# zhizdev/mvdfusion

Measured on AMD Instinct MI355X. Metric: denoising-steps/sec, higher is better.
Workload: dtype f16x3 (f16 MFMA operands split hi+lo, 3 partial products, fp32 accumulate); 1 GPU; BASELINE.json configs[1]: V=4 views x 256^2 images (32x32 latents), D=1, 50-step DDIM (eta 1), cfg 2.5, SD1.x UNet 320ch + 10 view-aligned transformers + GridAttn, random-init (deterministic fill) weights; views=4, latent=32, depth_samples=1, parallelism=single GPU, CFG pair batched as 2V, hipgraph=True, gemm_tuning=mvdfusion_amd/tuned/gemm_f16.json: 426 problems; 0 problems tuned in this run

## Files before the change

include/mvd_hip.h:

```cpp
#ifndef MVD_HIP_H
#define MVD_HIP_H
#include <stddef.h>
#include <stdint.h>
#ifdef __cplusplus
extern "C" {
#endif

typedef void* mvd_stream_t;

#define MVD_VERSION 100
#define MVD_PREC_X1 1
#define MVD_PREC_X3 3
#define MVD_PREC_X4 4

int mvd_version(void);
const char* mvd_last_error(void);
int mvd_operand_format(void);

size_t mvd_packed_weight_bytes(int N, int K);
int mvd_pack_linear_weight(const float* w, int N, int K, int ldw, int geglu, float scale, void* packed,
                           mvd_stream_t stream);
int mvd_pack_linear_weight_t(const float* wt, int N, int K, int ldw, float scale, void* packed, mvd_stream_t stream);
int mvd_pack_conv3x3_weight(const float* w, int Cout, int Cin, int cin_pad, float scale, void* packed,
                            mvd_stream_t stream);

#define MVD_A_DENSE 0
#define MVD_A_CONV3X3 1

#define MVD_EPI_STORE 0
#define MVD_EPI_GEGLU 1
#define MVD_EPI_QKV 2

#define MVD_ACT_NONE 0
#define MVD_ACT_GELU 1
#define MVD_ACT_SILU 2
#define MVD_ACT_QUICKGELU 3

#define MVD_GEMM_TILES 5
#define MVD_GEMM_LOOPS 8
#define MVD_GEMM_CFG_STRIDE 32
#define MVD_B_PACKED 0
#define MVD_B_PLANES 1

typedef struct mvd_prefetch_item_s {
  const void* ptr;
  unsigned long long bytes;
  int start_after;
  int consumer;
} mvd_prefetch_item;

typedef struct mvd_gemm_desc {
  int M, N, K;
  const void* A;
  int lda;
  int a_mode;
  int B, Hin, Win, Cin, Hout, Wout, stride, upsample;
  int no_pad_tl;
  const void* Wp;
  int b_mode;
  int ldb;
  float acc_scale;
  int prec;
  int epi;
  int act;
  float* out;
  int ldo;
  void* out_sp;
  int ldp;
  int n_store;
  const float* bias;
  const float* bias_b;
  int rows_per_batch;
  int ldbb;
  const float* colscale;
  const float* res;
  int ldr;
  void *q_hi, *q_lo, *k_hi, *k_lo, *vt_hi, *vt_lo;
  int heads, dhead, L, Lpad;
  float qscale;
  int splitk;
  float* workspace;
  size_t workspace_elems;
  int cfg;
  long long* gn_stats;
  int gn_hw, gn_groups;
  float* rs_out;
  int* rs_count;
  int rs_ld;
  const float* ln_stats;
  const int* ln_count;
  const float* ln_colsum;
  int ln_ld, ln_dim;
  float ln_eps;
  void* gna_out_sp;
  const float* gna_gamma;
  const float* gna_beta;
  float gna_eps;
  int gna_flags;
  const float* cat_b;
  int cat_cb;
  void* cat_raw_sp;
  const float* acc_scale_dev;
  const struct mvd_prefetch_item_s* pf_items;
  int pf_n;
  int tap_mode;
  const void* A2;
  int lda2, Cin2;
} mvd_gemm_desc;
#define MVD_TAPS_FULL 0
#define MVD_TAPS_UP4 1
#define MVD_TAPS_CENTRE_TAIL 2
#define MVD_GNA_SILU 1
#define MVD_GNA_ROUND_F16 2
#define MVD_GNA_OUT_UNUSED 4

int mvd_gemm(const mvd_gemm_desc* d, mvd_stream_t stream);
int mvd_gemm_cfg_supported(const mvd_gemm_desc* d, int cfg);

int mvd_split_planes(const float* x, void* sp, size_t rows, int cols, int ldx, int ldp, mvd_stream_t stream);
int mvd_split_planes_scaled(const float* x, void* sp, size_t rows, int cols, int ldx, int ldp, const float* scale_dev, mvd_stream_t stream);

int mvd_gemv(const float* W, const float* bias, const float* x, float* y, int M, int N, int K, int ldx, int ldy,
             int act_in, int act_out, mvd_stream_t stream);

int mvd_groupnorm_chunks(int HW);
int mvd_groupnorm_nhwc(const float* x, void* y_sp, const float* gamma, const float* beta, int B, int HW, int C,
                       int groups, float eps, int silu, double* ws, size_t ws_elems, mvd_stream_t stream);
int mvd_groupnorm_from_stats(const float* x, void* y_sp, const float* gamma, const float* beta, const long long* stats, int B, int HW,
                             int C, int groups, float eps, int silu, mvd_stream_t stream);
int mvd_softmax_rows(const float* x, void* y_sp, int rows, int cols, int ldx, float scale, float out_scale,
                     mvd_stream_t stream);

int mvd_layernorm(const float* x, void* y_sp, float* y_f32, const float* w, const float* b, int rows, int C, float eps,
                  int w_plus_one, mvd_stream_t stream);
int mvd_layernorm_groups(const float* x, void* y_sp, float* y_f32, const float* w, const float* b, int ldw, int rows, int rows_per_group,
                         int C, float eps, int w_plus_one, mvd_stream_t stream);

size_t mvd_attn_qk_plane_elems(int B, int heads, int L, int dhead);
size_t mvd_attn_vt_plane_elems(int B, int heads, int L, int dhead);
int mvd_attn_lpad(int L);
int mvd_attention(const void* q_hi, const void* q_lo, const void* k_hi, const void* k_lo, const void* vt_hi,
                  const void* vt_lo, void* out_sp, int ldo, int B, int heads, int L, int Lkeys, int dhead, int prec,
                  mvd_stream_t stream);

int mvd_pixel_cross_attn(const float* q, const float* k, const float* v, void* out_sp, int P, int D, int heads,
                         int dhead, mvd_stream_t stream);

int mvd_unet_input(const float* x, const float* input_latents, void* out_sp, int V, int S, int cpad, int cfg,
                   mvd_stream_t stream);
int mvd_unet_input_scenes(const float* x, const float* input_latents, void* out_sp, int nscene, int V, int S, int cpad, int cfg,
                          mvd_stream_t stream);
int mvd_concat_channels(const float* a, int Ca, const float* b, int Cb, float* out, void* out_sp, int rows, long long* gn_stats,
                        int gn_hw, int gn_groups, mvd_stream_t stream);
int mvd_concat_groupnorm_fits(int Ca, int Cb, int hw, int groups);
int mvd_concat_groupnorm(const float* a, int Ca, const float* b, int Cb, float* out, void* raw_sp, void* y_sp, const float* gamma,
                         const float* beta, long long* gn_stats, int B, int hw, int groups, float eps, int silu, mvd_stream_t stream);
int mvd_area_pool(const float* vol, void* out_sp, int B, int S, int D, int C, int factor, int ldp, mvd_stream_t stream);
int mvd_fill_zero(float* p, size_t n, mvd_stream_t stream);

#define MVD_STEP_STRIDE 8
int mvd_timestep_embedding(const float* steps, const int* iter, const float* freqs, float* out, int dim,
                           mvd_stream_t stream);
int mvd_timestep_embedding_scenes(const float* steps, const int* iter, const float* freqs, float* out, int dim, int nscene,
                                  int steps_scene_stride, mvd_stream_t stream);
int mvd_advance_iter(int* iter, mvd_stream_t stream);

#define MVD_CAM_RECORD 20
#define MVD_TOKEN_DIM 723
#define MVD_TOKEN_LD 736
int mvd_zembed(const float* lat, const float* w, const float* b, float* feat, int N, int S, mvd_stream_t stream);
int mvd_gridattn_tokens(const float* x, const float* depth_noise, const float* steps, const int* iter,
                        const float* grid_lin ,
                        const float* feat, const float* in_feat, const float* cams, const float* in_cam,
                        void* tokens_sp, int V, int q0, int Vq, int S, int D, float depth_scale, float depth_shift,
                        mvd_stream_t stream);
int mvd_gridattn_tokens_scenes(const float* x, const float* depth_noise, const float* steps, const int* iter, const float* grid_lin,
                               const float* feat, const float* in_feat, const float* cams, const float* in_cam, void* tokens_sp,
                               int nscene, int V, int q0, int Vq, int S, int D, float depth_scale, float depth_shift,
                               mvd_stream_t stream);
int mvd_gridattn_tokens_scenes_t(const float* x, const float* depth_noise, const float* steps, const int* iter, const float* grid_lin,
                                 const float* feat, const float* in_feat, const float* cams, const float* in_cam, void* tokens_sp,
                                 int nscene, int V, int q0, int Vq, int S, int D, float depth_scale, float depth_shift,
                                 int steps_scene_stride, mvd_stream_t stream);
int mvd_gridattn_fused_slots(void);
size_t mvd_gridattn_fused_stream_bytes(void);
size_t mvd_gridattn_fused_vec_floats(void);
int mvd_gridattn_fused(const float* x, const float* depth_noise, const float* steps, const int* iter, const float* grid_lin,
                       const float* feat, const float* in_feat, const float* cams, const float* in_cam, const void* wstream,
                       const float* vecs, void* pooled_sp, int V, int q0, int Vq, int S, int D, float depth_scale,
                       float depth_shift, int prec ,
                       mvd_stream_t stream);
int mvd_gridattn_fused_scenes(const float* x, const float* depth_noise, const float* steps, const int* iter, const float* grid_lin,
                              const float* feat, const float* in_feat, const float* cams, const float* in_cam, const void* wstream,
                              const float* vecs, void* pooled_sp, int nscene, int V, int q0, int Vq, int S, int D, float depth_scale,
                              float depth_shift, int prec, mvd_stream_t stream);
int mvd_gridattn_fused_scenes_t(const float* x, const float* depth_noise, const float* steps, const int* iter, const float* grid_lin,
                                const float* feat, const float* in_feat, const float* cams, const float* in_cam, const void* wstream,
                                const float* vecs, void* pooled_sp, int nscene, int V, int q0, int Vq, int S, int D, float depth_scale,
                                float depth_shift, int prec, int steps_scene_stride, int vecs_scene_stride, mvd_stream_t stream);
int mvd_gridattn_tokens_window(const float* x, const float* depth_noise, const float* steps, const int* iter, const float* grid_lin,
                               const float* feat, const float* in_feat, const float* cams, const float* in_cam, void* tokens_sp,
                               int nscene, int V, int q0, int Vq, int S, int D, float depth_scale, float depth_shift,
                               int steps_scene_stride, int window, mvd_stream_t stream);
int mvd_gridattn_fused_window(const float* x, const float* depth_noise, const float* steps, const int* iter, const float* grid_lin,
                              const float* feat, const float* in_feat, const float* cams, const float* in_cam, const void* wstream,
                              const float* vecs, void* pooled_sp, int nscene, int V, int q0, int Vq, int S, int D, float depth_scale,
                              float depth_shift, int prec, int steps_scene_stride, int vecs_scene_stride, int window,
                              mvd_stream_t stream);
int mvd_view_mha(const float* qkv, void* out_sp, int Nseq, int V, int heads, int dhead,
                 mvd_stream_t stream);
int mvd_view_pool(const float* x, const float* w, const float* b, void* out_sp, int Nseq, int V, int C,
                  mvd_stream_t stream);

int mvd_cfg_ddim_update(const float* eps_nhwc, int ldc, float* x, float* x0, float* eps_out,
                        const float* ddim_noise, size_t noise_stride ,
                        const float* steps, const int* iter, int V, int S, int cfg, float cfg_scale, int do_update,
                        mvd_stream_t stream);

int mvd_pin_views(float* x, float* x0, const float* known, const float* noise, size_t noise_stride ,
                  const float* steps, const int* iter, int groups, int group_views, int K, int S, int mode, mvd_stream_t stream);

#define MVD_FUSE_FOREGROUND 1
#define MVD_FUSE_STAGE_AUTO 0
#define MVD_FUSE_STAGE_GLOBAL 1
#define MVD_FUSE_STAGE_LDS 2
int mvd_fuse_points(const float* lat, const float* rgb, const float* cams, const float* ndc_lin, float* xyz, float* color,
                    uint8_t* support, uint8_t* conflict, uint8_t* flags, int nscene, int V, int S, int up, float depth_scale,
                    float depth_shift, float lo, float hi, float tau, int stage, mvd_stream_t stream);
size_t mvd_compact_points_scratch(size_t npts);
int mvd_compact_points(const float* xyz, const float* color, const uint8_t* support, const uint8_t* conflict, const uint8_t* flags,
                       size_t npts, int min_support, int max_conflicts, float* out_xyz, float* out_color, uint8_t* out_support,
                       int* out_index, unsigned* count, void* scratch, size_t scratch_bytes, mvd_stream_t stream);

#define MVD_SPLAT_MAX_RADIUS 4
#define MVD_RENDER_FILL 1
#define MVD_RENDER_SPLAT 2
#define MVD_RENDER_RESOLVE 4
#define MVD_RENDER_ALL 7
size_t mvd_render_points_scratch(int ncam, int P);
int mvd_render_points(const float* xyz, const float* color, const int* scene_start, const float* cams, size_t n, int nscene, int M, int P,
                      int radius, float znear, float empty_depth, const float* background, int* index, float* depth, float* rgb,
                      void* scratch, size_t scratch_bytes, mvd_stream_t stream);
int mvd_render_points_stages(const float* xyz, const float* color, const int* scene_start, const float* cams, size_t n, int nscene, int M,
                             int P, int radius, float znear, float empty_depth, const float* background, int* index, float* depth,
                             float* rgb, void* scratch, size_t scratch_bytes, int stages, mvd_stream_t stream);

size_t mvd_render_mesh_scratch(int ncam, int P);
int mvd_render_mesh(const float* vertices, const float* colors, const int* faces, const int* vertex_start, const int* face_start,
                    const float* cams, size_t nvert, size_t nface, int nscene, int M, int P, int cull, float znear, float empty_depth,
                    const float* background, int* face_out, float* depth, float* bary, float* normal, float* rgb, void* scratch,
                    size_t scratch_bytes, mvd_stream_t stream);
int mvd_render_mesh_stages(const float* vertices, const float* colors, const int* faces, const int* vertex_start, const int* face_start,
                           const float* cams, size_t nvert, size_t nface, int nscene, int M, int P, int cull, float znear,
                           float empty_depth, const float* background, int* face_out, float* depth, float* bary, float* normal, float* rgb,
                           void* scratch, size_t scratch_bytes, int stages, mvd_stream_t stream);

#define MVD_NN_AUTO 0
#define MVD_NN_BRUTE 1
#define MVD_NN_GRID 2
#define MVD_NN_BUILD 1
#define MVD_NN_QUERY 2
#define MVD_NN_ALL 3
size_t mvd_nearest_points_scratch(size_t nt, int nscene, int method, int grid);
int mvd_nearest_points(const float* query, const int* query_start, const float* target, const int* target_start, size_t nq, size_t nt,
                       int nscene, int method, int grid, int* index, float* dist2, void* scratch, size_t scratch_bytes,
                       mvd_stream_t stream);
int mvd_nearest_points_stages(const float* query, const int* query_start, const float* target, const int* target_start, size_t nq,
                              size_t nt, int nscene, int method, int grid, int* index, float* dist2, void* scratch, size_t scratch_bytes,
                              int stages, mvd_stream_t stream);

#define MVD_KNN_MAX_K 32
#define MVD_NORMALS_MAX_K 256
#define MVD_NORMALS_SWEEPS 10
int mvd_knn_points(const float* query, const int* query_start, const float* target, const int* target_start, size_t nq, size_t nt,
                   int nscene, int k, int method, int grid, int* index, float* dist2, void* scratch, size_t scratch_bytes,
                   mvd_stream_t stream);
int mvd_knn_points_stages(const float* query, const int* query_start, const float* target, const int* target_start, size_t nq, size_t nt,
                          int nscene, int k, int method, int grid, int* index, float* dist2, void* scratch, size_t scratch_bytes,
                          int stages, mvd_stream_t stream);
int mvd_point_normals(const float* target, size_t nt, const int* index, size_t n, int k, const float* points, const float* toward,
                      float* normal, float* variation, mvd_stream_t stream);

#define MVD_ALIGN_SCALE 1
#define MVD_ALIGN_NO_STEP 2
#define MVD_ALIGN_CHUNK 1024
#define MVD_ALIGN_SUMS 19
#define MVD_ALIGN_HISTORY 3
#define MVD_ALIGN_MAX_ITERS 1024
size_t mvd_align_scratch(size_t nq, size_t nt, int nscene, int method, int grid);
int mvd_align_solve(const double* sums, int flags, double* step, double* scale);
int mvd_align_apply(const float* src, const int* src_start, size_t n, int nscene, const double* transform, float* out,
                    mvd_stream_t stream);
int mvd_align_fit(const float* moved, const int* start, const float* target, const int* index, const float* dist2, size_t n, size_t nt,
                  int nscene, int flags, float max_dist2, double* transform, double* history_row, void* scratch, size_t scratch_bytes,
                  mvd_stream_t stream);
int mvd_align_icp(const float* source, const int* source_start, const float* target, const int* target_start, size_t nq, size_t nt,
                  int nscene, int method, int grid, int iters, int flags, float max_dist2, double* transform, double* history,
                  float* moved, int* index, float* dist2, void* scratch, size_t scratch_bytes, mvd_stream_t stream);

#define MVD_PLANE_NO_STEP 2
#define MVD_PLANE_SUMS 30
#define MVD_PLANE_HISTORY 4
#define MVD_PLANE_EPS_RANK 1e-9
size_t mvd_plane_scratch(size_t nq, size_t nt, int nscene, int method, int grid);
int mvd_plane_solve(const double* sums, double* step, int* rank);
int mvd_plane_fit(const float* moved, const int* start, const float* target, const float* normals, const int* index, const float* dist2,
                  size_t n, size_t nt, int nscene, int flags, float max_dist2, double* transform, double* history_row, void* scratch,
                  size_t scratch_bytes, mvd_stream_t stream);
int mvd_plane_icp(const float* source, const int* source_start, const float* target, const int* target_start, const float* normals,
                  size_t nq, size_t nt, int nscene, int method, int grid, int iters, float max_dist2, double* transform, double* history,
                  float* moved, int* index, float* dist2, void* scratch, size_t scratch_bytes, mvd_stream_t stream);

#define MVD_MESH_SPAN 3
size_t mvd_nearest_on_mesh_scratch(size_t nf, int nscene, int method, int grid);
int mvd_nearest_on_mesh(const float* query, const int* query_start, const float* vertices, const int* faces, const int* face_start, size_t nq,
                        size_t nv, size_t nf, int nscene, int method, int grid, int* face, float* dist2, float* point, float* bary,
                        int* region, float* normal, void* scratch, size_t scratch_bytes, mvd_stream_t stream);
int mvd_nearest_on_mesh_stages(const float* query, const int* query_start, const float* vertices, const int* faces, const int* face_start,
                               size_t nq, size_t nv, size_t nf, int nscene, int method, int grid, int* face, float* dist2, float* point,
                               float* bary, int* region, float* normal, void* scratch, size_t scratch_bytes, int stages,
                               mvd_stream_t stream);
size_t mvd_mesh_icp_scratch(size_t nq, size_t nf, int nscene, int method, int grid);
int mvd_mesh_icp(const float* source, const int* source_start, const float* vertices, const int* faces, const int* face_start, size_t nq,
                 size_t nv, size_t nf, int nscene, int method, int grid, int iters, float max_dist2, double* transform, double* history,
                 float* moved, int* face, float* dist2, float* point, float* normal, void* scratch, size_t scratch_bytes,
                 mvd_stream_t stream);

#define MVD_REGISTER_MAX_H 16384
#define MVD_REGISTER_MAX_K 32
size_t mvd_register_scratch(size_t ns, size_t nt, int nscene, int H, int method, int grid);
int mvd_register_score(const float* sample, const int* sample_start, const float* target, const int* target_start, size_t ns, size_t nt,
                       int nscene, int H, const double* hyp, float trunc2, int method, int grid, double* score, int* inliers, void* scratch,
                       size_t scratch_bytes, mvd_stream_t stream);
int mvd_register_select(const double* score, const double* quat, int nscene, int H, int K, double cos_half, int* top, double* top_score,
                        mvd_stream_t stream);

int mvd_tsdf_integrate(const float* lat, const float* rgb, const float* cams, float* tsdf, uint8_t* weight, float* color, uint8_t* cweight,
                       int nscene, int V, int S, int up, int G, float cx, float cy, float cz, float half_extent, float trunc, int carve,
                       float depth_scale, float depth_shift, float lo, float hi, mvd_stream_t stream);
size_t mvd_mesh_scratch(int nscene, int G);
int mvd_mesh_count(const float* tsdf, const uint8_t* weight, int nscene, int G, int* vertex_start, int* face_start, void* scratch,
                   size_t scratch_bytes, mvd_stream_t stream);
int mvd_mesh_emit(const float* tsdf, const uint8_t* weight, const float* color, const uint8_t* cweight, int nscene, int G, float cx, float cy,
                  float cz, float half_extent, const float* fill, float* vertices, float* colors, int* faces, size_t nvert, size_t nface,
                  const void* scratch, size_t scratch_bytes, mvd_stream_t stream);

#define MVD_TOPO_TOTALS 11
#define MVD_TOPO_FLAG_BOUNDARY 1
#define MVD_TOPO_FLAG_NONMANIFOLD 2
#define MVD_SMOOTH_MAX_PASSES 2000
size_t mvd_mesh_incidence_scratch(size_t nv, size_t nf);
int mvd_mesh_incidence(const int* faces, const int* vertex_start, const int* face_start, size_t nv, size_t nf, int nscene, int* inc_start,
                       int* inc, void* scratch, size_t scratch_bytes, mvd_stream_t stream);
size_t mvd_mesh_label_scratch(size_t nv, size_t nf);
int mvd_mesh_label(const int* faces, const int* vertex_start, const int* face_start, size_t nv, size_t nf, int nscene, int* vertex_component,
                   int* face_component, int* component_start, void* scratch, size_t scratch_bytes, mvd_stream_t stream);
int mvd_mesh_component_table(const int* vertex_component, const int* face_component, size_t nv, size_t nf, size_t ncomp, int* root, int* faces,
                             int* vertices, mvd_stream_t stream);
size_t mvd_mesh_topology_scratch(size_t nv, size_t nf);
int mvd_mesh_topology(const int* faces, const int* vertex_start, const int* face_start, size_t nv, size_t nf, int nscene, const int* inc_start,
                      const int* inc, const int* vertex_component, const int* component_start, int* totals, uint8_t* vertex_flags,
                      void* scratch, size_t scratch_bytes, mvd_stream_t stream);
size_t mvd_mesh_filter_scratch(size_t nv, size_t nf);
int mvd_mesh_filter_count(const int* faces, const uint8_t* keep, const int* vertex_start, const int* face_start, size_t nv, size_t nf,
                          int nscene, int* new_vertex_start, int* new_face_start, void* scratch, size_t scratch_bytes, mvd_stream_t stream);
int mvd_mesh_filter_emit(const float* vertices, const float* rgb, const int* faces, size_t nv, size_t nf, float* out_vertices, float* out_rgb,
                         int* out_faces, int* vertex_index, int* face_index, size_t nvo, size_t nfo, const void* scratch,
                         size_t scratch_bytes, mvd_stream_t stream);
int mvd_mesh_vertex_normals(const float* vertices, const int* faces, const int* inc_start, const int* inc, size_t nv, size_t nf,
                            float* normals, mvd_stream_t stream);
// ... 92 lines not shown
```

mvdfusion_amd/csrc/elementwise.hip:

```cpp
#include "common.hpp"
#include "../../include/mvd_hip.h"

namespace {

__device__ __forceinline__ float act_apply(float v, int act) {
  if (act == MVD_ACT_GELU) return gelu_erf(v);
  if (act == MVD_ACT_SILU) return silu_f(v);
  return v;
}

template <int MR>
__global__ __launch_bounds__(256) void gemv_kernel(const float* __restrict__ W, const float* __restrict__ bias,
                                                   const float* __restrict__ x, float* __restrict__ y, int M, int N, int K, int ldx,
                                                   int ldy, int act_in, int act_out) {
  const int lane = threadIdx.x & 63;
  const int n = blockIdx.x * 4 + (threadIdx.x >> 6);
  if (n >= N) return;
  float acc[MR];
#pragma unroll
  for (int m = 0; m < MR; ++m) acc[m] = 0.f;
  const float* wr = W + (size_t)n * K;
  if ((K & 3) == 0) {
    for (int k = lane * 4; k < K; k += 256) {
      const float4 w4 = *(const float4*)(wr + k);
#pragma unroll
      for (int m = 0; m < MR; ++m) {
        if (m < M) {
          float4 x4 = *(const float4*)(x + (size_t)m * ldx + k);
          if (act_in) {
            x4.x = act_apply(x4.x, act_in);
            x4.y = act_apply(x4.y, act_in);
            x4.z = act_apply(x4.z, act_in);
            x4.w = act_apply(x4.w, act_in);
          }
          acc[m] += w4.x * x4.x + w4.y * x4.y + w4.z * x4.z + w4.w * x4.w;
        }
      }
    }
  } else {
    for (int k = lane; k < K; k += 64) {
      const float w1 = wr[k];
#pragma unroll
      for (int m = 0; m < MR; ++m)
        if (m < M) acc[m] += w1 * act_apply(x[(size_t)m * ldx + k], act_in);
    }
  }
#pragma unroll
  for (int m = 0; m < MR; ++m) {
    if (m < M) {
      float v = wave_sum(acc[m]);
      if (lane == 0) {
        if (bias) v += bias[n];
        y[(size_t)m * ldy + n] = act_apply(v, act_out);
      }
    }
  }
}

__global__ __launch_bounds__(256) void unet_input_kernel(const float* __restrict__ x, const float* __restrict__ il,
                                                         u16* __restrict__ out_sp, int V, int Vs, int S, int cpad, int nb) {
  const int SS = S * S;
  const size_t total = (size_t)nb * SS * cpad;
  for (size_t e = (size_t)blockIdx.x * 256 + threadIdx.x; e < total; e += (size_t)gridDim.x * 256) {
    const int c = (int)(e % cpad);
    const int pix = (int)((e / cpad) % SS);
    const int b = (int)(e / ((size_t)cpad * SS));
    const int v = b < V ? b : b - V;
    float o = 0.f;
    if (c < 5) {
      o = x[((size_t)v * 5 + c) * SS + pix];
    } else if (c < 10 && b < V) {
      const float t = il[((size_t)(b / Vs) * 5 + (c - 5)) * SS + pix];
      o = (c < 9) ? t / 0.18215f : t;
    }
    store_sp1(out_sp, e / cpad, cpad, c, o);
  }
}

__global__ __launch_bounds__(256) void concat_kernel(const float4* __restrict__ a, int ca4, const float4* __restrict__ b, int cb4,
                                                     float4* __restrict__ out, u16* __restrict__ out_sp, size_t rows) {
  const int c4 = ca4 + cb4;
  const size_t total = rows * c4;
  for (size_t e = (size_t)blockIdx.x * 256 + threadIdx.x; e < total; e += (size_t)gridDim.x * 256) {
    const size_t r = e / c4;
    const int c = (int)(e - r * c4);
    const float4 v = c < ca4 ? a[r * ca4 + c] : b[r * cb4 + (c - ca4)];
    out[e] = v;
    if (out_sp) store_sp4(out_sp, r, c4 * 4, c * 4, v.x, v.y, v.z, v.w);
  }
}

__global__ __launch_bounds__(256) void concat_stats_kernel(const float4* __restrict__ a, int ca4, const float4* __restrict__ b, int cb4,
                                                           float4* __restrict__ out, u16* __restrict__ out_sp, long long* __restrict__ stats,
                                                           int hw, int groups) {
  __shared__ float cs[2][4][256];
  const int c4n = ca4 + cb4, C = c4n * 4;
  const size_t m0 = (size_t)blockIdx.x * 16;
  const int n0 = blockIdx.y * 256;
  const int c4 = blockIdx.y * 64 + (threadIdx.x & 63), rg = threadIdx.x >> 6;
  float4 s = make_float4(0.f, 0.f, 0.f, 0.f), q = make_float4(0.f, 0.f, 0.f, 0.f);
  if (c4 < c4n) {
    float4 v[4];
#pragma unroll
    for (int r = 0; r < 4; ++r) {
      const size_t row = m0 + rg * 4 + r;
      v[r] = c4 < ca4 ? a[row * ca4 + c4] : b[row * cb4 + (c4 - ca4)];
    }
#pragma unroll
    for (int r = 0; r < 4; ++r) {
      const size_t row = m0 + rg * 4 + r;
      out[row * c4n + c4] = v[r];
      if (out_sp) store_sp4(out_sp, row, C, c4 * 4, v[r].x, v[r].y, v[r].z, v[r].w);
      s.x += v[r].x; s.y += v[r].y; s.z += v[r].z; s.w += v[r].w;
      q.x += v[r].x * v[r].x; q.y += v[r].y * v[r].y; q.z += v[r].z * v[r].z; q.w += v[r].w * v[r].w;
    }
  }
  *(float4*)&cs[0][rg][(threadIdx.x & 63) * 4] = s;
  *(float4*)&cs[1][rg][(threadIdx.x & 63) * 4] = q;
  __syncthreads();
  const int c = threadIdx.x, nn = n0 + c;
  const float cs_ = cs[0][0][c] + cs[0][1][c] + cs[0][2][c] + cs[0][3][c];
  const float cq_ = cs[1][0][c] + cs[1][1][c] + cs[1][2][c] + cs[1][3][c];
  __syncthreads();
  cs[0][0][c] = cs_;
  cs[1][0][c] = cq_;
  __syncthreads();
  if (nn >= C) return;
  const int cg = C / groups;
  const int g = nn / cg, pos = nn - g * cg;
  if (c != 0 && pos != 0) return;
  int len = cg - pos;
  if (len > 256 - c) len = 256 - c;
  float ss = 0.f, qq = 0.f;
  for (int j = 0; j < len; ++j) {
    ss += cs[0][0][c + j];
    qq += cs[1][0][c + j];
  }
  gn_stats_add(stats, (int)(m0 / hw), g, groups, ss, qq);
}

#define MVD_CGN_THREADS 1024
__global__ __launch_bounds__(MVD_CGN_THREADS) void concat_gn_kernel(const float* __restrict__ a, int ca, const float* __restrict__ b, int cb,
                                                                    float* __restrict__ out, u16* __restrict__ raw_sp, u16* __restrict__ y_sp,
                                                                    const float* __restrict__ gamma, const float* __restrict__ beta,
                                                                    long long* __restrict__ stats, int hw, int groups, float eps, int flags) {
  constexpr int NT = MVD_CGN_THREADS, NWV = NT / 64, U = 4;
  extern __shared__ float s_val[];
  __shared__ double s_red[2][NWV];
  __shared__ float s_coef[2][128];
  const int C = ca + cb, cg = C / groups, cg2 = cg >> 1;
  int g, img;
  {
    const int bid = blockIdx.x;
    if ((groups & 7) == 0) {
      const int gpx = groups >> 3, x = bid & 7, r = bid >> 3;
      g = x * gpx + r % gpx;
      img = r / gpx;
    } else {
      g = bid % groups;
      img = bid / groups;
    }
  }
  const int tid = threadIdx.x, lane = tid & 63, wave = tid >> 6;
  const int c0 = g * cg;
  const size_t m0 = (size_t)img * hw;
  const int total = hw * cg2;
  const int dq = NT / cg2, dj = NT - dq * cg2;
  const int rs = tid / cg2, js = tid - rs * cg2;
  const int r0 = tid < total ? rs : 0, j0 = tid < total ? js : 0;
  float s = 0.f, q = 0.f;
  {
    int r = rs, j = js;
    for (int e0 = tid; e0 < total; e0 += NT * U) {
      float2 v[U];
      int rr[U], jj[U];
      bool ok[U];
#pragma unroll
      for (int u = 0; u < U; ++u) {
        ok[u] = e0 + u * NT < total;
        rr[u] = ok[u] ? r : r0;
        jj[u] = ok[u] ? j : j0;
        r += dq;
        j += dj;
        if (j >= cg2) {
          j -= cg2;
          ++r;
        }
      }
#pragma unroll
      for (int u = 0; u < U; ++u) {
        const size_t m = m0 + rr[u];
        const int n = c0 + 2 * jj[u];
        v[u] = *(const float2*)(n < ca ? a + m * ca + n : b + m * cb + (n - ca));
      }
#pragma unroll
      for (int u = 0; u < U; ++u) {
        if (ok[u]) {
          const size_t m = m0 + rr[u];
          const int n = c0 + 2 * jj[u];
          if (out) *(float2*)(out + m * C + n) = v[u];
          if (raw_sp) {
            uint32_t hh, ll;
            split_op16x2(v[u].x, v[u].y, hh, ll);
            u16* pp = raw_sp + sp_index(m, C, n);
            *(uint32_t*)pp = hh;
            *(uint32_t*)(pp + 32) = ll;
          }
          *(float2*)(s_val + 2 * (e0 + u * NT)) = v[u];
          s += v[u].x + v[u].y;
          q += v[u].x * v[u].x + v[u].y * v[u].y;
        }
      }
    }
  }
  {
    const double sd = wave_sum_d((double)s), qd = wave_sum_d((double)q);
    if (lane == 0) {
      s_red[0][wave] = sd;
      s_red[1][wave] = qd;
    }
  }
  __syncthreads();
  double S1 = 0.0, S2 = 0.0;
#pragma unroll
  for (int w = 0; w < NWV; ++w) {
    S1 += s_red[0][w];
    S2 += s_red[1][w];
  }
  const double cnt = (double)hw * cg;
  const double mean = S1 / cnt;
  double var = S2 / cnt - mean * mean;
  if (var < 0.0) var = 0.0;
  const float rstd = (float)(1.0 / sqrt(var + (double)eps));
  if (tid < cg) {
    const float aa = rstd * gamma[c0 + tid];
    s_coef[0][tid] = aa;
    s_coef[1][tid] = beta[c0 + tid] - (float)mean * aa;
  }
  if (tid == 0 && stats) gn_stats_add(stats, img, g, groups, (float)S1, (float)S2);
  __syncthreads();
  {
    int r = rs, j = js;
    for (int e = tid; e < total; e += NT) {
      float2 v = *(const float2*)(s_val + 2 * e);
      v.x = v.x * s_coef[0][2 * j] + s_coef[1][2 * j];
      v.y = v.y * s_coef[0][2 * j + 1] + s_coef[1][2 * j + 1];
      if (flags & 2) {
        v.x = (float)(_Float16)v.x;
        v.y = (float)(_Float16)v.y;
      }
      if (flags & 1) {
        v.x = silu_f(v.x);
        v.y = silu_f(v.y);
      }
      uint32_t hh, ll;
      split_op16x2(v.x, v.y, hh, ll);
      u16* pp = y_sp + sp_index(m0 + r, C, c0 + 2 * j);
      *(uint32_t*)pp = hh;
      *(uint32_t*)(pp + 32) = ll;
      r += dq;
      j += dj;
      if (j >= cg2) {
        j -= cg2;
        ++r;
      }
    }
  }
}

__global__ __launch_bounds__(256) void area_pool_kernel(const float4* __restrict__ vol, u16* __restrict__ out_sp, int B, int S,
                                                        int D, int C4, int f, int ldp) {
  const int So = S / f;
  const size_t total = (size_t)B * So * So * D * C4;
  const float inv = 1.0f / (float)(f * f);
  for (size_t e = (size_t)blockIdx.x * 256 + threadIdx.x; e < total; e += (size_t)gridDim.x * 256) {
    const int c = (int)(e % C4);
    size_t r = e / C4;
    const int d = (int)(r % D);
    r /= D;
    const int ox = (int)(r % So);
    r /= So;
    const int oy = (int)(r % So);
    const int b = (int)(r / So);
    float4 acc = make_float4(0.f, 0.f, 0.f, 0.f);
    for (int dy = 0; dy < f; ++dy)
#pragma unroll 8
      for (int dx = 0; dx < f; ++dx) {
        const float4 v = vol[((((size_t)b * S + oy * f + dy) * S + ox * f + dx) * D + d) * C4 + c];
        acc.x += v.x;
        acc.y += v.y;
        acc.z += v.z;
        acc.w += v.w;
      }
    store_sp4(out_sp, e / C4, ldp, c * 4, acc.x * inv, acc.y * inv, acc.z * inv, acc.w * inv);
  }
}

__global__ __launch_bounds__(256) void fill_zero_kernel(float* p, size_t n) {
  for (size_t e = (size_t)blockIdx.x * 256 + threadIdx.x; e < n; e += (size_t)gridDim.x * 256) p[e] = 0.f;
}

__global__ void timestep_embedding_kernel(const float* __restrict__ steps, const int* __restrict__ iter,
                                          const float* __restrict__ freqs, float* __restrict__ out, int dim, int steps_scene_stride) {
  const float t = steps[((size_t)iter[0] + (size_t)blockIdx.x * steps_scene_stride) * MVD_STEP_STRIDE + 0];
  out += (size_t)blockIdx.x * dim;
  const int half = dim / 2;
  for (int i = threadIdx.x; i < half; i += blockDim.x) {
    const float a = t * freqs[i];
    out[i] = cosf(a);
    out[half + i] = sinf(a);
  }
}

__global__ void advance_iter_kernel(int* iter) {
  if (threadIdx.x == 0) iter[0] += 1;
}

__global__ __launch_bounds__(256) void cfg_ddim_kernel(const float* __restrict__ eps_nhwc, int ldc, float* __restrict__ x,
                                                       float* __restrict__ x0, float* __restrict__ eps_out,
                                                       const float* __restrict__ noise, const float* __restrict__ steps,
                                                       const int* __restrict__ iter, int V, int S, int cfg, float cfg_scale,
                                                       int do_update, size_t noise_stride) {
  const int it = iter[0];
  const float* st = steps + (size_t)it * MVD_STEP_STRIDE;
  const float a_t = st[3], a_prev = st[4], sigma = st[5], s1m = st[6], has_noise = st[7];
  const int SS = S * S;
  const size_t total = (size_t)V * 5 * SS;
  for (size_t e = (size_t)blockIdx.x * 256 + threadIdx.x; e < total; e += (size_t)gridDim.x * 256) {
    const int pix = (int)(e % SS);
    const int c = (int)((e / SS) % 5);
    const int b = (int)(e / ((size_t)5 * SS));
    float ep = eps_nhwc[((size_t)b * SS + pix) * ldc + c];
    if (cfg) {
      const float eu = eps_nhwc[((size_t)(V + b) * SS + pix) * ldc + c];
      ep = eu + cfg_scale * (ep - eu);
    }
    if (eps_out) eps_out[e] = ep;
    if (do_update) {
      const float xv = x[e];
      const float px0 = (xv - s1m * ep) / sqrtf(a_t);
      const float dir = sqrtf(fmaxf(1.0f - a_prev - sigma * sigma, 1e-7f)) * ep;
      float xp = sqrtf(a_prev) * px0 + dir;
      if (has_noise != 0.f) xp = xp + sigma * noise[(size_t)it * noise_stride + e];
      x0[e] = px0;
      x[e] = xp;
    }
  }
}

template <typename T>
__device__ __forceinline__ T pin_axpy(float sa, const T& k, float s1, const T& n);
template <>
__device__ __forceinline__ float pin_axpy<float>(float sa, const float& k, float s1, const float& n) {
  return sa * k + s1 * n;
}
template <>
__device__ __forceinline__ float4 pin_axpy<float4>(float sa, const float4& k, float s1, const float4& n) {
  return make_float4(sa * k.x + s1 * n.x, sa * k.y + s1 * n.y, sa * k.z + s1 * n.z, sa * k.w + s1 * n.w);
}

template <typename T>
__global__ __launch_bounds__(256) void pin_views_kernel(T* __restrict__ x, T* __restrict__ x0, const T* __restrict__ known,
                                                        const T* __restrict__ noise, size_t nstride, const float* __restrict__ steps,
                                                        const int* __restrict__ iter, int group_views, int K, size_t rowlen, size_t total,
                                                        int mode) {
  float sa = 1.f, s1 = 0.f;
  size_t nbase = 0;
  if (mode == 1) {
    const int it = iter[0];
    const float* st = steps + (size_t)it * MVD_STEP_STRIDE;
    sa = st[1];
    s1 = st[6];
    nbase = (size_t)it * nstride;
  }
  for (size_t e = (size_t)blockIdx.x * 256 + threadIdx.x; e < total; e += (size_t)gridDim.x * 256) {
    const size_t p = e / rowlen;
    const size_t off = e - p * rowlen;
    const size_t dst = ((p / K) * group_views + p % K) * rowlen + off;
    const T kv = known[e];
    if (mode == 1) {
      x[dst] = pin_axpy<T>(sa, kv, s1, noise[nbase + e]);
      x0[dst] = kv;
    } else {
      x[dst] = kv;
    }
  }
}

inline int grid_for(size_t total, int cap = 2048) {
  size_t b = (total + 255) / 256;
  if (b > (size_t)cap) b = cap;
  if (b < 1) b = 1;
  return (int)b;
}

}

extern "C" int mvd_gemv(const float* W, const float* bias, const float* x, float* y, int M, int N, int K, int ldx, int ldy,
                        int act_in, int act_out, mvd_stream_t stream) {
  MVD_CHECK_ARG(W && x && y && M > 0 && M <= 16 && N > 0 && K > 0, "mvd_gemv: bad arguments (M <= 16)");
  if ((K & 3) == 0) MVD_CHECK_ARG((ldx & 3) == 0, "mvd_gemv: ldx must be a multiple of 4 when K is");
  hipStream_t s = (hipStream_t)stream;
  dim3 grid(cdiv(N, 4)), block(256);
  if (M <= 1)
    hipLaunchKernelGGL(gemv_kernel<1>, grid, block, 0, s, W, bias, x, y, M, N, K, ldx, ldy, act_in, act_out);
  else if (M <= 4)
    hipLaunchKernelGGL(gemv_kernel<4>, grid, block, 0, s, W, bias, x, y, M, N, K, ldx, ldy, act_in, act_out);
  else
    hipLaunchKernelGGL(gemv_kernel<16>, grid, block, 0, s, W, bias, x, y, M, N, K, ldx, ldy, act_in, act_out);
  MVD_CHECK_LAUNCH("mvd_gemv");
  return 0;
}

extern "C" int mvd_unet_input_scenes(const float* x, const float* input_latents, void* out_sp, int nscene, int V, int S, int cpad, int cfg,
                                     mvd_stream_t stream) {
  MVD_CHECK_ARG(x && input_latents && out_sp && cpad % 32 == 0 && V > 0 && S > 0 && cpad >= 10, "mvd_unet_input: bad arguments");
  MVD_CHECK_ARG(nscene >= 1 && (long long)nscene * V <= 0x3fffffff, "mvd_unet_input_scenes: nscene=%d (>= 1)", nscene);
  const int NV = nscene * V;
  const int nb = cfg ? 2 * NV : NV;
  const size_t total = (size_t)nb * S * S * cpad;
  hipLaunchKernelGGL(unet_input_kernel, dim3(grid_for(total)), dim3(256), 0, (hipStream_t)stream, x, input_latents, (u16*)out_sp, NV, V,
                     S, cpad, nb);
  MVD_CHECK_LAUNCH("mvd_unet_input");
  return 0;
}

extern "C" int mvd_unet_input(const float* x, const float* input_latents, void* out_sp, int V, int S, int cpad, int cfg,
                              mvd_stream_t stream) {
  return mvd_unet_input_scenes(x, input_latents, out_sp, 1, V, S, cpad, cfg, stream);
}

extern "C" int mvd_concat_channels(const float* a, int Ca, const float* b, int Cb, float* out, void* out_sp, int rows,
                                   long long* gn_stats, int gn_hw, int gn_groups, mvd_stream_t stream) {
  if (out_sp) MVD_CHECK_ARG((Ca + Cb) % 32 == 0, "mvd_concat_channels: split-planes output needs (Ca+Cb) %% 32 == 0");
  MVD_CHECK_ARG(a && b && out && rows > 0 && Ca > 0 && Cb > 0 && Ca % 4 == 0 && Cb % 4 == 0,
                "mvd_concat_channels: bad arguments (channel counts must be multiples of 4)");
  if (gn_stats) {
    MVD_CHECK_ARG(rows % 16 == 0 && gn_hw > 0 && gn_hw % 16 == 0 && gn_groups > 0 && (Ca + Cb) % gn_groups == 0,
                  "mvd_concat_channels: gn_stats needs rows %% 16 == 0, gn_hw %% 16 == 0, C %% groups == 0");
    hipLaunchKernelGGL(concat_stats_kernel, dim3(rows / 16, (Ca + Cb + 255) / 256), dim3(256), 0, (hipStream_t)stream, (const float4*)a, Ca / 4,
                       (const float4*)b, Cb / 4, (float4*)out, (u16*)out_sp, gn_stats, gn_hw, gn_groups);
    MVD_CHECK_LAUNCH("mvd_concat_channels/stats");
    return 0;
  }
  const size_t total = (size_t)rows * (Ca + Cb) / 4;
  hipLaunchKernelGGL(concat_kernel, dim3(grid_for(total)), dim3(256), 0, (hipStream_t)stream, (const float4*)a, Ca / 4,
                     (const float4*)b, Cb / 4, (float4*)out, (u16*)out_sp, (size_t)rows);
  MVD_CHECK_LAUNCH("mvd_concat_channels");
  return 0;
}

extern "C" int mvd_concat_groupnorm_fits(int Ca, int Cb, int hw, int groups) {
  const int C = Ca + Cb;
  if (groups <= 0 || C % groups || (Ca & 1) || (Cb & 1)) return 0;
  const int cg = C / groups;
  return (cg & 1) == 0 && cg <= 128 && (size_t)hw * cg * 4 <= 128 * 1024 ? 1 : 0;
}

extern "C" int mvd_concat_groupnorm(const float* a, int Ca, const float* b, int Cb, float* out, void* raw_sp, void* y_sp, const float* gamma,
                                    const float* beta, long long* gn_stats, int B, int hw, int groups, float eps, int silu,
                                    mvd_stream_t stream) {
  MVD_CHECK_ARG(a && b && y_sp && gamma && beta && B > 0 && hw > 0, "mvd_concat_groupnorm: null pointer / bad shape");
  MVD_CHECK_ARG((Ca + Cb) % 32 == 0 && mvd_concat_groupnorm_fits(Ca, Cb, hw, groups),
                "mvd_concat_groupnorm: needs (Ca+Cb) %% 32 == 0, even Ca / Cb / group width <= 128 and hw * (C / groups) * 4 <= 128 KiB of LDS "
                "(Ca=%d Cb=%d hw=%d groups=%d): use mvd_concat_channels + mvd_groupnorm_from_stats", Ca, Cb, hw, groups);
  MVD_CHECK_ARG(((uintptr_t)a & 7) == 0 && ((uintptr_t)b & 7) == 0 && ((uintptr_t)out & 7) == 0 && ((uintptr_t)y_sp & 127) == 0 &&
                    ((uintptr_t)raw_sp & 127) == 0, "mvd_concat_groupnorm: alignment");
  const size_t lds = (size_t)hw * ((Ca + Cb) / groups) * 4;
  {
    static unsigned long long raised = 0;
    const hipError_t e = mvd_raise_dynamic_lds((const void*)concat_gn_kernel, 128 * 1024, &raised);
    MVD_CHECK_ARG(e == hipSuccess, "mvd_concat_groupnorm: hipFuncSetAttribute(MaxDynamicSharedMemorySize): %s", hipGetErrorString(e));
  }
  hipLaunchKernelGGL(concat_gn_kernel, dim3(B * groups), dim3(MVD_CGN_THREADS), lds, (hipStream_t)stream, a, Ca, b, Cb, out, (u16*)raw_sp,
                     (u16*)y_sp, gamma, beta, gn_stats, hw, groups, eps, silu);
  MVD_CHECK_LAUNCH("mvd_concat_groupnorm");
  return 0;
}

extern "C" int mvd_area_pool(const float* vol, void* out_sp, int B, int S, int D, int C, int factor, int ldp,
                             mvd_stream_t stream) {
  MVD_CHECK_ARG(vol && out_sp && C % 32 == 0 && B > 0 && S > 0 && D > 0 && C % 4 == 0 && factor >= 1 && S % factor == 0,
                "mvd_area_pool: bad arguments");
  if (ldp == 0) ldp = C;
  MVD_CHECK_ARG(ldp >= C && ldp % 32 == 0 && ((uintptr_t)out_sp & 127) == 0, "mvd_area_pool: ldp=%d must be >= C, %% 32 == 0", ldp);
  const int So = S / factor;
  const size_t total = (size_t)B * So * So * D * (C / 4);
  hipLaunchKernelGGL(area_pool_kernel, dim3(grid_for(total)), dim3(256), 0, (hipStream_t)stream, (const float4*)vol,
                     (u16*)out_sp, B, S, D, C / 4, factor, ldp);
  MVD_CHECK_LAUNCH("mvd_area_pool");
  return 0;
}

extern "C" int mvd_fill_zero(float* p, size_t n, mvd_stream_t stream) {
  MVD_CHECK_ARG(p != nullptr, "mvd_fill_zero: null pointer");
  if (n == 0) return 0;
  hipLaunchKernelGGL(fill_zero_kernel, dim3(grid_for(n)), dim3(256), 0, (hipStream_t)stream, p, n);
  MVD_CHECK_LAUNCH("mvd_fill_zero");
  return 0;
}

extern "C" int mvd_timestep_embedding(const float* steps, const int* iter, const float* freqs, float* out, int dim,
                                      mvd_stream_t stream) {
  MVD_CHECK_ARG(steps && iter && freqs && out && dim > 0 && dim % 2 == 0, "mvd_timestep_embedding: bad arguments");
  hipLaunchKernelGGL(timestep_embedding_kernel, dim3(1), dim3(256), 0, (hipStream_t)stream, steps, iter, freqs, out, dim, 0);
  MVD_CHECK_LAUNCH("mvd_timestep_embedding");
  return 0;
}

extern "C" int mvd_timestep_embedding_scenes(const float* steps, const int* iter, const float* freqs, float* out, int dim, int nscene,
                                             int steps_scene_stride, mvd_stream_t stream) {
  MVD_CHECK_ARG(steps && iter && freqs && out && dim > 0 && dim % 2 == 0, "mvd_timestep_embedding: bad arguments");
  MVD_CHECK_ARG(nscene >= 1 && nscene <= 65535 && steps_scene_stride >= 0 && (nscene > 1 || steps_scene_stride == 0),
                "mvd_timestep_embedding_scenes: nscene=%d (1 ... 65535), steps_scene_stride=%d (>= 0; 0 when nscene = 1)", nscene,
                steps_scene_stride);
  hipLaunchKernelGGL(timestep_embedding_kernel, dim3(nscene), dim3(256), 0, (hipStream_t)stream, steps, iter, freqs, out, dim,
                     steps_scene_stride);
  MVD_CHECK_LAUNCH("mvd_timestep_embedding_scenes");
  return 0;
}

extern "C" int mvd_advance_iter(int* iter, mvd_stream_t stream) {
  MVD_CHECK_ARG(iter != nullptr, "mvd_advance_iter: null pointer");
  hipLaunchKernelGGL(advance_iter_kernel, dim3(1), dim3(64), 0, (hipStream_t)stream, iter);
  MVD_CHECK_LAUNCH("mvd_advance_iter");
  return 0;
}

extern "C" int mvd_cfg_ddim_update(const float* eps_nhwc, int ldc, float* x, float* x0, float* eps_out,
                                   const float* ddim_noise, size_t noise_stride, const float* steps, const int* iter, int V,
                                   int S, int cfg, float cfg_scale, int do_update, mvd_stream_t stream) {
  MVD_CHECK_ARG(eps_nhwc && steps && iter && V > 0 && S > 0 && ldc >= 5, "mvd_cfg_ddim_update: bad arguments");
  if (do_update) MVD_CHECK_ARG(x && x0 && ddim_noise, "mvd_cfg_ddim_update: update needs x, x0, ddim_noise");
  const size_t total = (size_t)V * 5 * S * S;
  hipLaunchKernelGGL(cfg_ddim_kernel, dim3(grid_for(total)), dim3(256), 0, (hipStream_t)stream, eps_nhwc, ldc, x, x0, eps_out,
                     ddim_noise, steps, iter, V, S, cfg, cfg_scale, do_update, noise_stride);
  MVD_CHECK_LAUNCH("mvd_cfg_ddim_update");
  return 0;
}

extern "C" int mvd_pin_views(float* x, float* x0, const float* known, const float* noise, size_t noise_stride, const float* steps,
                             const int* iter, int groups, int group_views, int K, int S, int mode, mvd_stream_t stream) {
  MVD_CHECK_ARG(x && known && groups > 0 && group_views > 0 && S > 0 && (mode == 0 || mode == 1),
                "mvd_pin_views: bad arguments (null x / known, groups=%d, group_views=%d, S=%d, mode=%d)", groups, group_views, S, mode);
  MVD_CHECK_ARG(K > 0 && K <= group_views, "mvd_pin_views: K=%d pinned views of a %d-view group (0 < K <= group_views)", K, group_views);
  MVD_CHECK_ARG((long long)groups * group_views <= 0x3fffffff, "mvd_pin_views: groups * group_views too large");
  const size_t row = (size_t)5 * S * S;
  if (mode == 1)
    MVD_CHECK_ARG(x0 && noise && steps && iter && noise_stride >= (size_t)groups * K * row,
                  "mvd_pin_views: mode 1 needs x0, noise, steps, iter and noise_stride >= groups * K * 5 * S * S");
  const size_t total = (size_t)groups * K * row;
  hipStream_t s = (hipStream_t)stream;
  if (((size_t)S * S) % 4 == 0) {
    MVD_CHECK_ARG(((uintptr_t)x & 15) == 0 && ((uintptr_t)known & 15) == 0, "mvd_pin_views: x / known must be 16-byte aligned");
    if (mode == 1)
      MVD_CHECK_ARG(((uintptr_t)x0 & 15) == 0 && ((uintptr_t)noise & 15) == 0 && noise_stride % 4 == 0,
                    "mvd_pin_views: x0 / noise must be 16-byte aligned and noise_stride a multiple of 4");
    hipLaunchKernelGGL(pin_views_kernel<float4>, dim3(grid_for(total / 4)), dim3(256), 0, s, (float4*)x, (float4*)x0, (const float4*)known,
                       (const float4*)noise, noise_stride / 4, steps, iter, group_views, K, row / 4, total / 4, mode);
  } else {
    hipLaunchKernelGGL(pin_views_kernel<float>, dim3(grid_for(total)), dim3(256), 0, s, x, x0, known, noise, noise_stride, steps, iter,
                       group_views, K, row, total, mode);
  }
  MVD_CHECK_LAUNCH("mvd_pin_views");
  return 0;
}
```

mvdfusion_amd/csrc/gridattn.hip:

```cpp
#include "gridattn_common.hpp"

namespace {

__device__ __forceinline__ float harmonic(const float* vec, int dim, int e) {
  const int n = dim * 7;
  if (e >= 2 * n) return vec[e - 2 * n];
  const int ee = e < n ? e : e - n;
  const int di = ee / 7, k = ee - di * 7;
  const float w = 0.1f * (float)(1 << k);
  const float a = vec[di] * w;
  return e < n ? sinf(a) : cosf(a);
}
__device__ __forceinline__ void embed105(const Plucker& pl, float depth, int lane, float& v0, float& v1) {
  const float p6[6] = {pl.a, pl.b, pl.c, pl.d, pl.e, pl.f}, dp[1] = {depth};
  const int e0 = lane, e1 = lane + 64;
  v0 = e0 < 90 ? harmonic(p6, 6, e0) : harmonic(dp, 1, e0 - 90);
  v1 = e1 >= 105 ? 0.f : e1 < 90 ? harmonic(p6, 6, e1) : harmonic(dp, 1, e1 - 90);
}

__global__ __launch_bounds__(256) void tokens_kernel(GridGeom g, const float* __restrict__ feat, const float* __restrict__ in_feat,
                                                     u16* __restrict__ tok) {
  const int lane = threadIdx.x & 63;
  const int S = g.S, SS = S * S, W = slots_per_point(g);
  const size_t pt = (size_t)blockIdx.x * 4 + (threadIdx.x >> 6);
  if (pt >= num_points(g)) return;
  const GeomPoint q = decode_point(g, pt, wave_scene(g, pt));
  const Cam cb = view_cam(g, q, q.b);
  float X[3], dir[3];
  const float depth = world_point(g, q, cb, X, dir);
  float qe0, qe1;
  embed105(plucker(dir[0], dir[1], dir[2], cb.C), depth, lane, qe0, qe1);
  const float4 fin = bilinear4(in_feat + (size_t)q.scene * SS * 256, view_taps(input_cam(g, q), X, S), lane * 4);
  for_each_slot(g, q.b, [&](int slot, int vr) {
    const Cam cv = view_cam(g, q, vr);
    const float4 fr = bilinear4(feat + (size_t)(q.gv0 + vr) * SS * 256, view_taps(cv, X, S), lane * 4);
    const Plucker rpl = plucker_to(cv, X);
    float re0, re1;
    embed105(rpl, rpl.norm, lane, re0, re1);
    const size_t row = pt * W + slot;
    store_sp4(tok, row, MVD_TOKEN_LD, lane * 4, fr.x, fr.y, fr.z, fr.w);
    store_sp4(tok, row, MVD_TOKEN_LD, 256 + lane * 4, fin.x, fin.y, fin.z, fin.w);
    store_sp1(tok, row, MVD_TOKEN_LD, 512 + lane, re0);
    if (lane + 64 < 105) store_sp1(tok, row, MVD_TOKEN_LD, 512 + lane + 64, re1);
    store_sp1(tok, row, MVD_TOKEN_LD, 617 + lane, qe0);
    if (lane + 64 < 105) store_sp1(tok, row, MVD_TOKEN_LD, 617 + lane + 64, qe1);
    if (lane < MVD_TOKEN_LD - 722) store_sp1(tok, row, MVD_TOKEN_LD, 722 + lane, lane == 0 ? 1.0f : 0.0f);
  });
}

__global__ __launch_bounds__(256) void zembed_kernel(const float* __restrict__ lat, const float* __restrict__ w,
                                                     const float* __restrict__ bias, float* __restrict__ feat, int N, int SS) {
  const int lane = threadIdx.x & 63;
  const size_t p = (size_t)blockIdx.x * 4 + (threadIdx.x >> 6);
  if (p >= (size_t)N * SS) return;
  const int n = (int)(p / SS), pix = (int)(p % SS);
  float in[5];
#pragma unroll
  for (int c = 0; c < 5; ++c) in[c] = lat[((size_t)n * 5 + c) * SS + pix];
  float o[4];
#pragma unroll
  for (int j = 0; j < 4; ++j) {
    const int ch = lane * 4 + j;
    float a = 0.f;
#pragma unroll
    for (int c = 0; c < 5; ++c) a += in[c] * w[ch * 5 + c];
    o[j] = gelu_erf(a + bias[ch]);
  }
  *(float4*)(feat + p * 256 + lane * 4) = make_float4(o[0], o[1], o[2], o[3]);
}

__device__ __forceinline__ void scatter4(long long* __restrict__ acc, const Taps& t, int ch, float4 g, float scale) {
#pragma unroll
  for (int k = 0; k < 4; ++k) {
    if (t.pix[k] < 0) continue;
    unsigned long long* p = (unsigned long long*)(acc + (size_t)t.pix[k] * 256 + ch);
    const float w = t.w[k] * scale;
    atomicAdd(p + 0, (unsigned long long)(long long)llrintf(g.x * w));
    atomicAdd(p + 1, (unsigned long long)(long long)llrintf(g.y * w));
    atomicAdd(p + 2, (unsigned long long)(long long)llrintf(g.z * w));
    atomicAdd(p + 3, (unsigned long long)(long long)llrintf(g.w * w));
  }
}

__global__ __launch_bounds__(256) void tokens_bwd_kernel(GridGeom g, const float* __restrict__ dtok, int ldt, long long* __restrict__ dfeat,
                                                         long long* __restrict__ din_feat, float scale) {
  const int lane = threadIdx.x & 63;
  const int S = g.S, SS = S * S, W = slots_per_point(g);
  const size_t pt = (size_t)blockIdx.x * 4 + (threadIdx.x >> 6);
  if (pt >= num_points(g)) return;
  const GeomPoint q = decode_point(g, pt, wave_scene(g, pt));
  float X[3], dir[3];
  world_point(g, q, view_cam(g, q, q.b), X, dir);
  float4 gin = make_float4(0.f, 0.f, 0.f, 0.f);
  for_each_slot(g, q.b, [&](int slot, int vr) {
    const float* row = dtok + (pt * W + slot) * (size_t)ldt;
    const float4 gr = *(const float4*)(row + lane * 4);
    scatter4(dfeat + (size_t)(q.gv0 + vr) * SS * 256, view_taps(view_cam(g, q, vr), X, S), lane * 4, gr, scale);
    const float4 gi = *(const float4*)(row + 256 + lane * 4);
    gin.x += gi.x; gin.y += gi.y; gin.z += gi.z; gin.w += gi.w;
  });
  scatter4(din_feat + (size_t)q.scene * SS * 256, view_taps(input_cam(g, q), X, S), lane * 4, gin, scale);
}

}

extern "C" int mvd_zembed(const float* lat, const float* w, const float* b, float* feat, int N, int S, mvd_stream_t stream) {
  MVD_CHECK_ARG(lat && w && b && feat && N > 0 && S > 0, "mvd_zembed: bad arguments");
  const size_t npix = (size_t)N * S * S;
  hipLaunchKernelGGL(zembed_kernel, dim3(cdiv(npix, 4)), dim3(256), 0, (hipStream_t)stream, lat, w, b, feat, N, S * S);
  MVD_CHECK_LAUNCH("mvd_zembed");
  return 0;
}

extern "C" int mvd_gridattn_tokens_window(const float* x, const float* depth_noise, const float* steps, const int* iter,
                                          const float* grid_lin, const float* feat, const float* in_feat, const float* cams,
                                          const float* in_cam, void* tokens_sp, int nscene, int V, int q0, int Vq, int S, int D,
                                          float depth_scale, float depth_shift, int steps_scene_stride, int window, mvd_stream_t stream) {
  const GridGeom g = {x, depth_noise, steps, iter, grid_lin, cams, in_cam, nscene, V, q0, Vq, S, D, depth_scale, depth_shift, steps_scene_stride, window};
  if (const int e = check_geom("mvd_gridattn_tokens_window", g)) return e;
  MVD_CHECK_ARG(feat && in_feat && tokens_sp, "mvd_gridattn_tokens_window: null pointer");
  const size_t npts = num_points(g);
  MVD_CHECK_ARG((npts + 3) / 4 <= 0x7fffffff, "mvd_gridattn_tokens_window: grid too large");
  hipLaunchKernelGGL(tokens_kernel, dim3(cdiv(npts, 4)), dim3(256), 0, (hipStream_t)stream, g, feat, in_feat, (u16*)tokens_sp);
  MVD_CHECK_LAUNCH("mvd_gridattn_tokens_window");
  return 0;
}

extern "C" int mvd_gridattn_tokens_scenes_t(const float* x, const float* depth_noise, const float* steps, const int* iter,
                                            const float* grid_lin, const float* feat, const float* in_feat, const float* cams,
                                            const float* in_cam, void* tokens_sp, int nscene, int V, int q0, int Vq, int S, int D,
                                            float depth_scale, float depth_shift, int steps_scene_stride, mvd_stream_t stream) {
  return mvd_gridattn_tokens_window(x, depth_noise, steps, iter, grid_lin, feat, in_feat, cams, in_cam, tokens_sp, nscene, V, q0, Vq, S, D,
                                    depth_scale, depth_shift, steps_scene_stride, 0, stream);
}

extern "C" int mvd_gridattn_tokens_scenes(const float* x, const float* depth_noise, const float* steps, const int* iter,
                                          const float* grid_lin, const float* feat, const float* in_feat, const float* cams,
                                          const float* in_cam, void* tokens_sp, int nscene, int V, int q0, int Vq, int S, int D,
                                          float depth_scale, float depth_shift, mvd_stream_t stream) {
  return mvd_gridattn_tokens_scenes_t(x, depth_noise, steps, iter, grid_lin, feat, in_feat, cams, in_cam, tokens_sp, nscene, V, q0, Vq, S,
                                      D, depth_scale, depth_shift, 0, stream);
}

extern "C" int mvd_gridattn_tokens(const float* x, const float* depth_noise, const float* steps, const int* iter,
                                   const float* grid_lin, const float* feat, const float* in_feat, const float* cams,
                                   const float* in_cam, void* tokens_sp, int V, int q0, int Vq, int S, int D, float depth_scale,
                                   float depth_shift, mvd_stream_t stream) {
  return mvd_gridattn_tokens_scenes(x, depth_noise, steps, iter, grid_lin, feat, in_feat, cams, in_cam, tokens_sp, 1, V, q0, Vq, S, D,
                                    depth_scale, depth_shift, stream);
}

extern "C" int mvd_gridattn_tokens_backward_window(const float* x, const float* depth_noise, const float* steps, const int* iter,
                                                   const float* grid_lin, const float* cams, const float* in_cam, const float* dtok, int ldt,
                                                   long long* dfeat_acc, long long* din_feat_acc, float scale, int nscene, int V, int q0,
                                                   int Vq, int S, int D, float depth_scale, float depth_shift, int steps_scene_stride,
                                                   int window, mvd_stream_t stream) {
  const GridGeom g = {x, depth_noise, steps, iter, grid_lin, cams, in_cam, nscene, V, q0, Vq, S, D, depth_scale, depth_shift, steps_scene_stride, window};
  if (const int e = check_geom("mvd_gridattn_tokens_backward_window", g)) return e;
  MVD_CHECK_ARG(dtok && dfeat_acc && din_feat_acc, "mvd_gridattn_tokens_backward_window: null pointer");
  MVD_CHECK_ARG(ldt >= 512 && ldt % 4 == 0 && ((uintptr_t)dtok & 15) == 0 && scale > 0.f,
                "mvd_gridattn_tokens_backward_window: bad shape (ldt >= 512, 16-byte aligned dtok, scale > 0)");
  const size_t npts = num_points(g);
  MVD_CHECK_ARG((npts + 3) / 4 <= 0x7fffffff, "mvd_gridattn_tokens_backward_window: grid too large");
  hipLaunchKernelGGL(tokens_bwd_kernel, dim3(cdiv(npts, 4)), dim3(256), 0, (hipStream_t)stream, g, dtok, ldt, dfeat_acc, din_feat_acc, scale);
  MVD_CHECK_LAUNCH("mvd_gridattn_tokens_backward_window");
  return 0;
}

extern "C" int mvd_gridattn_tokens_backward_scenes(const float* x, const float* depth_noise, const float* steps, const int* iter,
                                                   const float* grid_lin, const float* cams, const float* in_cam, const float* dtok, int ldt,
                                                   long long* dfeat_acc, long long* din_feat_acc, float scale, int nscene, int V, int q0,
                                                   int Vq, int S, int D, float depth_scale, float depth_shift, int steps_scene_stride,
                                                   mvd_stream_t stream) {
  return mvd_gridattn_tokens_backward_window(x, depth_noise, steps, iter, grid_lin, cams, in_cam, dtok, ldt, dfeat_acc, din_feat_acc, scale,
                                             nscene, V, q0, Vq, S, D, depth_scale, depth_shift, steps_scene_stride, 0, stream);
}

extern "C" int mvd_gridattn_tokens_backward(const float* x, const float* depth_noise, const float* steps, const int* iter,
                                            const float* grid_lin, const float* cams, const float* in_cam, const float* dtok, int ldt,
                                            long long* dfeat_acc, long long* din_feat_acc, float scale, int V, int q0, int Vq, int S, int D,
                                            float depth_scale, float depth_shift, mvd_stream_t stream) {
  return mvd_gridattn_tokens_backward_scenes(x, depth_noise, steps, iter, grid_lin, cams, in_cam, dtok, ldt, dfeat_acc, din_feat_acc, scale,
                                             1, V, q0, Vq, S, D, depth_scale, depth_shift, 0, stream);
}
```

mvdfusion_amd/engine.py:

```python
import os

import torch

from . import hip


GN_SLOTS = 256
GN_SLOT_ELEMS = 64 * 32 * 2


class Workspace:

    def __init__(self, device):
        self.device = torch.device(device)
        self.bufs = {}
        self.frozen = False

    def get(self, tag, shape, dtype=torch.float32, zero=False):
        key = (tag, tuple(int(s) for s in shape), dtype)
        t = self.bufs.get(key)
        if t is None:
            assert not self.frozen, f"workspace buffer {key} requested during graph capture (the eager warm-up step must " \
                                    "allocate every buffer the captured step uses)"
            t = (torch.zeros if zero else torch.empty)(key[1], dtype=dtype, device=self.device)
            self.bufs[key] = t
        return t

    def planes(self, tag, rows, cols):
        assert cols % 32 == 0, (tag, cols)
        return self.get(tag, (rows, 2 * cols), torch.int16)

    def attn_planes(self, B, heads, L, dhead):
        key = ("attn_planes", B, heads, L, dhead)
        t = self.bufs.get(key)
        if t is None:
            assert not self.frozen, f"attention planes {key} requested during graph capture"
            t = hip.alloc_attn_planes(B, heads, L, dhead, self.device)
            self.bufs[key] = t
        return t

    def nbytes(self):
        n = 0
        for v in self.bufs.values():
            for t in (v if isinstance(v, tuple) else (v,)):
                n += t.numel() * t.element_size()
        return n


class Ctx:
    gn_from_producer = True
    ln_fold = True
    gn_fuse = True

    def __init__(self, device, prec=hip.PREC_X4, policy=None):
        self.device = torch.device(device)
        self.ws = Workspace(device)
        self.prec = prec
        self.policy = dict(policy or {})
        self.B = 0
        self.D = 1
        self.context = None
        self.vol_levels = None
        self.emb_bias = None
        self._rot = {}
        self.capturing = False
        self.gemm_ws = torch.empty(64 * 1024 * 1024, dtype=torch.float32, device=self.device)
        self.gn_arena = torch.zeros(GN_SLOTS * GN_SLOT_ELEMS, dtype=torch.int64, device=self.device)
        self._gn_next = 0
        self._gn = {}
        self._rs = {}
        self.next_gn = None
        self._gn_done = {}
        self._unwritten = set()
        self.next_cat = None
        self._cat_done = set()
        self.keep_fp32 = False

    def begin_step(self):
        self._rot.clear()
        self._gn.clear()
        self._gn_done.clear()
        self._unwritten.clear()
        self._cat_done.clear()
        self.next_gn = None
        self.next_cat = None
        self._gn_next = 0
        if self.gn_from_producer:
            hip.check(hip.lib().mvd_fill_zero(hip.ptr(self.gn_arena), self.gn_arena.numel() * 2, hip.stream()))

    def gn_slot(self, out, B, HW, C):
        n = B * 32 * 2
        if n > GN_SLOT_ELEMS or self._gn_next >= GN_SLOTS:
            return None
        st = self.gn_arena[self._gn_next * GN_SLOT_ELEMS:self._gn_next * GN_SLOT_ELEMS + n]
        self._gn_next += 1
        self._gn[out.data_ptr()] = (st, B, HW, C)
        return st

    def _forget(self, out):
        ptr = out.data_ptr()
        self._gn.pop(ptr, None)
        self._unwritten.discard(ptr)
        if self._gn_done:
            for k in [k for k in self._gn_done if k[0] == ptr]:
                del self._gn_done[k]

    def row_stats(self, tag, rows, width):
        key = (tag, int(rows), int(width))
        rs = self._rs.get(key)
        if rs is None:
            assert not self.ws.frozen, f"row statistics {key} requested during graph capture"
            rs = hip.RowStats(rows, width, self.device)
            self._rs[key] = rs
        return rs

    def act(self, shape):
        key = tuple(int(s) for s in shape)
        i = self._rot.get(key, 0)
        self._rot[key] = (i + 1) % 3
        return self.ws.get(f"act{i}", key)

    def prec_of(self, kind):
        return self.policy.get(kind, self.prec)

    def ln_fold_enabled(self):
        return (self.ln_fold and hip.OPERAND_FORMAT == "f16" and self.prec_of("qkv") >= hip.PREC_X3 and
                self.prec_of("geglu") >= hip.PREC_X3 and self.prec_of("proj") >= hip.PREC_X3)

    def gemm(self, A, W, out, gn=None, kind=None, gn_apply=None, **kw):
        kw.setdefault("prec", self.prec_of(kind))
        kw.setdefault("workspace", self.gemm_ws)
        applied = False
        if out is not None:
            self._forget(out)
            handled = False
            if gn is not None and gn_apply is None and self.next_cat is not None and self.gn_fuse and self.gn_from_producer and \
                    gn[1] % 16 == 0 and out.is_contiguous():
                sk, cat, catp, norm, pname, silu = self.next_cat
                N, cb = out.shape[-1], sk.shape[-1]
                if norm.num_groups == 32 and norm.num_channels == N + cb and sk.shape[0] == out.shape[0] == gn[0] * gn[1] and \
                        sk.is_contiguous() and hip.lib().mvd_concat_groupnorm_fits(N, cb, gn[1], 32):
                    st = self.gn_slot(cat, gn[0], gn[1], N + cb)
                    if st is not None:
                        planes = self.ws.planes(pname, out.shape[0], N + cb)
                        kw.update(gn_stats=st, gn_hw=gn[1], gn_groups=32, cat=(sk, catp),
                                  gn_apply=(norm.weight, norm.bias, norm.eps, (hip.GNA_SILU if silu else 0) | hip.GNA_OUT_UNUSED, planes))
                        self._gn.pop(cat.data_ptr(), None)
                        self._gn_done[(cat.data_ptr(), id(norm))] = (planes, bool(silu))
                        self._unwritten.add(cat.data_ptr())
                        self._unwritten.add(out.data_ptr())
                        self._cat_done.add(cat.data_ptr())
                        handled = True
            if not handled and gn is not None and self.gn_from_producer and gn[1] % 16 == 0 and out.shape[-1] % 32 == 0:
                st = self.gn_slot(out, gn[0], gn[1], out.shape[-1])
                if st is not None:
                    kw.update(gn_stats=st, gn_hw=gn[1], gn_groups=32)
                    if gn_apply is not None and self.gn_fuse and gn_apply[0].num_groups == 32 and out.is_contiguous():
                        norm, planes, silu, unused = gn_apply
                        kw["gn_apply"] = (norm.weight, norm.bias, norm.eps, (hip.GNA_SILU if silu else 0) | (hip.GNA_OUT_UNUSED if unused else 0),
                                          planes)
                        applied = True
                    elif gn_apply is None and self.next_gn is not None and self.gn_fuse and out.is_contiguous():
                        norm, pname, silu = self.next_gn
                        if norm.num_groups == 32 and norm.num_channels == out.shape[-1] and out.shape[0] == gn[0] * gn[1]:
                            planes = self.ws.planes(pname, out.shape[0], out.shape[-1])
                            kw["gn_apply"] = (norm.weight, norm.bias, norm.eps, hip.GNA_SILU if silu else 0, planes)
                            self._gn_done[(out.data_ptr(), id(norm))] = (planes, bool(silu))
        if gn is not None:
            if os.environ.get("MVD_GN_DEBUG") and not self.capturing:
                print(f"[gn] kind={kind} M={out.shape[0]} N={out.shape[-1]} explicit={gn_apply is not None} hint={self.next_gn is not None} "
                      f"cat={self.next_cat is not None} -> fused_apply={'gn_apply' in kw} cat={'cat' in kw}", flush=True)
            if gn_apply is None:
                self.next_gn = None
                self.next_cat = None
        r = hip.gemm(A, W, out, **kw)
        if gn_apply is not None and not applied:
            self.groupnorm(out, gn_apply[1], gn_apply[0], gn[0], gn[1], out.shape[-1], gn_apply[2])
        return r

    def groupnorm(self, x, y, norm, B, HW, C, silu):
        done = self._gn_done.pop((x.data_ptr(), id(norm)), None)
        if done is not None and done[0].data_ptr() == y.data_ptr() and done[0].shape == y.shape and done[1] == bool(silu) and silu in (True, False):
            return y
        if x.data_ptr() in self._unwritten:
            raise RuntimeError("GroupNorm of a tensor whose fused producer left the fp32 data unwritten (Ctx.concat(need_out=False))")
        ent = self._gn.get(x.data_ptr())
        if ent is not None and ent[1:] == (B, HW, C) and norm.num_groups == 32:
            return hip.groupnorm_from_stats(x, y, norm.weight, norm.bias, ent[0], B, HW, C, norm.eps, silu)
        ws = self.ws.get("gn_ws", (B * hip.lib().mvd_groupnorm_chunks(HW) * 32 * 2,), torch.float64)
        return hip.groupnorm(x, y, norm.weight, norm.bias, B, HW, C, norm.eps, silu, ws)

    def concat(self, a, ca, b, cb, out, out_planes, B, HW, gn_apply=None, need_out=True):
        self._forget(out)
        st = None
        if gn_apply is not None and self.gn_fuse and self.gn_from_producer and HW % 16 == 0 and (ca + cb) % 32 == 0 and \
                gn_apply[0].num_groups == 32 and gn_apply[0].num_channels == ca + cb and \
                hip.lib().mvd_concat_groupnorm_fits(ca, cb, HW, 32):
            norm, pname, silu = gn_apply
            st = self.gn_slot(out, B, HW, ca + cb)
            planes = self.ws.planes(pname, B * HW, ca + cb)
            hip.check(hip.lib().mvd_concat_groupnorm(hip.ptr(a), ca, hip.ptr(b), cb, hip.ptr(out) if need_out else None, hip.ptr(out_planes),
                                                     hip.ptr(planes), hip.ptr(norm.weight), hip.ptr(norm.bias),
                                                     hip.ptr(st) if st is not None else None, B, HW, 32, norm.eps, 1 if silu else 0,
                                                     hip.stream()))
            if not need_out:
                self._gn.pop(out.data_ptr(), None)
                self._unwritten.add(out.data_ptr())
            self._gn_done[(out.data_ptr(), id(norm))] = (planes, bool(silu))
            return out
        if self.gn_from_producer and HW % 16 == 0 and (ca + cb) % 32 == 0:
            st = self.gn_slot(out, B, HW, ca + cb)
        hip.check(hip.lib().mvd_concat_channels(hip.ptr(a), ca, hip.ptr(b), cb, hip.ptr(out), hip.ptr(out_planes), B * HW,
                                                hip.ptr(st) if st is not None else None, HW, 32, hip.stream()))
        return out

    def layernorm(self, x, y, norm, rows, C):
        return hip.layernorm(x, y, norm.weight, norm.bias, rows, C, norm.eps)

    def gemv_rows(self, W, bias, x, y, act_in=hip.ACT_NONE, act_out=hip.ACT_NONE):
        for r in range(0, x.shape[0], 16):
            hip.gemv(W, bias, x[r:r + 16], y[r:r + 16], act_in, act_out)
        return y


def ddim_step_table(scheduler_tables, ddim, iters):
    rows = []
    for index in iters:
        t = int(ddim["timesteps"][index])
        sac = float(scheduler_tables["sqrt_alphas_cumprod"][t])
        s1m = float(scheduler_tables["sqrt_one_minus_alphas_cumprod"][t])
        dstd = (scheduler_tables["sqrt_one_minus_alphas_cumprod"][t] / scheduler_tables["sqrt_alphas_cumprod"][t] / 10.0)
        rows.append([float(t), sac, float(dstd), float(ddim["alphas"][index]), float(ddim["alphas_prev"][index]),
                     float(ddim["sigmas"][index]), float(ddim["sqrt_one_minus_alphas"][index]),
                     1.0 if index > 0 else 0.0])
        del s1m
    return torch.tensor(rows, dtype=torch.float32)
```

mvdfusion_amd/hip.py:

```python
import ctypes as C
import os

import torch

_HERE = os.path.dirname(os.path.abspath(__file__))
LIB_PATHS = {"f16": os.path.join(_HERE, "csrc", "libmvd_hip.so"), "bf16": os.path.join(_HERE, "csrc", "libmvd_hip_bf16.so")}
if os.environ.get("MVD_HIP_LIB"):
    LIB_PATHS["f16"] = os.environ["MVD_HIP_LIB"]
LIB_PATH = LIB_PATHS["f16"]
OPERAND_FORMAT = os.environ.get("MVD_OPERAND_FORMAT", "f16")

PREC_X1, PREC_X3, PREC_X4 = 1, 3, 4
PREC_KINDS = ("conv", "skip", "proj", "qkv", "attn", "out", "geglu", "ffproj", "xattn", "ga")


def parse_precision(name):
    base, _, over = name.partition(":")
    names = {"f16": ("f16", PREC_X1), "bf16": ("bf16", PREC_X1), "f16x3": ("f16", PREC_X3), "f16x4": ("f16", PREC_X4),
             "bf16x3": ("bf16", PREC_X3), "bf16x4": ("bf16", PREC_X4)}
    if base not in names:
        raise ValueError(f"precision '{name}': base must be one of {sorted(names)}")
    fmt, default = names[base]
    policy = {}
    for item in filter(None, over.split(",")):
        k, _, v = item.partition("=")
        k = k.strip()
        if k not in PREC_KINDS or int(v) not in (PREC_X1, PREC_X3, PREC_X4):
            raise ValueError(f"precision policy '{name}': '{item}' is not <kind>=<1|3|4> with kind in {PREC_KINDS}")
        policy[k] = int(v)
    return fmt, default, policy
A_DENSE, A_CONV3X3 = 0, 1
TAPS_FULL, TAPS_CENTRE_TAIL = 0, 2
TAPS_UP4 = 1
EPI_STORE, EPI_GEGLU, EPI_QKV = 0, 1, 2
ACT_NONE, ACT_GELU, ACT_SILU, ACT_QUICKGELU = 0, 1, 2, 3
STEP_STRIDE = 8
CAM_RECORD = 20
TOKEN_DIM, TOKEN_LD = 723, 736
FUSE_FOREGROUND = 1
FUSE_STAGE_AUTO, FUSE_STAGE_GLOBAL, FUSE_STAGE_LDS = 0, 1, 2
SPLAT_MAX_RADIUS = 4
RENDER_FILL, RENDER_SPLAT, RENDER_RESOLVE, RENDER_ALL = 1, 2, 4, 7
NN_AUTO, NN_BRUTE, NN_GRID = 0, 1, 2
NN_BUILD, NN_QUERY, NN_ALL = 1, 2, 3
NN_MAX_GRID = 256
KNN_MAX_K = 32
NORMALS_MAX_K, NORMALS_SWEEPS = 256, 10
ALIGN_SCALE, ALIGN_NO_STEP = 1, 2
ALIGN_CHUNK = 1024
ALIGN_SUMS, ALIGN_HISTORY = 19, 3
PLANE_NO_STEP = 2
PLANE_SUMS, PLANE_HISTORY = 30, 4
PLANE_EPS_RANK = 1e-9
ALIGN_MAX_ITERS = 1024
REGISTER_MAX_H, REGISTER_MAX_K = 16384, 32
MESH_SPAN = 3
TOPO_TOTALS = 11
TOPO_FIELDS = ("vertices_used", "unreferenced", "faces_regular", "faces_repeated", "faces_invalid", "edges", "boundary_edges",
               "nonmanifold_edges", "misoriented_edges", "components", "euler")
TOPO_FLAG_BOUNDARY, TOPO_FLAG_NONMANIFOLD = 1, 2
SMOOTH_MAX_PASSES = 2000
SIMPLIFY_MAX_CELLS = 256
SIMPLIFY_MEAN, SIMPLIFY_QUADRIC = 0, 1
SIMPLIFY_PLACED_MEAN, SIMPLIFY_PLACED_QUADRIC, SIMPLIFY_PLACED_FALLBACK = 0, 1, 2
SIMPLIFY_RANK_RATIO = 1e-3
SIMPLIFY_BOX_SLACK_DIV = 1024
SIMPLIFY_MAX_TABLE = 2 ** 28
WIND_AUTO, WIND_EXACT, WIND_CELLS = 0, 1, 2
WIND_MAX_CELLS = 64
WIND_FACE_TILE, WIND_CELL_TILE = 512, 128
WIND_MAX_TABLE = 2 ** 28

_vp, _i, _f, _sz = C.c_void_p, C.c_int, C.c_float, C.c_size_t
c_void_p = C.c_void_p


class GemmDesc(C.Structure):
    _fields_ = [
        ("M", _i), ("N", _i), ("K", _i),
        ("A", _vp), ("lda", _i), ("a_mode", _i),
        ("B", _i), ("Hin", _i), ("Win", _i), ("Cin", _i), ("Hout", _i), ("Wout", _i), ("stride", _i), ("upsample", _i), ("no_pad_tl", _i),
        ("Wp", _vp), ("b_mode", _i), ("ldb", _i), ("acc_scale", _f), ("prec", _i),
        ("epi", _i), ("act", _i), ("out", _vp), ("ldo", _i), ("out_sp", _vp), ("ldp", _i),
        ("n_store", _i),
        ("bias", _vp), ("bias_b", _vp), ("rows_per_batch", _i), ("ldbb", _i), ("colscale", _vp), ("res", _vp), ("ldr", _i),
        ("q_hi", _vp), ("q_lo", _vp), ("k_hi", _vp), ("k_lo", _vp), ("vt_hi", _vp), ("vt_lo", _vp),
        ("heads", _i), ("dhead", _i), ("L", _i), ("Lpad", _i), ("qscale", _f),
        ("splitk", _i), ("workspace", _vp), ("workspace_elems", _sz), ("cfg", _i),
        ("gn_stats", _vp), ("gn_hw", _i), ("gn_groups", _i),
        ("rs_out", _vp), ("rs_count", _vp), ("rs_ld", _i),
        ("ln_stats", _vp), ("ln_count", _vp), ("ln_colsum", _vp), ("ln_ld", _i), ("ln_dim", _i), ("ln_eps", _f),
        ("gna_out_sp", _vp), ("gna_gamma", _vp), ("gna_beta", _vp), ("gna_eps", _f), ("gna_flags", _i),
        ("cat_b", _vp), ("cat_cb", _i), ("cat_raw_sp", _vp),
        ("acc_scale_dev", _vp), ("pf_items", _vp), ("pf_n", _i),
        ("tap_mode", _i), ("A2", _vp), ("lda2", _i), ("Cin2", _i),
    ]


class PrefetchItem(C.Structure):
    _fields_ = [("ptr", _vp), ("bytes", C.c_ulonglong), ("start_after", _i), ("consumer", _i)]


SIGNATURES = {
    "mvd_version": (_i, []),
    "mvd_last_error": (C.c_char_p, []),
    "mvd_packed_weight_bytes": (_sz, [_i, _i]),
    "mvd_operand_format": (_i, []),
    "mvd_pack_linear_weight": (_i, [_vp, _i, _i, _i, _i, _f, _vp, _vp]),
    "mvd_pack_linear_weight_t": (_i, [_vp, _i, _i, _i, _f, _vp, _vp]),
    "mvd_pack_conv3x3_weight": (_i, [_vp, _i, _i, _i, _f, _vp, _vp]),
    "mvd_gemm": (_i, [C.POINTER(GemmDesc), _vp]),
    "mvd_gemm_cfg_supported": (_i, [C.POINTER(GemmDesc), _i]),
    "mvd_split_planes": (_i, [_vp, _vp, _sz, _i, _i, _i, _vp]),
    "mvd_gemv": (_i, [_vp, _vp, _vp, _vp, _i, _i, _i, _i, _i, _i, _i, _vp]),
    "mvd_groupnorm_chunks": (_i, [_i]),
    "mvd_groupnorm_nhwc": (_i, [_vp, _vp, _vp, _vp, _i, _i, _i, _i, _f, _i, _vp, _sz, _vp]),
    "mvd_layernorm": (_i, [_vp, _vp, _vp, _vp, _vp, _i, _i, _f, _i, _vp]),
    "mvd_layernorm_groups": (_i, [_vp, _vp, _vp, _vp, _vp, _i, _i, _i, _i, _f, _i, _vp]),
    "mvd_softmax_rows": (_i, [_vp, _vp, _i, _i, _i, _f, _f, _vp]),
    "mvd_attn_qk_plane_elems": (_sz, [_i, _i, _i, _i]),
    "mvd_attn_vt_plane_elems": (_sz, [_i, _i, _i, _i]),
    "mvd_attn_lpad": (_i, [_i]),
    "mvd_attention": (_i, [_vp] * 7 + [_i, _i, _i, _i, _i, _i, _i, _vp]),
    "mvd_pixel_cross_attn": (_i, [_vp, _vp, _vp, _vp, _i, _i, _i, _i, _vp]),
    "mvd_unet_input": (_i, [_vp, _vp, _vp, _i, _i, _i, _i, _vp]),
    "mvd_unet_input_scenes": (_i, [_vp, _vp, _vp, _i, _i, _i, _i, _i, _vp]),
    "mvd_concat_channels": (_i, [_vp, _i, _vp, _i, _vp, _vp, _i, _vp, _i, _i, _vp]),
    "mvd_concat_groupnorm_fits": (_i, [_i, _i, _i, _i]),
    "mvd_concat_groupnorm": (_i, [_vp, _i, _vp, _i, _vp, _vp, _vp, _vp, _vp, _vp, _i, _i, _i, _f, _i, _vp]),
    "mvd_transpose_planes": (_i, [_vp, _i, _i, _i, _i, _vp, _i, _vp]),
    "mvd_im2col3x3_t_planes": (_i, [_vp, _i, _i, _i, _i, _vp, _i, _vp]),
    "mvd_col_sum_workspace_doubles": (_sz, [_i, _i]),
    "mvd_col_sum": (_i, [_vp, _i, _i, _i, _vp, _vp, _sz, _vp]),
    "mvd_col_sum_groups_workspace_doubles": (_sz, [_i, _i, _i]),
    "mvd_col_sum_groups": (_i, [_vp, _i, _i, _i, _i, _vp, _vp, _sz, _vp]),
    "mvd_col_sum_pow2": (_i, [_vp, _i, _i, _i, _vp, _vp, _sz, _vp, _vp, _vp]),
    "mvd_gridattn_tokens_backward": (_i, [_vp, _vp, _vp, _vp, _vp, _vp, _vp, _vp, _i, _vp, _vp, _f, _i, _i, _i, _i, _i, _f, _f, _vp]),
    "mvd_gridattn_tokens_backward_scenes": (_i, [_vp, _vp, _vp, _vp, _vp, _vp, _vp, _vp, _i, _vp, _vp, _f, _i, _i, _i, _i, _i, _i, _f, _f, _i,
                                                 _vp]),
    "mvd_gridattn_tokens_backward_window": (_i, [_vp, _vp, _vp, _vp, _vp, _vp, _vp, _vp, _i, _vp, _vp, _f, _i, _i, _i, _i, _i, _i, _f, _f, _i,
                                                 _i, _vp]),
    "mvd_layernorm_backward": (_i, [_vp, _vp, _vp, _i, _i, _f, _vp, _vp, _vp]),
    "mvd_layernorm_backward_groups": (_i, [_vp, _vp, _vp, _i, _i, _i, _i, _f, _vp, _vp, _vp, _vp, _vp, _sz, _vp]),
    "mvd_geglu_backward": (_i, [_vp, _vp, _i, _i, _vp, _vp]),
    "mvd_act_planes": (_i, [_vp, _vp, _vp, _sz, _i, _i, _i, _i, _i, _vp]),
    "mvd_act_backward": (_i, [_vp, _vp, _vp, _sz, _i, _vp]),
    "mvd_attention_backward": (_i, [_vp, _vp, _vp, _vp, _i, _i, _i, _i, _vp, _vp, _vp, _vp, _sz, _vp]),
    "mvd_pixel_cross_attn_backward": (_i, [_vp, _vp, _vp, _vp, _i, _i, _i, _i, _vp, _vp, _vp, _vp]),
    "mvd_groupnorm_backward": (_i, [_vp, _vp, _vp, _vp, _i, _i, _i, _i, _f, _i, _vp, _vp, _vp, _vp, _sz, _vp]),
    "mvd_groupnorm_from_stats": (_i, [_vp, _vp, _vp, _vp, _vp, _i, _i, _i, _i, _f, _i, _vp]),
    "mvd_area_pool": (_i, [_vp, _vp, _i, _i, _i, _i, _i, _i, _vp]),
    "mvd_fill_zero": (_i, [_vp, _sz, _vp]),
    "mvd_pow2_scale": (_i, [_vp, _sz, _vp, _vp, _vp]),
    "mvd_split_planes_scaled": (_i, [_vp, _vp, _sz, _i, _i, _i, _vp, _vp]),
    "mvd_transpose_planes_scaled": (_i, [_vp, _i, _i, _i, _vp, _i, _vp, _vp]),
    "mvd_adamw_multi": (_i, [_vp, _i, _i, _f, _f, _f, _f, _f, _f, _f, _f, _vp]),
    "mvd_timestep_embedding": (_i, [_vp, _vp, _vp, _vp, _i, _vp]),
    "mvd_timestep_embedding_scenes": (_i, [_vp, _vp, _vp, _vp, _i, _i, _i, _vp]),
    "mvd_advance_iter": (_i, [_vp, _vp]),
    "mvd_zembed": (_i, [_vp, _vp, _vp, _vp, _i, _i, _vp]),
    "mvd_gridattn_tokens": (_i, [_vp] * 10 + [_i, _i, _i, _i, _i, _f, _f, _vp]),
    "mvd_gridattn_tokens_scenes": (_i, [_vp] * 10 + [_i, _i, _i, _i, _i, _i, _f, _f, _vp]),
    "mvd_gridattn_tokens_scenes_t": (_i, [_vp] * 10 + [_i, _i, _i, _i, _i, _i, _f, _f, _i, _vp]),
    "mvd_gridattn_fused_slots": (_i, []),
    "mvd_gridattn_fused_stream_bytes": (_sz, []),
    "mvd_gridattn_fused_vec_floats": (_sz, []),
    "mvd_gridattn_fused": (_i, [_vp] * 12 + [_i, _i, _i, _i, _i, _f, _f, _i, _vp]),
    "mvd_gridattn_fused_scenes": (_i, [_vp] * 12 + [_i, _i, _i, _i, _i, _i, _f, _f, _i, _vp]),
    "mvd_gridattn_fused_scenes_t": (_i, [_vp] * 12 + [_i, _i, _i, _i, _i, _i, _f, _f, _i, _i, _i, _vp]),
    "mvd_gridattn_tokens_window": (_i, [_vp] * 10 + [_i, _i, _i, _i, _i, _i, _f, _f, _i, _i, _vp]),
    "mvd_gridattn_fused_window": (_i, [_vp] * 12 + [_i, _i, _i, _i, _i, _i, _f, _f, _i, _i, _i, _i, _vp]),
    "mvd_view_mha": (_i, [_vp, _vp, _i, _i, _i, _i, _vp]),
    "mvd_view_pool": (_i, [_vp, _vp, _vp, _vp, _i, _i, _i, _vp]),
    "mvd_cfg_ddim_update": (_i, [_vp, _i, _vp, _vp, _vp, _vp, _sz, _vp, _vp, _i, _i, _i, _f, _i, _vp]),
    "mvd_pin_views": (_i, [_vp, _vp, _vp, _vp, _sz, _vp, _vp, _i, _i, _i, _i, _i, _vp]),
    "mvd_fuse_points": (_i, [_vp] * 9 + [_i, _i, _i, _i, _f, _f, _f, _f, _f, _i, _vp]),
    "mvd_compact_points_scratch": (_sz, [_sz]),
    "mvd_compact_points": (_i, [_vp] * 5 + [_sz, _i, _i, _vp, _vp, _vp, _vp, _vp, _vp, _sz, _vp]),
    "mvd_render_points_scratch": (_sz, [_i, _i]),
    "mvd_render_points": (_i, [_vp] * 4 + [_sz, _i, _i, _i, _i, _f, _f, C.POINTER(_f), _vp, _vp, _vp, _vp, _sz, _vp]),
    "mvd_render_points_stages": (_i, [_vp] * 4 + [_sz, _i, _i, _i, _i, _f, _f, C.POINTER(_f), _vp, _vp, _vp, _vp, _sz, _i, _vp]),
    "mvd_render_mesh_scratch": (_sz, [_i, _i]),
    "mvd_render_mesh": (_i, [_vp] * 6 + [_sz, _sz, _i, _i, _i, _i, _f, _f, C.POINTER(_f)] + [_vp] * 6 + [_sz, _vp]),
    "mvd_render_mesh_stages": (_i, [_vp] * 6 + [_sz, _sz, _i, _i, _i, _i, _f, _f, C.POINTER(_f)] + [_vp] * 6 + [_sz, _i, _vp]),
    "mvd_nearest_points_scratch": (_sz, [_sz, _i, _i, _i]),
    "mvd_nearest_points": (_i, [_vp] * 4 + [_sz, _sz, _i, _i, _i, _vp, _vp, _vp, _sz, _vp]),
    "mvd_nearest_points_stages": (_i, [_vp] * 4 + [_sz, _sz, _i, _i, _i, _vp, _vp, _vp, _sz, _i, _vp]),
    "mvd_knn_points": (_i, [_vp] * 4 + [_sz, _sz, _i, _i, _i, _i, _vp, _vp, _vp, _sz, _vp]),
    "mvd_knn_points_stages": (_i, [_vp] * 4 + [_sz, _sz, _i, _i, _i, _i, _vp, _vp, _vp, _sz, _i, _vp]),
    "mvd_point_normals": (_i, [_vp, _sz, _vp, _sz, _i, _vp, _vp, _vp, _vp, _vp]),
    "mvd_align_scratch": (_sz, [_sz, _sz, _i, _i, _i]),
    "mvd_align_solve": (_i, [_vp, _i, _vp, _vp]),
    "mvd_align_apply": (_i, [_vp, _vp, _sz, _i, _vp, _vp, _vp]),
    "mvd_align_fit": (_i, [_vp] * 5 + [_sz, _sz, _i, _i, _f, _vp, _vp, _vp, _sz, _vp]),
    "mvd_align_icp": (_i, [_vp] * 4 + [_sz, _sz, _i, _i, _i, _i, _i, _f] + [_vp] * 6 + [_sz, _vp]),
    "mvd_plane_scratch": (_sz, [_sz, _sz, _i, _i, _i]),
    "mvd_plane_solve": (_i, [_vp, _vp, _vp]),
    "mvd_plane_fit": (_i, [_vp] * 6 + [_sz, _sz, _i, _i, _f, _vp, _vp, _vp, _sz, _vp]),
    "mvd_plane_icp": (_i, [_vp] * 5 + [_sz, _sz, _i, _i, _i, _i, _f] + [_vp] * 6 + [_sz, _vp]),
    "mvd_nearest_on_mesh_scratch": (_sz, [_sz, _i, _i, _i]),
    "mvd_nearest_on_mesh": (_i, [_vp] * 5 + [_sz, _sz, _sz, _i, _i, _i] + [_vp] * 7 + [_sz, _vp]),
    "mvd_nearest_on_mesh_stages": (_i, [_vp] * 5 + [_sz, _sz, _sz, _i, _i, _i] + [_vp] * 7 + [_sz, _i, _vp]),
    "mvd_mesh_icp_scratch": (_sz, [_sz, _sz, _i, _i, _i]),
    "mvd_mesh_icp": (_i, [_vp] * 5 + [_sz, _sz, _sz, _i, _i, _i, _i, _f] + [_vp] * 8 + [_sz, _vp]),
    "mvd_register_scratch": (_sz, [_sz, _sz, _i, _i, _i, _i]),
    "mvd_register_score": (_i, [_vp] * 4 + [_sz, _sz, _i, _i, _vp, _f, _i, _i, _vp, _vp, _vp, _sz, _vp]),
    "mvd_register_select": (_i, [_vp, _vp, _i, _i, _i, C.c_double, _vp, _vp, _vp]),
    "mvd_tsdf_integrate": (_i, [_vp] * 7 + [_i, _i, _i, _i, _i, _f, _f, _f, _f, _f, _i, _f, _f, _f, _f, _vp]),
    "mvd_mesh_scratch": (_sz, [_i, _i]),
    "mvd_mesh_count": (_i, [_vp, _vp, _i, _i, _vp, _vp, _vp, _sz, _vp]),
    "mvd_mesh_emit": (_i, [_vp] * 4 + [_i, _i, _f, _f, _f, _f, C.POINTER(_f), _vp, _vp, _vp, _sz, _sz, _vp, _sz, _vp]),
    "mvd_mesh_incidence_scratch": (_sz, [_sz, _sz]),
    "mvd_mesh_incidence": (_i, [_vp] * 3 + [_sz, _sz, _i, _vp, _vp, _vp, _sz, _vp]),
    "mvd_mesh_label_scratch": (_sz, [_sz, _sz]),
    "mvd_mesh_label": (_i, [_vp] * 3 + [_sz, _sz, _i, _vp, _vp, _vp, _vp, _sz, _vp]),
    "mvd_mesh_component_table": (_i, [_vp, _vp, _sz, _sz, _sz, _vp, _vp, _vp, _vp]),
    "mvd_mesh_topology_scratch": (_sz, [_sz, _sz]),
    "mvd_mesh_topology": (_i, [_vp] * 3 + [_sz, _sz, _i] + [_vp] * 7 + [_sz, _vp]),
    "mvd_mesh_filter_scratch": (_sz, [_sz, _sz]),
    "mvd_mesh_filter_count": (_i, [_vp] * 4 + [_sz, _sz, _i, _vp, _vp, _vp, _sz, _vp]),
    "mvd_mesh_filter_emit": (_i, [_vp] * 3 + [_sz, _sz] + [_vp] * 5 + [_sz, _sz, _vp, _sz, _vp]),
    "mvd_mesh_vertex_normals": (_i, [_vp] * 4 + [_sz, _sz, _vp, _vp]),
    "mvd_mesh_smooth": (_i, [_vp] * 5 + [_sz, _sz, _i, C.c_double, C.c_double, _i, _vp, _vp, _vp]),
    "mvd_mesh_cluster_scratch": (_sz, [_sz, _sz, _i, _i]),
    "mvd_mesh_cluster_count": (_i, [_vp] * 3 + [_sz, _sz, _i, _i, _vp, _vp, _vp, _sz, _vp]),
    "mvd_mesh_cluster_emit": (_i, [_vp] * 8 + [_sz, _sz, _i, _i, _i, _sz] + [_vp] * 8 + [_sz, _vp]),
    "mvd_mesh_cluster_dedupe": (_i, [_vp] * 4 + [_sz, _sz, _vp, _vp]),
    "mvd_winding_scratch": (_sz, [_sz, _i, _i, _i]),
    "mvd_winding_number": (_i, [_vp] * 5 + [_sz, _sz, _sz, _i, _i, _i, C.c_double, _vp, _vp, _vp, _sz, _vp]),
    "mvd_winding_number_stages": (_i, [_vp] * 5 + [_sz, _sz, _sz, _i, _i, _i, C.c_double, _vp, _vp, _vp, _sz, _i, _vp]),
    "mvd_graph_begin": (_i, [_vp]),
    "mvd_graph_end": (_i, [_vp, C.POINTER(_vp)]),
    "mvd_graph_launch": (_i, [_vp, _vp]),
    "mvd_graph_destroy": (_i, [_vp]),
    "mvd_event_create": (_i, [C.POINTER(_vp)]),
    "mvd_event_record": (_i, [_vp, _vp]),
    "mvd_event_elapsed_ms": (_i, [_vp, _vp, C.POINTER(_f)]),
    "mvd_event_destroy": (_i, [_vp]),
}

_lib = None


def lib():
    global _lib
    if _lib is None:
        path = LIB_PATHS[OPERAND_FORMAT]
        if not os.path.exists(path):
            raise RuntimeError(
                f"{path} not found: build it with `python -m mvdfusion_amd.csrc.build` "
                "(or `python -c 'import __graft_entry__ as g; g.build()'`). mvdfusion_amd has no CPU fallback.")
        l = C.CDLL(path)
        for name, (res, args) in SIGNATURES.items():
            fn = getattr(l, name)
            fn.restype, fn.argtypes = res, args
        assert l.mvd_operand_format() == {"f16": 0xf16, "bf16": 0xbf16}[OPERAND_FORMAT]
        _lib = l
        load_default_tuned()
    return _lib


def set_operand_format(fmt):
    global OPERAND_FORMAT
    assert fmt in LIB_PATHS
    if _lib is not None and fmt != OPERAND_FORMAT:
        raise RuntimeError(f"operand format already fixed to {OPERAND_FORMAT} for this process")
    OPERAND_FORMAT = fmt


def check(rc):
    if rc != 0:
        raise RuntimeError(f"mvd_hip error {rc}: {lib().mvd_last_error().decode()}")


try:
    _raw_stream = torch._C._cuda_getCurrentRawStream
    _cur_device = torch._C._cuda_getDevice
except AttributeError:
    _raw_stream = None


def stream():
    if _raw_stream is not None:
        return C.c_void_p(_raw_stream(_cur_device()))
    return C.c_void_p(torch.cuda.current_stream().cuda_stream)


def ptr(t):
    if t is None:
        return None
    return C.c_void_p(t.data_ptr())


def _req(t, dtype=torch.float32):
    assert t.is_cuda and t.dtype == dtype and t.is_contiguous(), (t.device, t.dtype, t.shape, t.stride())
    return t


class PackedWeight:

    __slots__ = ("data", "N", "K", "n_real", "bias", "geglu", "conv_cin", "acc_scale", "tail_cin", "up4")

    def __init__(self, data, N, K, n_real, bias, geglu=False, conv_cin=0, acc_scale=1.0, tail_cin=0, up4=False):
        self.data, self.N, self.K, self.n_real, self.bias, self.geglu, self.conv_cin = data, N, K, n_real, bias, geglu, conv_cin
        self.acc_scale = acc_scale
        self.tail_cin = tail_cin
        self.up4 = up4


class RowStats:

    __slots__ = ("slots", "count", "ld")
# ... 115 lines not shown
    w = weight.detach().contiguous().float()
    Cout, Cin = w.shape[0], w.shape[1]
    cin_pad = (Cin + 31) // 32 * 32
    Np = (Cout + 15) // 16 * 16
    data = torch.empty(Np * 9 * cin_pad * 4, dtype=torch.uint8, device=w.device)
    scale = _pack_scale(w, like if like is not None else weight)
    check(lib().mvd_pack_conv3x3_weight(ptr(w), Cout, Cin, cin_pad, scale, ptr(data), stream()))
    b = None
    if bias is not None:
        b = torch.zeros(Np, dtype=torch.float32, device=w.device)
        b[:Cout] = bias.detach().float()
    return PackedWeight(data, Np, 9 * cin_pad, Cout, b, conv_cin=cin_pad, acc_scale=1.0 / scale)


def tap_schedule(cin, cin2=0):
    assert cin % 32 == 0 and cin2 % 32 == 0
    return [(0, cb, tap) for cb in range(cin // 32) for tap in range(9)] + [(1, cb, 4) for cb in range(cin2 // 32)]


def up4_schedule(weight):
    w = weight.detach()
    assert w.dim() == 4 and tuple(w.shape[2:]) == (3, 3)
    rows = torch.tensor([[[1, 0, 0], [0, 1, 1]], [[1, 1, 0], [0, 0, 1]]], dtype=torch.float64, device=w.device)
    wq = torch.einsum("ayk,cxl,oikl->acoiyx", rows, rows, w.double()).reshape(4, w.shape[0], w.shape[1], 2, 2).to(w.dtype)
    nb = (w.shape[1] + 31) // 32
    return wq, [(par, cb, tap) for par in range(4) for cb in range(nb) for tap in range(4)]


def pack_conv3x3_up4(weight, bias=None):
    wq, _ = up4_schedule(weight.detach().float())
    Cout, Cin = wq.shape[1], wq.shape[2]
    cin_pad, Np = (Cin + 31) // 32 * 32, (Cout + 15) // 16 * 16
    K = 4 * cin_pad
    m = torch.zeros(4, Cout, cin_pad, 4, dtype=torch.float32, device=wq.device)
    m[:, :, :Cin] = wq.reshape(4, Cout, Cin, 4)
    m = m.reshape(4, Cout, cin_pad // 32, 32, 4).permute(0, 1, 2, 4, 3).reshape(4, Cout, K).contiguous()
    img = Np * K * 4
    data = torch.empty(4 * img, dtype=torch.uint8, device=wq.device)
    scale = _pack_scale(m)
    for par in range(4):
        check(lib().mvd_pack_linear_weight(ptr(m[par]), Cout, K, K, 0, scale, ptr(data[par * img:]), stream()))
    b = None
    if bias is not None:
        b = torch.zeros(Np, dtype=torch.float32, device=wq.device)
        b[:Cout] = bias.detach().float()
    return PackedWeight(data, Np, K, Cout, b, conv_cin=cin_pad, acc_scale=1.0 / scale, up4=True)


UP4_MIN_ROWS = int(os.environ.get("MVD_UP4_MIN_ROWS", "128"))


def use_up4(B, Hin, Win, training=False):
    return UP4_MIN_ROWS > 0 and not training and (Hin * Win) % 16 == 0 and B * Hin * Win >= UP4_MIN_ROWS


def compose_conv_tail_bias(bias, tail_bias):
    if bias is None and tail_bias is None:
        return None
    terms = [t.detach().double() for t in (bias, tail_bias) if t is not None]
    return sum(terms[1:], terms[0]).float()


def pack_conv3x3_tail(weight, bias, tail_weight, tail_bias):
    w = weight.detach().contiguous().float()
    wt = tail_weight.detach().reshape(tail_weight.shape[0], -1).contiguous().float()
    Cout, Cin, Cin2 = w.shape[0], w.shape[1], wt.shape[1]
    assert wt.shape[0] == Cout
    cin_pad, cin2_pad, Np = (Cin + 31) // 32 * 32, (Cin2 + 31) // 32 * 32, (Cout + 15) // 16 * 16
    n_main = Np * 9 * cin_pad * 4
    data = torch.empty(n_main + Np * cin2_pad * 4, dtype=torch.uint8, device=w.device)
    scale = min(_pack_scale(w, weight), _pack_scale(wt, tail_weight))
    check(lib().mvd_pack_conv3x3_weight(ptr(w), Cout, Cin, cin_pad, scale, ptr(data), stream()))
    check(lib().mvd_pack_linear_weight(ptr(wt), Cout, Cin2, Cin2, 0, scale, ptr(data[n_main:]), stream()))
    bsum = compose_conv_tail_bias(bias, tail_bias)
    b = None
    if bsum is not None:
        b = torch.zeros(Np, dtype=torch.float32, device=w.device)
        b[:Cout] = bsum
    return PackedWeight(data, Np, 9 * cin_pad + cin2_pad, Cout, b, conv_cin=cin_pad, acc_scale=1.0 / scale, tail_cin=cin2_pad)


_CACHE_ATTRS = ("_p", "_p4", "_pg", "_temb", "_xattn", "_head", "_pq", "_q", "_fused", "_lnf")


def params_signature(module):
    slots = module.__dict__.get("_mvd_sig_slots")
    if slots is None:
        ps, bs, seen = [], [], set()
        for m in module.modules():
            for n, p in m._parameters.items():
                if p is not None and id(p) not in seen:
                    seen.add(id(p))
                    ps.append((m._parameters, n))
            for n, b in m._buffers.items():
                if b is not None and id(b) not in seen:
                    seen.add(id(b))
                    bs.append((m._buffers, n))
        slots = module.__dict__["_mvd_sig_slots"] = (ps, bs)
    ps, bs = slots
    sig = []
    for d_, n in ps:
        p = d_.get(n)
        sig.append((p.data_ptr(), p._version) if p is not None else None)
    for d_, n in bs:
        b = d_.get(n)
        sig.append(b.data_ptr() if b is not None else None)
    return hash(tuple(sig))


def drop_packed_caches(module):
    module.__dict__.pop("_mvd_sig_slots", None)
    for m in module.modules():
        for name in _CACHE_ATTRS:
            if name in m.__dict__:
                cur = m.__dict__[name]
                if isinstance(cur, dict):
                    m.__dict__[name] = {}
                elif cur is not None:
                    m.__dict__[name] = None


def check_finite(t, what):
    if not bool(torch.isfinite(t).all()):
        raise FloatingPointError(
            f"{what}: non-finite values. mvd_hip splits GEMM operands into fp16 hi + lo (range +-65504); an activation or "
            "weight outside that range overflowed. Use precision='bf16x3' (bf16 operands, fp32 range) for such weights.")
    return t


def planes_like(rows, cols, device):
    assert cols % 32 == 0, cols
    return torch.empty(rows, 2 * cols, dtype=torch.int16, device=device)


def sp_cols(p):
    return p.shape[-1] // 2


def split_planes(x, out=None, ldp=None, scale=None):
    rows, cols = x.numel() // x.shape[-1], x.shape[-1]
    ldp = (cols + 31) // 32 * 32 if ldp is None else ldp
    if out is None:
        out = planes_like(rows, ldp, x.device)
    if scale is None:
        check(lib().mvd_split_planes(ptr(x), ptr(out), rows, cols, cols, ldp, stream()))
    else:
        check(lib().mvd_split_planes_scaled(ptr(x), ptr(out), rows, cols, cols, ldp, ptr(scale), stream()))
    return out


def gemm(A, W, out=None, *, prec=PREC_X4, M=None, lda=None, bias=True, act=ACT_NONE, res=None, colscale=None,
         bias_b=None, rows_per_batch=0, epi=EPI_STORE, conv=None, qkv=None, workspace=None, splitk=0, ldo=None,
         out_planes=None, out_planes_col=0, cfg=None, gn_stats=None, gn_hw=0, gn_groups=32, row_stats=None, ln=None, gn_apply=None, cat=None,
         acc_scale_dev=None, a2=None):
    assert A.dtype == torch.int16, "A must be in split-planes format (see hip.split_planes)"
    d = GemmDesc()
    d.N, d.K = W.N, W.K
    d.A = A.data_ptr()
    d.Wp = W.data.data_ptr()
    if isinstance(W, PlanesOperand):
        d.b_mode, d.ldb = 1, W.ld
    d.acc_scale = W.acc_scale
    if acc_scale_dev is not None:
        d.acc_scale_dev = acc_scale_dev.data_ptr()
    d.prec = prec
    if conv is not None:
        d.a_mode = A_CONV3X3
        for k in ("B", "Hin", "Win", "Cin", "Hout", "Wout", "stride", "upsample"):
            setattr(d, k, int(conv[k]))
        d.no_pad_tl = int(conv.get("no_pad_tl", 0))
        d.M = conv["B"] * conv["Hout"] * conv["Wout"]
        tail_cin = getattr(W, "tail_cin", 0)
        assert (a2 is not None) == bool(tail_cin), "a weight of pack_conv3x3_tail needs a2=, and only such a weight takes it"
        if a2 is not None:
            assert a2.dtype == torch.int16 and a2.numel() // a2.shape[-1] == d.M and a2.shape[-1] // 2 >= tail_cin
            d.tap_mode, d.A2, d.lda2, d.Cin2 = TAPS_CENTRE_TAIL, a2.data_ptr(), int(a2.shape[-1] // 2), int(tail_cin)
        if getattr(W, "up4", False):
            assert a2 is None and conv["Cin"] * 4 == W.K, (conv["Cin"], W.K)
            d.tap_mode = TAPS_UP4
        else:
            assert conv["Cin"] * 9 + tail_cin == W.K, (conv["Cin"], tail_cin, W.K)
    else:
        d.a_mode = A_DENSE
        d.M = int(M if M is not None else A.numel() // A.shape[-1])
        d.lda = int(lda if lda is not None else A.shape[-1] // 2)
        assert a2 is None, "a2= (centre-tap tail) belongs to a convolution"
        assert d.lda >= W.K, f"A has {d.lda} columns, packed K is {W.K} (pad A)"
    d.epi, d.act = epi, act
    if out is not None:
        d.out = out.data_ptr()
        d.ldo = int(ldo if ldo is not None else out.shape[-1])
    if out_planes is not None:
        assert out_planes_col % 32 == 0 and out_planes.dtype == torch.int16
        d.out_sp = out_planes.data_ptr() + 4 * int(out_planes_col)
        d.ldp = int(out_planes.shape[-1] // 2)
    d.n_store = W.n_real
    if bias and W.bias is not None:
        d.bias = W.bias.data_ptr()
    if bias_b is not None:
        d.bias_b = bias_b.data_ptr()
        d.rows_per_batch = int(rows_per_batch)
        d.ldbb = bias_b.stride(0) if bias_b.dim() == 2 else 0
    if colscale is not None:
        d.colscale = colscale.data_ptr()
    if res is not None:
        d.res = res.data_ptr()
        d.ldr = int(res.shape[-1])
    if qkv is not None:
        qh, ql, kh, kl, vh, vl = qkv["planes"]
        d.q_hi, d.q_lo, d.k_hi, d.k_lo, d.vt_hi, d.vt_lo = (t.data_ptr() for t in (qh, ql, kh, kl, vh, vl))
        d.heads, d.dhead, d.L = qkv["heads"], qkv["dhead"], qkv["L"]
        d.Lpad = lib().mvd_attn_lpad(qkv["L"])
        d.qscale = float(qkv["dhead"]) ** -0.5 * 1.4426950408889634
    if gn_stats is not None:
        d.gn_stats, d.gn_hw, d.gn_groups = gn_stats.data_ptr(), int(gn_hw), int(gn_groups)
    if gn_apply is not None:
        gamma, beta, eps, flags, planes = gn_apply
        ct = d.N + (cat[0].shape[-1] if cat is not None else 0)
        assert gn_stats is not None and out is not None and planes.dtype == torch.int16 and planes.shape[-1] == 2 * ct
        if cat is not None:
            skip, raw = cat
            assert skip.dtype == torch.float32 and skip.is_contiguous() and skip.shape[0] == d.M and (raw is None or raw.shape[-1] == 2 * ct)
            d.cat_b, d.cat_cb, d.cat_raw_sp = skip.data_ptr(), int(skip.shape[-1]), (raw.data_ptr() if raw is not None else None)
        d.gna_gamma, d.gna_beta, d.gna_eps, d.gna_flags, d.gna_out_sp = gamma.data_ptr(), beta.data_ptr(), float(eps), int(flags), planes.data_ptr()
    if row_stats is not None:
        assert row_stats.slots.shape[0] >= d.M and row_stats.ld >= (d.N + 31) // 32
        d.rs_out, d.rs_count, d.rs_ld = row_stats.slots.data_ptr(), row_stats.count.data_ptr(), row_stats.ld
    if ln is not None:
        rs, fold = ln
        d.ln_stats, d.ln_count, d.ln_ld = rs.slots.data_ptr(), rs.count.data_ptr(), rs.ld
        d.ln_colsum, d.ln_dim, d.ln_eps = fold.colsum.data_ptr(), fold.dim, fold.eps
        splitk = 1
    d.splitk = splitk
    if workspace is not None:
        d.workspace = workspace.data_ptr()
        d.workspace_elems = workspace.numel()
    key = (d.M, d.N, d.K, d.a_mode, d.Cin, d.stride, d.upsample, d.no_pad_tl, d.epi, d.prec, res is not None, out is not None,
           out_planes is not None, splitk, d.b_mode, row_stats is not None, ln is not None, gn_apply is not None, cat[0].shape[-1] if cat is not None else 0,
           d.tap_mode, d.Cin2)
    if cfg is None:
        tuned = _TUNED.get(key)
        if tuned is None and AUTOTUNE and 2.0 * d.M * d.N * d.K >= AUTOTUNE_MIN_FLOPS:
            tuned = _autotune(d, A if A.is_contiguous() else None, W_data=W.data if not isinstance(W, PlanesOperand) else None)
            _TUNED[key] = tuned
            global TUNED_IN_RUN
            TUNED_IN_RUN += 1
        if tuned is not None:
            cfg, d.splitk = tuned
    d.cfg = cfg or 0
    global LAST_CFG
    LAST_CFG = d.cfg
    if GEMM_SEQUENCE is not None:
        GEMM_SEQUENCE.note(d, W)
    check(lib().mvd_gemm(C.byref(d), stream()))
    return out


GEMM_SEQUENCE = None
SELF_PREFETCH_MIN = int(os.environ.get("MVD_SELF_PREFETCH_MIN", "0"))


class WeightPrefetcher:

    def __init__(self, device, window=24 << 20, max_items=24, gn_hosts=0, self_min=None):
        self.device = device
        self.window, self.max_items = int(window), int(max_items)
        self.self_min = int(SELF_PREFETCH_MIN if self_min is None else self_min)
        self.gn_hosts = bool(gn_hosts)
        self.seq, self.recording, self.table, self.n, self.launch_idx, self.shares = [], False, None, 0, 0, {}

    class _Following:
        def __init__(self, pf, record):
            self.pf, self.record = pf, record

        def __enter__(self):
            global GEMM_SEQUENCE
            self.prev, GEMM_SEQUENCE = GEMM_SEQUENCE, self.pf
            self.pf.recording = self.record
            self.pf.launch_idx = 0
            if self.record:
                self.pf.seq = []
            return self.pf

        def __exit__(self, *exc):
            global GEMM_SEQUENCE
            GEMM_SEQUENCE = self.prev
            if self.record and exc[0] is None:
                self.pf._build()
            self.pf.recording = False
            return False

    def following(self, record=False):
        return WeightPrefetcher._Following(self, record)

    def note(self, d, W):
        j = self.launch_idx
        self.launch_idx += 1
        is_ws = bool(d.cfg) and _cfg_parts(d.cfg)[1] == WS_LOOP
        host = 1 if is_ws else (2 if (d.gna_out_sp and d.splitk != 1 and self.gn_hosts) else 0)
        if self.recording:
            packed = not isinstance(W, PlanesOperand)
            self.seq.append((W.data.data_ptr(), W.data.numel() * W.data.element_size(), host) if packed else (0, 0, host))
            return
        if host and j in self.shares:
            first, n = self.shares[j]
            d.pf_items, d.pf_n = self.table.data_ptr() + first * C.sizeof(PrefetchItem), n

    def _build(self):
        items = []
        self.shares = {}
        hosts = [j for j, e in enumerate(self.seq) if e[2]]
        sure = [j for j, e in enumerate(self.seq) if e[2] == 1]
        for j in hosts:
            nxt = [k for k in sure if k > j]
            end = nxt[0] if nxt else len(self.seq) - 1
            first, acc, seen = len(items), 0, set()
            if self.self_min > 0 and self.seq[j][2] == 1 and self.seq[j][1] >= self.self_min:
                items.append((self.seq[j][0], self.seq[j][1], j, j))
                seen.add(self.seq[j][0])
            for k in range(j + 1, end + 1):
                ptr_, nbytes, _ = self.seq[k]
                if not nbytes or ptr_ in seen or acc + nbytes > self.window or len(items) - first >= self.max_items:
                    continue
                seen.add(ptr_)
                acc += nbytes
                items.append((ptr_, nbytes, j, k))
            if len(items) > first:
                self.shares[j] = (first, len(items) - first)
        self.n = len(items)
        arr = (PrefetchItem * max(self.n, 1))()
        for i, (ptr_, nbytes, sa, cons) in enumerate(items):
            arr[i].ptr, arr[i].bytes, arr[i].start_after, arr[i].consumer = ptr_, nbytes, sa, cons
        self.table = torch.frombuffer(bytearray(bytes(arr)), dtype=torch.uint8).clone().to(self.device)
        self.items = items


CFG_STRIDE = 32
GNA_SILU, GNA_ROUND_F16, GNA_OUT_UNUSED = 1, 2, 4
TUNE_CACHE_VERSION = 12
GEMM_TILES = ((64, 64, 2, 2), (128, 128, 2, 4), (128, 80, 4, 1), (64, 80, 4, 1), (128, 160, 4, 2))
GEMM_LOOPS = (2, 3, 4, None, 6, 7, "patch", "ws")
REMOVED_LOOPS = tuple(i for i, l in enumerate(GEMM_LOOPS) if l is None)
PATCH_LOOP = 6
WS_LOOP = 7


def _cfg_parts(cfg):
    return (cfg - 1) // CFG_STRIDE, ((cfg - 1) % CFG_STRIDE) >> 1, (cfg - 1) & 1
# ... 297 lines not shown
```

mvdfusion_amd/unet.py:

```python
import math

import torch
import torch.nn as nn

from . import hip
from .attention import SpatialTransformer, ViewAlignedFeatureTransformer
from .engine import Ctx


class GroupNorm32(nn.GroupNorm):
    pass


def normalization(channels):
    return GroupNorm32(32, channels)


class TimestepBlock(nn.Module):
    pass


class Upsample(nn.Module):
    def __init__(self, channels, use_conv, dims=2, out_channels=None, padding=1):
        super().__init__()
        self.channels, self.out_channels = channels, out_channels or channels
        self.conv = nn.Conv2d(self.channels, self.out_channels, 3, padding=padding)
        self._p = self._p4 = None

    def run(self, ctx, x, H, W, out=None):
        if hip.use_up4(ctx.B, H, W, training=ctx.keep_fp32):
            if self._p4 is None:
                self._p4 = hip.pack_conv3x3_up4(self.conv.weight, self.conv.bias)
            wp = self._p4
        else:
            if self._p is None:
                self._p = hip.pack_conv3x3(self.conv.weight, self.conv.bias)
            wp = self._p
        if out is None:
            out = ctx.act((ctx.B * 4 * H * W, self.out_channels))
        xp = hip.split_planes(x, ctx.ws.planes("updown.x", ctx.B * H * W, self.channels))
        ctx.gemm(xp, wp, out, conv=dict(B=ctx.B, Hin=H, Win=W, Cin=self.channels, Hout=2 * H, Wout=2 * W,
                                            stride=1, upsample=1), gn=(ctx.B, 4 * H * W), kind="conv")
        return out, 2 * H, 2 * W


class Downsample(nn.Module):
    def __init__(self, channels, use_conv, dims=2, out_channels=None, padding=1):
        super().__init__()
        self.channels, self.out_channels = channels, out_channels or channels
        self.op = nn.Conv2d(self.channels, self.out_channels, 3, stride=2, padding=padding)
        self._p = None

    def run(self, ctx, x, H, W, out=None):
        if self._p is None:
            self._p = hip.pack_conv3x3(self.op.weight, self.op.bias)
        Ho, Wo = H // 2, W // 2
        if out is None:
            out = ctx.act((ctx.B * Ho * Wo, self.out_channels))
        xp = hip.split_planes(x, ctx.ws.planes("updown.x", ctx.B * H * W, self.channels))
        ctx.gemm(xp, self._p, out, conv=dict(B=ctx.B, Hin=H, Win=W, Cin=self.channels, Hout=Ho, Wout=Wo, stride=2,
                                            upsample=0), gn=(ctx.B, Ho * Wo), kind="conv")
        return out, Ho, Wo


class ResBlock(TimestepBlock):

    def __init__(self, channels, emb_channels, dropout, out_channels=None, dims=2, use_checkpoint=False,
                 use_scale_shift_norm=False):
        super().__init__()
        assert not use_scale_shift_norm
        self.channels, self.out_channels = channels, out_channels or channels
        self.in_layers = nn.Sequential(normalization(channels), nn.SiLU(),
                                       nn.Conv2d(channels, self.out_channels, 3, padding=1))
        self.emb_layers = nn.Sequential(nn.SiLU(), nn.Linear(emb_channels, self.out_channels))
        self.out_layers = nn.Sequential(normalization(self.out_channels), nn.SiLU(), nn.Dropout(p=dropout),
                                        nn.Conv2d(self.out_channels, self.out_channels, 3, padding=1))
        self.skip_connection = nn.Identity() if self.out_channels == channels else \
            nn.Conv2d(channels, self.out_channels, 1)
        self._p = None

    def packed(self, fuse_skip=True):
        c1, c2, sk = self.in_layers[2], self.out_layers[3], self.skip_connection
        fuse = bool(fuse_skip) and not isinstance(sk, nn.Identity)
        if self._p is None:
            self._p = (hip.pack_conv3x3(c1.weight, None), None, None)
        if self._p[1] is None or bool(self._p[1].tail_cin) != fuse:
            w2 = hip.pack_conv3x3_tail(c2.weight, c2.bias, sk.weight, sk.bias) if fuse else hip.pack_conv3x3(c2.weight, c2.bias)
            wsk = None if fuse or isinstance(sk, nn.Identity) else hip.pack_linear(sk.weight, sk.bias)
            self._p = (self._p[0], w2, wsk)
        return self._p

    def run(self, ctx, x, H, W, out=None, x_planes=None):
        B, Ci, Co = ctx.B, self.channels, self.out_channels
        M = B * H * W
        w1, w2, wsk = self.packed(fuse_skip=ctx.prec_of("skip") == ctx.prec_of("conv"))
        geo = dict(B=B, Hin=H, Win=W, Hout=H, Wout=W, stride=1, upsample=0)
        a = ctx.ws.planes("res.a", M, Ci)
        ctx.groupnorm(x, a, self.in_layers[0], B, H * W, Ci, silu=True)
        h = ctx.ws.get("res.h", (M, Co))
        a2 = ctx.ws.planes("res.a2", M, Co)
        eb = ctx.emb_bias[self]
        ctx.gemm(a, w1, h, conv=dict(Cin=Ci, **geo), bias=False, bias_b=eb, rows_per_batch=M // eb.shape[0],
                 gn=(B, H * W), kind="conv",
                 gn_apply=(self.out_layers[0], a2, True, True))
        if (wsk is not None or w2.tail_cin) and x_planes is None:
            x_planes = hip.split_planes(x, ctx.ws.planes("res.xp", M, Ci))
        if out is None:
            out = ctx.act((M, Co))
        if w2.tail_cin:
            ctx.gemm(a2, w2, out, conv=dict(Cin=Co, **geo), a2=x_planes, gn=(B, H * W), kind="conv")
            return out
        skip = x
        if wsk is not None:
            skip = ctx.ws.get("res.skip", (M, Co))
            ctx.gemm(x_planes, wsk, skip, kind="skip")
        ctx.gemm(a2, w2, out, conv=dict(Cin=Co, **geo), res=skip, gn=(B, H * W), kind="conv")
        return out


def gn_hint(layer):
    from .attention import SpatialTransformer, ViewAlignedFeatureTransformer
    if isinstance(layer, tuple):
        return layer
    if isinstance(layer, ResBlock):
        return layer.in_layers[0], "res.a", True
    if isinstance(layer, SpatialTransformer):
        return layer.norm, "tf.n", False
    if isinstance(layer, ViewAlignedFeatureTransformer):
        return layer.aligned_attn_norm, "tf.n", False
    return None


class TimestepEmbedSequential(nn.Sequential, TimestepBlock):
    def run(self, ctx, x, H, W, out=None, x_planes=None, next_layer=None, next_cat=None):
        n = len(self)
        for i, layer in enumerate(self):
            dst = out if i == n - 1 else None
            ctx.next_gn = gn_hint(self[i + 1] if i + 1 < n else next_layer)
            ctx.next_cat = next_cat if i == n - 1 else None
            if isinstance(layer, (Upsample, Downsample)):
                x, H, W = layer.run(ctx, x, H, W, out=dst)
            elif isinstance(layer, ResBlock):
                x = layer.run(ctx, x, H, W, out=dst, x_planes=x_planes if i == 0 else None)
            else:
                x = layer.run(ctx, x, H, W, out=dst)
            ctx.next_gn = None
            ctx.next_cat = None
        return x, H, W


class _StemConv(nn.Conv2d):
    _p = None

    def run(self, ctx, x, H, W, out):
        if self._p is None:
            self._p = hip.pack_conv3x3(self.weight, self.bias)
        ctx.gemm(x, self._p, out, conv=dict(B=ctx.B, Hin=H, Win=W, Cin=self._p.conv_cin, Hout=H, Wout=W, stride=1,
                                            upsample=0), gn=(ctx.B, H * W), kind="conv")
        return out


class UNetModel(nn.Module):
    def __init__(self, image_size, in_channels, model_channels, out_channels, num_res_blocks, attention_resolutions,
                 dropout=0, channel_mult=(1, 2, 4, 8), conv_resample=True, dims=2, num_classes=None,
                 use_checkpoint=False, use_fp16=False, num_heads=-1, num_head_channels=-1, num_heads_upsample=-1,
                 use_scale_shift_norm=False, resblock_updown=False, use_new_attention_order=False,
                 use_spatial_transformer=True, use_view_aligned_transformer=True, transformer_depth=1,
                 context_dim=None, n_embed=None, legacy=True):
        super().__init__()
        assert use_view_aligned_transformer and use_spatial_transformer and context_dim is not None
        assert dims == 2 and num_classes is None and not resblock_updown and n_embed is None and conv_resample
        assert num_heads != -1 and num_head_channels == -1, "this build supports the num_heads form (configs/*.yaml)"
        if isinstance(context_dim, (list, tuple)) or type(context_dim).__name__ == "ListConfig":
            context_dim = list(context_dim)[0]
        channel_mult = tuple(channel_mult)
        attention_resolutions = tuple(attention_resolutions)
        self.image_size, self.in_channels, self.model_channels = image_size, in_channels, model_channels
        self.out_channels, self.num_res_blocks, self.channel_mult = out_channels, num_res_blocks, channel_mult
        self.attention_resolutions, self.num_heads, self.context_dim = attention_resolutions, num_heads, context_dim
        ted = model_channels * 4
        self.time_embed = nn.Sequential(nn.Linear(model_channels, ted), nn.SiLU(), nn.Linear(ted, ted))

        def res(cin, cout):
            return ResBlock(cin, ted, dropout, out_channels=cout, use_checkpoint=use_checkpoint)

        def st(c):
            return SpatialTransformer(c, num_heads, c // num_heads, depth=transformer_depth, context_dim=context_dim)

        def vaft(c):
            return ViewAlignedFeatureTransformer(c, num_heads, c // num_heads, depth=transformer_depth,
                                                 context_dim=context_dim, image_size=image_size)

        self.input_blocks = nn.ModuleList([TimestepEmbedSequential(_StemConv(in_channels, model_channels, 3, padding=1))])
        skip_chans = [model_channels]
        ch, ds = model_channels, 1
        for level, mult in enumerate(channel_mult):
            for _ in range(num_res_blocks):
                layers = [res(ch, mult * model_channels)]
                ch = mult * model_channels
                if ds in attention_resolutions:
                    layers.append(st(ch))
                self.input_blocks.append(TimestepEmbedSequential(*layers))
                skip_chans.append(ch)
            if level != len(channel_mult) - 1:
                self.input_blocks.append(TimestepEmbedSequential(Downsample(ch, True, out_channels=ch)))
                skip_chans.append(ch)
                ds *= 2
        self.middle_block = TimestepEmbedSequential(res(ch, ch), st(ch), vaft(ch), res(ch, ch))
        self.output_blocks = nn.ModuleList([])
        for level, mult in list(enumerate(channel_mult))[::-1]:
            for i in range(num_res_blocks + 1):
                layers = [res(ch + skip_chans.pop(), model_channels * mult)]
                ch = model_channels * mult
                if ds in attention_resolutions:
                    layers += [st(ch), vaft(ch)]
                if level and i == num_res_blocks:
                    layers.append(Upsample(ch, True, out_channels=ch))
                    ds //= 2
                self.output_blocks.append(TimestepEmbedSequential(*layers))
        self.out = nn.Sequential(normalization(ch), nn.SiLU(), nn.Conv2d(model_channels, out_channels, 3, padding=1))
        self._head = None
        self._temb = None
        self._xattn = None
        self._head_saved = None
        self._record = None

    def get_cross_attn_parameters(self, finetune_cross_attn, finetune_view_attn):
        out = []
        for name, p in self.named_parameters():
            if finetune_cross_attn and any(k in name for k in (".norm.", ".proj_in.", ".transformer_blocks.", ".proj_out.")):
                out.append(p)
            if finetune_view_attn and ".aligned_attn_" in name:
                out.append(p)
        return out

    def disable_unet_grad(self):
        for name, p in self.named_parameters():
            if ".aligned_attn_" not in name:
                p.requires_grad_(False)

    def _resblocks(self):
        return [m for m in self.modules() if isinstance(m, ResBlock)]

    def time_biases(self, ctx, t_sin):
        if self._temb is None:
            blocks = self._resblocks()
            w = torch.cat([b.emb_layers[1].weight.detach() for b in blocks], 0).contiguous()
            bias = torch.cat([b.emb_layers[1].bias.detach() + b.in_layers[2].bias.detach() for b in blocks], 0).contiguous()
            offs, o = {}, 0
            for b in blocks:
                offs[b] = (o, o + b.out_channels)
                o += b.out_channels
            self._temb = (w, bias, offs)
        w, bias, offs = self._temb
        ted = self.model_channels * 4
        R = t_sin.shape[0]
        e1, emb = ctx.ws.get("temb.e1", (R, ted)), ctx.ws.get("temb.emb", (R, ted))
        out = ctx.ws.get("temb.bias", (R, w.shape[0]))
        ctx.gemv_rows(self.time_embed[0].weight, self.time_embed[0].bias, t_sin, e1, act_out=hip.ACT_SILU)
        ctx.gemv_rows(self.time_embed[2].weight, self.time_embed[2].bias, e1, emb)
        ctx.gemv_rows(w, bias, emb, out, act_in=hip.ACT_SILU)
        ctx.emb_bias = {b: out[:, lo:hi] for b, (lo, hi) in offs.items()}

    def cross_attn_vectors(self, ctx):
        if self._xattn is None:
            sts = [m for m in self.modules() if isinstance(m, SpatialTransformer)]
            ws, bs, offs, o = [], [], {}, 0
            for st in sts:
                a2 = st.transformer_blocks[0].attn2
                wo, wv = a2.to_out[0].weight.detach().double(), a2.to_v.weight.detach().double()
                ws.append((wo @ wv).float())
                bs.append(a2.to_out[0].bias.detach().float())
                offs[st] = (o, o + st.in_channels)
                o += st.in_channels
            self._xattn = (torch.cat(ws, 0).contiguous(), torch.cat(bs, 0).contiguous(), offs, o)
        w, bias, offs, total = self._xattn
        out = ctx.ws.get("xattn.vec", (ctx.context.shape[0], total))
        ctx.gemv_rows(w, bias, ctx.context, out)
        ctx.xattn_vec = {st: out[:, lo:hi] for st, (lo, hi) in offs.items()}

    def run(self, ctx, x_in, t_sin, S):
        B = ctx.B
        self.time_biases(ctx, t_sin)
        self.cross_attn_vectors(ctx)
        hs = []
        H = W = S
        h = x_in
        rec = self._record
        for bi, blk in enumerate(self.input_blocks):
            if rec is not None:
                rec.append((blk, h.clone(), H, W, 0))
            if bi == 0:
                o = ctx.ws.get("hs0", (B * H * W, self.model_channels))
                ctx.next_gn = gn_hint(self.input_blocks[1][0])
                h = blk[0].run(ctx, h, H, W, o)
                ctx.next_gn = None
            else:
                last = blk[-1]
                Ho, Wo = (H // 2, W // 2) if isinstance(last, Downsample) else (H, W)
                co = last.out_channels if isinstance(last, (ResBlock, Downsample)) else last.in_channels
                o = ctx.ws.get(f"hs{bi}", (B * Ho * Wo, co))
                nxt = self.input_blocks[bi + 1][0] if bi + 1 < len(self.input_blocks) else self.middle_block[0]
                h, H, W = blk.run(ctx, h, H, W, out=o, next_layer=nxt)
            hs.append((h, H, W))
        if rec is not None:
            rec.append((self.middle_block, h.clone(), H, W, 0))
        keep = rec is not None or ctx.keep_fp32

        def cat_hint(nblk, co, Hn, Wn):
            first = nblk[0]
            if keep or not isinstance(first, ResBlock) or isinstance(first.skip_connection, nn.Identity):
                return None
            nsk = hs[-1][0]
            Mn = B * Hn * Wn
            return (nsk, ctx.ws.get("cat", (Mn, co + nsk.shape[-1])), ctx.ws.planes("catp", Mn, co + nsk.shape[-1])) + gn_hint(first)

        def out_geometry(blk, H, W):
            last = blk[-1]
            co = last.out_channels if isinstance(last, (ResBlock, Upsample)) else last.in_channels
            return (co, 2 * H, 2 * W) if isinstance(last, Upsample) else (co, H, W)

        h, H, W = self.middle_block.run(ctx, h, H, W, next_cat=cat_hint(self.output_blocks[0], *out_geometry(self.middle_block, H, W)))
        for bi, blk in enumerate(self.output_blocks):
            sk, _, _ = hs.pop()
            M = B * H * W
            ca, cb = h.shape[-1], sk.shape[-1]
            cat = ctx.ws.get("cat", (M, ca + cb))
            catp = ctx.ws.planes("catp", M, ca + cb)
            first = blk[0]
            if cat.data_ptr() in ctx._cat_done:
                ctx._cat_done.discard(cat.data_ptr())
            else:
                need_cat = keep or not isinstance(first, ResBlock) or isinstance(first.skip_connection, nn.Identity)
                ctx.concat(h, ca, sk, cb, cat, catp, B, H * W, gn_apply=gn_hint(first), need_out=need_cat)
            if rec is not None:
                rec.append((blk, cat.clone(), H, W, ca))
            last_blk = bi + 1 == len(self.output_blocks)
            h, H, W = blk.run(ctx, cat, H, W, x_planes=catp, next_layer=(self.out[0], "res.a", True) if last_blk else None,
                              next_cat=None if last_blk else cat_hint(self.output_blocks[bi + 1], *out_geometry(blk, H, W)))
        if self._head is None:
            self._head = hip.pack_conv3x3(self.out[2].weight, self.out[2].bias)
        M = B * H * W
        a = ctx.ws.planes("res.a", M, self.model_channels)
        ctx.groupnorm(h, a, self.out[0], B, H * W, self.model_channels, silu=True)
        y = ctx.ws.get("head", (M, 8))
        ctx.gemm(a, self._head, y, conv=dict(B=B, Hin=H, Win=W, Cin=self.model_channels, Hout=H, Wout=W, stride=1,
                                             upsample=0), ldo=8, kind="conv")
        self._head_saved = (h, a)
        return y


class UNetWrapper(nn.Module):

    def __init__(self, unet_config, unet_path=None, drop_conditions=False, drop_scheme="default", use_zero_123=False,
                 finetune_unet=False, finetune_cross_attn=False, finetune_view_attn=True, remove_keys=()):
        super().__init__()
        params = unet_config.get("params", unet_config) if hasattr(unet_config, "get") else unet_config
        self.unet_model = UNetModel(**dict(params))
        if unet_path:
            from .load_model import load_unet_checkpoint
            load_unet_checkpoint(self.unet_model, unet_path, remove_keys=remove_keys)
        if not finetune_unet:
            self.unet_model.disable_unet_grad()
        self.drop_conditions, self.drop_scheme, self.use_zero_123 = drop_conditions, drop_scheme, use_zero_123
        self.finetune_unet, self.finetune_cross_attn, self.finetune_view_attn = \
            finetune_unet, finetune_cross_attn, finetune_view_attn

    def get_trainable_parameters(self):
        if self.finetune_unet:
            return self.unet_model.parameters()
        return self.unet_model.get_cross_attn_parameters(finetune_cross_attn=self.finetune_cross_attn,
                                                         finetune_view_attn=self.finetune_view_attn)

    def level_channels(self):
        u = self.unet_model
        return [u.model_channels * m for m in u.channel_mult]

    def level0_operand(self, ctx, B, S, D):
        rows = B * S * S * D
        if D == 1:
            c0 = self.level_channels()[0]
            return ctx.ws.get("ovol0", (rows, 2 * (c0 + 768)), torch.int16, zero=True), c0
        return ctx.ws.get("vol0", (rows, 2 * 768), torch.int16, zero=True), 0

    def volume_pyramid(self, ctx, vol, B, S, D):
        levels = [self.level0_operand(ctx, B, S, D)]
        Cc = vol.shape[-1]
        chans = self.level_channels()
        for i in range(1, len(self.unet_model.channel_mult)):
            f = 2 ** i
            rows = B * (S // f) * (S // f) * D
            if D == 1:
                ld, col = chans[i] + Cc, chans[i]
                o = ctx.ws.get(f"ovol{i}", (rows, 2 * ld), torch.int16, zero=True)
            else:
                ld, col = Cc, 0
                o = ctx.ws.planes(f"vol{i}", rows, Cc)
            hip.check(hip.lib().mvd_area_pool(hip.ptr(vol), hip.c_void_p(o.data_ptr() + 4 * col), B, S, D, Cc, f, ld, hip.stream()))
            levels.append((o, col))
        return levels
```

mvdfusion_amd/view_attn_efficient2.py:

```python
import torch
import torch.nn as nn

from . import hip
from .cameras import pack_cameras


_G4_VEC_BLOCK, _G4_VEC_MISC = 3328, 3 * 3328


def window_size(keep_top_k_views, top_k):
    return 2 * (int(top_k) // 2) + 1 if keep_top_k_views else 0


def window_view_table(V, top_k):
    half = int(top_k) // 2
    return (torch.arange(-half, half + 1)[:, None] + torch.arange(int(V))[None, :]) % int(V)


_MT_INDEX = {}


def _microtile_index(dev):
    t = _MT_INDEX.get(str(dev))
    if t is None:
# ... 60 lines not shown
        for ch in range(8):
            tiles.append(f1[4 * ch:4 * ch + 4].permute(1, 0, 2).reshape(-1, 1024))
            tiles.append(f2[:, 2 * ch:2 * ch + 2].permute(1, 0, 2).reshape(-1, 1024))
        o = bi * _G4_VEC_BLOCK
        put(o + 1536, blk.attn.qkv.bias)
        put(o + 2304, blk.attn.proj.bias)
        put(o + 2560, blk.mlp.fc1.bias)
        put(o + 3072, blk.mlp.fc2.bias)
        for k, v in enumerate((s_q, s_p, s_1, s_2)):
            host[_G4_VEC_MISC + 521 + 4 * bi + k] = v
    idx = sorted(host)
    vecs[torch.tensor(idx, device=dev)] = torch.tensor([host[k] for k in idx], dtype=torch.float32).to(dev)
    stream = torch.cat(tiles, 0).contiguous()
    assert stream.shape[0] == 16 * hip.lib().mvd_gridattn_fused_slots(), stream.shape
    return stream, vecs


class _TimmAttention(nn.Module):
    def __init__(self, dim, num_heads):
        super().__init__()
        self.num_heads = num_heads
        self.qkv = nn.Linear(dim, dim * 3, bias=True)
        self.proj = nn.Linear(dim, dim)


class _TimmMlp(nn.Module):
    def __init__(self, dim, hidden):
        super().__init__()
        self.fc1 = nn.Linear(dim, hidden)
        self.fc2 = nn.Linear(hidden, dim)


class DiTBlock(nn.Module):

    def __init__(self, hidden_size, num_heads, cond_dim=None, mlp_ratio=4.0):
        super().__init__()
        cond_dim = hidden_size if cond_dim is None else cond_dim
        self.attn = _TimmAttention(hidden_size, num_heads)
        self.mlp = _TimmMlp(hidden_size, int(hidden_size * mlp_ratio))
        self.adaLN_modulation = nn.Sequential(nn.SiLU(), nn.Linear(cond_dim, 6 * hidden_size, bias=True))
        self.hidden_size, self.num_heads = hidden_size, num_heads
        self._p = None

    def packed(self):
        if self._p is None:
            self._p = (hip.pack_linear(self.attn.qkv.weight, self.attn.qkv.bias),
                       hip.pack_linear(self.attn.proj.weight, self.attn.proj.bias),
                       hip.pack_linear(self.mlp.fc1.weight, self.mlp.fc1.bias),
                       hip.pack_linear(self.mlp.fc2.weight, self.mlp.fc2.bias))
        return self._p

    def run(self, ctx, h, h_alt, c, T, V):
        C = self.hidden_size
        wqkv, wproj, wfc1, wfc2 = self.packed()
        lin = self.adaLN_modulation[1]
        mod = ctx.ws.get("ga.mod", (1, 6 * C))
        hip.gemv(lin.weight, lin.bias, c, mod, act_in=hip.ACT_SILU)
        sh1, sc1, g1, sh2, sc2, g2 = (mod[0, i * C:(i + 1) * C] for i in range(6))
        ln = ctx.ws.planes("ga.ln", T, C)
        hip.layernorm(h, ln, sc1, sh1, T, C, eps=1e-6, w_plus_one=True)
        qkv = ctx.ws.get("ga.qkv", (T, 3 * C))
        ctx.gemm(ln, wqkv, qkv, kind="ga")
        att = ctx.ws.planes("ga.att", T, C)
        hip.check(hip.lib().mvd_view_mha(hip.ptr(qkv), hip.ptr(att), T // V, V, self.num_heads, C // self.num_heads,
                                         hip.stream()))
        ctx.gemm(att, wproj, h_alt, res=h, colscale=g1, kind="ga")
        hip.layernorm(h_alt, ln, sc2, sh2, T, C, eps=1e-6, w_plus_one=True)
        f1 = ctx.ws.planes("ga.f1", T, wfc1.N)
        ctx.gemm(ln, wfc1, None, act=hip.ACT_GELU, out_planes=f1, kind="ga")
        ctx.gemm(f1, wfc2, h, res=h_alt, colscale=g2, kind="ga")
        return h


class AggregationTransformer(nn.Module):
    def __init__(self, hidden_size, num_layers=3, num_heads=8, mlp_ratio=2.0, use_t=False):
        super().__init__()
        if not use_t:
            raise NotImplementedError
        self.use_t = use_t
        self.layer_list = nn.ModuleList([DiTBlock(hidden_size, num_heads=num_heads, mlp_ratio=mlp_ratio)
                                         for _ in range(num_layers)])
        self.weight_layer = nn.Linear(hidden_size, 1)


class _TimestepEmbedder(nn.Module):
    def __init__(self, hidden_size, frequency_embedding_size=256):
        super().__init__()
        self.mlp = nn.Sequential(nn.Linear(frequency_embedding_size, hidden_size, bias=True), nn.SiLU(),
                                 nn.Linear(hidden_size, hidden_size, bias=True))


class GridAttn(nn.Module):
    def __init__(self, input_size=32, in_channels=4, hidden_size=256, output_dim=768, num_heads=8, mlp_ratio=2.0,
                 num_layers=3, side_length=32, world_scale=0.6, z_near_far_scale=0.8, depth_scale=2.0,
                 depth_shift=0.5, n_pts_per_ray=3, use_t=True, keep_top_k_views=False, top_k=4, device="cpu"):
        super().__init__()
        self.keep_top_k_views, self.top_k = bool(keep_top_k_views), int(top_k)
        assert not self.keep_top_k_views or 1 <= self.window <= 16, f"top_k={top_k}: the window {self.window} exceeds 16 rows per 3-D point"
        assert hidden_size == 256, "the token kernel is specialised for 256-channel feature maps"
        assert in_channels == 5, "mvd_zembed reads 4 VAE + 1 depth latent channels (configs/*.yaml: in_channels: 5)"
        self.input_size, self.hidden_size, self.output_dim = input_size, hidden_size, output_dim
        self.depth_scale, self.depth_shift, self.n_pts_per_ray = depth_scale, depth_shift, n_pts_per_ray
        self.z_near_far_scale = z_near_far_scale
        self.z_embedder = nn.Sequential(nn.Linear(in_channels, 256), nn.GELU())
        self.t_embedder = _TimestepEmbedder(hidden_size)
        self.use_t = use_t
        self.pre_layer_b = nn.Sequential(nn.Linear(256 * 2 + 90 * 2 + 15 * 2 + 1, hidden_size), nn.GELU())
        self.aggregation_transformer = AggregationTransformer(hidden_size, num_layers, num_heads, mlp_ratio, use_t)
        self.final_layer_b = nn.Linear(hidden_size, output_dim)
        for blk in self.aggregation_transformer.layer_list:
            nn.init.constant_(blk.adaLN_modulation[-1].weight, 0)
            nn.init.constant_(blk.adaLN_modulation[-1].bias, 0)
        self._p = None
        self._fused = None

    def packed(self):
        if self._p is None:
            self._p = (hip.pack_linear(self.pre_layer_b[0].weight, self.pre_layer_b[0].bias),
                       hip.pack_linear(self.final_layer_b.weight, self.final_layer_b.bias))
        return self._p

    def packed_fused(self, device):
        if self._fused is None:
            stream, vecs = pack_fused_stream(self, bf16=hip.OPERAND_FORMAT == "bf16")
            self._fused = (stream.to(device), vecs.to(device))
        return self._fused

    @property
    def window(self):
        return window_size(self.keep_top_k_views, self.top_k)

    def rows_per_point(self, V):
        return self.window or int(V)

    def fused_supported(self, V, T):
        blocks = self.aggregation_transformer.layer_list
        R = self.rows_per_point(V)
        Vp = 1 << max(R - 1, 0).bit_length()
        return (V >= 1 and 1 <= R <= 16 and (T // R * Vp) % 64 == 0 and T % R == 0 and self.hidden_size == 256 and len(blocks) == 3 and
                all(b.num_heads == 8 and b.mlp.fc1.out_features == 512 for b in blocks))

    def run(self, ctx, x, depth_noise, steps, it, cams_rec, in_cam_rec, input_latents, c, vol_out, V, S, D, q0=0, Vq=None,
            vol_planes=None, vol_planes_col=0, fused=None, depth_src=None, depth_steps=None, scenes=1, steps_scene_stride=0):
        Vq = V if Vq is None else Vq
        N = int(scenes)
        L = hip.lib()
        assert x.shape[1] == 5, "depth wise efficient attention requires 4+1 channels"
        assert N == 1 or (N > 1 and x.shape[0] == N * V and input_latents.shape[0] == N and q0 == 0 and Vq == V), \
            (N, V, q0, Vq, tuple(x.shape), tuple(input_latents.shape))
        w_pre, w_fin = self.packed()
        z = self.z_embedder[0]
        feat = ctx.ws.get("ga.feat", (N * V, S, S, 256))
        in_feat = ctx.ws.get("ga.infeat", (N, S, S, 256))
        hip.check(L.mvd_zembed(hip.ptr(x), hip.ptr(z.weight), hip.ptr(z.bias), hip.ptr(feat), N * V, S, hip.stream()))
        hip.check(L.mvd_zembed(hip.ptr(input_latents), hip.ptr(z.weight), hip.ptr(z.bias), hip.ptr(in_feat), N, S,
                               hip.stream()))
        nseq = N * Vq * S * S * D
        W = self.window
        R = self.rows_per_point(V)
        T = nseq * R
        dsrc = x if depth_src is None else depth_src
        dsteps = steps if depth_steps is None else depth_steps
        assert (depth_src is None) == (depth_steps is None) and dsrc.shape == x.shape
        grid_lin = ctx.ws.bufs.get(("ga.lin", S))
        if grid_lin is None:
            half = 1.0 / float(S)
            grid_lin = torch.linspace(1.0 - half, -1.0 + half, S, dtype=torch.float32).to(ctx.device)
            ctx.ws.bufs[("ga.lin", S)] = grid_lin
        if fused is None:
            fused = self.fused_supported(V, T // N)
        sst = int(steps_scene_stride)
        if sst:
            assert N > 1 and c.shape[0] == N, (N, tuple(c.shape))
            if fused is False or not self.fused_supported(V, T // N):
                raise NotImplementedError(f"GridAttn.run: per-scene timesteps need the fused aggregation kernel (V={V}, T={T // N} per scene); "
                                          "the unfused chain shares one adaLN modulation")
            fused = True
        if fused:
            assert self.fused_supported(V, T // N), (V, T // N)
            stream, vecs = self.packed_fused(ctx.device)
            nv = vecs.numel()
            vecs = vecs.view(1, nv)
            if sst:
                vecs = ctx.ws.get("ga.vecs_scenes", (N, nv)).copy_(vecs.expand(N, nv))
            for bi, blk in enumerate(self.aggregation_transformer.layer_list):
                lin = blk.adaLN_modulation[1]
                ctx.gemv_rows(lin.weight, lin.bias, c, vecs[:, bi * _G4_VEC_BLOCK:bi * _G4_VEC_BLOCK + 1536], act_in=hip.ACT_SILU)
            pool = ctx.ws.planes("ga.pool", nseq, self.hidden_size)
            hip.check(L.mvd_gridattn_fused_window(hip.ptr(dsrc), hip.ptr(depth_noise), hip.ptr(dsteps), hip.ptr(it), hip.ptr(grid_lin),
                                                  hip.ptr(feat), hip.ptr(in_feat), hip.ptr(cams_rec), hip.ptr(in_cam_rec), hip.ptr(stream),
                                                  hip.ptr(vecs), hip.ptr(pool), N, V, q0, Vq, S, D, float(self.depth_scale),
                                                  float(self.depth_shift), 3 if ctx.prec_of("ga") == 3 else 4, sst, sst * nv, W, hip.stream()))
            ctx.gemm(pool, w_fin, vol_out, M=nseq, out_planes=vol_planes, out_planes_col=vol_planes_col, kind="ga")
            return vol_out
        tokens = ctx.ws.planes("ga.tokens", T, hip.TOKEN_LD)
        hip.check(L.mvd_gridattn_tokens_window(hip.ptr(dsrc), hip.ptr(depth_noise), hip.ptr(dsteps), hip.ptr(it), hip.ptr(grid_lin),
                                               hip.ptr(feat), hip.ptr(in_feat), hip.ptr(cams_rec), hip.ptr(in_cam_rec),
                                               hip.ptr(tokens), N, V, q0, Vq, S, D, float(self.depth_scale), float(self.depth_shift),
                                               0, W, hip.stream()))
        h = ctx.ws.get("ga.h", (T, self.hidden_size))
        h_alt = ctx.ws.get("ga.h_alt", (T, self.hidden_size))
        ctx.gemm(tokens, w_pre, h, act=hip.ACT_GELU, kind="ga")
        for blk in self.aggregation_transformer.layer_list:
            h = blk.run(ctx, h, h_alt, c, T, R)
        wl = self.aggregation_transformer.weight_layer
        pool = ctx.ws.planes("ga.pool", nseq, self.hidden_size)
        hip.check(L.mvd_view_pool(hip.ptr(h), hip.ptr(wl.weight), hip.ptr(wl.bias), hip.ptr(pool), nseq, R, self.hidden_size,
                                  hip.stream()))
        ctx.gemm(pool, w_fin, vol_out, M=nseq, out_planes=vol_planes, out_planes_col=vol_planes_col, kind="ga")
        return vol_out
```

mvdfusion_amd/viewfusion_zero_depth_rgb.py:

```python
import math

import torch
import torch.nn as nn

from . import hip
from .cameras import Cameras, get_camera_slice, get_relative_camera, pack_cameras
from .engine import Ctx, ddim_step_table
from .sampler import DDIMSampler
from .scheduler import DDPMScheduler
from .unet import UNetWrapper
from .view_attn_efficient2 import GridAttn

import os

PREFETCH_WEIGHTS = os.environ.get("MVD_PREFETCH", "ws")
PREFETCH_OPTIONS = {k: int(v) for k, v in (kv.split("=") for kv in os.environ.get("MVD_PREFETCH_OPTS", "").split(",") if kv)}


def _sinusoid_freqs(dim, max_period=10000):
    half = dim // 2
    return torch.exp(-math.log(max_period) * torch.arange(start=0, end=half, dtype=torch.float32) / half)


class StepEngine:

    def __init__(self, model, V, S, D, cfg, device, prec, q0=0, Vq=None, policy=None, scenes=1):
        self.m, self.V, self.S, self.D, self.cfg = model, V, S, D, bool(cfg)
        self.q0, self.Vq = q0, (V if Vq is None else Vq)
        self.N = N = int(scenes)
        if N < 1 or (N > 1 and (self.q0 != 0 or self.Vq != V)):
            raise ValueError(f"StepEngine(scenes={scenes}, q0={q0}, Vq={Vq}, V={V}): view-parallel sharding is single-scene only")
        NV = N * V
        self.ctx = Ctx(device, prec, policy)
        dev = self.ctx.device
        B = 2 * N * self.Vq if cfg else N * self.Vq
        self.B = B
        z = lambda *s: torch.zeros(*s, dtype=torch.float32, device=dev)
        self.x = z(NV, 5, S, S)
        self.x0 = z(NV, 5, S, S)
        self.eps = z(NV, 5, S, S)
        self.input_latents = z(N, 5, S, S)
        self.clip_v_embed = z(NV, 796)
        self.cams = z(NV, hip.CAM_RECORD)
        self.in_cam = z(N, hip.CAM_RECORD)
        self.context = z(B, 768)
        self.vol = z(B * S * S * D, 768)
        self.vol_planes, self.vol_col = model.unet_model.level0_operand(self.ctx, B, S, D)
        self.x_in = torch.zeros(B * S * S, 2 * 32, dtype=torch.int16, device=dev)
        self.iter = torch.zeros(1, dtype=torch.int32, device=dev)
        self.steps = z(1, hip.STEP_STRIDE)
        self.steps_nodiv = z(1, hip.STEP_STRIDE)
        self.prev = z(NV, 5, S, S)
        self.depth_mode = 0
        self.pin = None
        self.known = z(1, 5, S, S)
        self.pin_noise = None
        self.depth_noise = z(1, NV, D, S, S)
        self.ddim_noise = z(1, NV, 5, S, S)
        self.f256 = _sinusoid_freqs(256).to(dev)
        self.funet = _sinusoid_freqs(model.unet_model.unet_model.model_channels).to(dev)
        self.graphs = {}
        self.prefetchers = {}
        self.drop_masks = None
        self.n_rows = 1
        self.steps_scene_stride = 0
        self.done = 0

    def set_conditioning(self, batch_cameras, input_latents, input_cameras, clip_v_embed):
        self.set_conditioning_scenes([(batch_cameras, input_latents, input_cameras, clip_v_embed)])

    def set_conditioning_scenes(self, conds):
        if len(conds) != self.N:
            raise ValueError(f"set_conditioning_scenes: {len(conds)} scenes for a {self.N}-scene engine")
        V, S = self.V, self.S
        for n, (bc, il, ic, ce) in enumerate(conds):
            self.cams[n * V:(n + 1) * V].copy_(pack_cameras(bc).to(self.cams.device))
            self.in_cam[n:n + 1].copy_(pack_cameras(ic).to(self.cams.device))
            self.input_latents[n:n + 1].copy_(il.reshape(1, 5, S, S))
            self.clip_v_embed[n * V:(n + 1) * V].copy_(ce.reshape(V, 796))

    def set_schedule(self, steps_table, depth_noise, ddim_noise):
        self._set_tables(steps_table, depth_noise, ddim_noise, scene_stride=0)

    def set_schedule_scenes(self, steps_table, depth_noise, ddim_noise=None):
        if self.cfg:
            raise ValueError("StepEngine.set_schedule_scenes: per-scene timesteps need a cfg=False engine (the training step); "
                             "guided sampling steps share one timestep")
        if tuple(steps_table.shape) != (self.N, hip.STEP_STRIDE):
            raise ValueError(f"StepEngine.set_schedule_scenes: step table {tuple(steps_table.shape)} for {self.N} scenes "
                             f"(expected ({self.N}, {hip.STEP_STRIDE}))")
        if ddim_noise is None:
            ddim_noise = torch.zeros(1, self.N * self.V, 5, self.S, self.S)
        self._set_tables(steps_table, depth_noise, ddim_noise, scene_stride=1 if self.N > 1 else 0)

    def _set_tables(self, steps_table, depth_noise, ddim_noise, scene_stride):
        dev = self.ctx.device
        if self.steps.shape != steps_table.shape:
            self.graphs.clear()
            self.prefetchers.clear()
            self.steps = steps_table.to(dev).contiguous()
            self.steps_nodiv = self.steps.clone()
            self.depth_noise = depth_noise.to(dev).contiguous()
            self.ddim_noise = ddim_noise.to(dev).contiguous()
        else:
            self.steps.copy_(steps_table)
            self.depth_noise.copy_(depth_noise)
            self.ddim_noise.copy_(ddim_noise)
        self.steps_nodiv.copy_(self.steps)
        self.steps_nodiv[:, 1] = 1.0
        self.steps_scene_stride = scene_stride
        self.n_rows = int(steps_table.shape[0]) - (self.N - 1) * scene_stride
        self.rewind()

    def set_pin(self, mode, known, noise=None):
        dev = self.ctx.device
        nk = int(known.shape[0])
        K = nk // self.N
        if mode not in (0, 1) or K < 1 or K * self.N != nk or K > self.V or tuple(known.shape[1:]) != (5, self.S, self.S):
            raise ValueError(f"StepEngine.set_pin: mode {mode}, known {tuple(known.shape)} for {self.N} scene(s) of {self.V} views at "
                             f"S = {self.S} (expected (N*K, 5, S, S), 1 <= K <= V)")
        if mode == 1 and (noise is None or tuple(noise.shape) != (int(self.steps.shape[0]), nk, 5, self.S, self.S)):
            raise ValueError(f"StepEngine.set_pin: mode 1 needs noise ({int(self.steps.shape[0])}, {nk}, 5, {self.S}, {self.S}), got "
                             f"{None if noise is None else tuple(noise.shape)}")
        if self.known.shape != known.shape:
            self.graphs.clear()
            self.prefetchers.clear()
            self.known = known.to(dev, torch.float32).contiguous().clone()
        else:
            self.known.copy_(known)
        if mode == 1:
            if self.pin_noise is None or self.pin_noise.shape != noise.shape:
                self.graphs.clear()
                self.prefetchers.clear()
                self.pin_noise = noise.to(dev, torch.float32).contiguous().clone()
            else:
                self.pin_noise.copy_(noise)
        self.pin = (int(mode), K)

    def clear_pin(self):
        self.pin = None

    def rewind(self, it=0):
        assert 0 <= it < self.n_rows
        self.iter.fill_(it)
        self.done = it

    def depth_geo(self):
        if self.depth_mode == 0:
            return self.x, self.steps
        return (self.x0 if self.depth_mode == 1 else self.prev), self.steps_nodiv

    def enqueue(self, cfg_scale, do_update, prefetcher=None):
        m, ctx, L = self.m, self.ctx, hip.lib()
        V, S, D, B, q0, Vq, N = self.V, self.S, self.D, self.B, self.q0, self.Vq, self.N
        NVq = N * Vq
        ctx.B, ctx.D = B, D
        ctx.begin_step()
        st = hip.stream
        sst, R = self.steps_scene_stride, self.t_rows
        if sst and do_update:
            raise ValueError("StepEngine: per-scene timesteps (set_schedule_scenes) are a training step: no DDIM update")
        if self.pin is not None:
            mode, K = self.pin
            pn = self.pin_noise if mode == 1 else None
            hip.check(L.mvd_pin_views(hip.ptr(self.x), hip.ptr(self.x0), hip.ptr(self.known), hip.ptr(pn), N * K * 5 * S * S,
                                      hip.ptr(self.steps), hip.ptr(self.iter), N, V, K, S, mode, st()))
        ts = ctx.ws.get("vf.tsin", (R, 256))
        te1 = ctx.ws.get("vf.te1", (R, 256))
        c = ctx.ws.get("vf.c", (R, 256))
        hip.check(L.mvd_timestep_embedding_scenes(hip.ptr(self.steps), hip.ptr(self.iter), hip.ptr(self.f256), hip.ptr(ts), 256, R, sst,
                                                  st()))
        ctx.gemv_rows(m.time_embed[0].weight, m.time_embed[0].bias, ts, te1, act_out=hip.ACT_SILU)
        ctx.gemv_rows(m.time_embed[2].weight, m.time_embed[2].bias, te1, c)
        dsrc, dsteps = self.depth_geo()
        m.view_attn.run(ctx, self.x, self.depth_noise, self.steps, self.iter, self.cams, self.in_cam,
                        self.input_latents, c, self.vol, V, S, D, q0=q0, Vq=Vq, vol_planes=self.vol_planes,
                        vol_planes_col=self.vol_col, depth_src=None if self.depth_mode == 0 else dsrc,
                        depth_steps=None if self.depth_mode == 0 else dsteps, scenes=N, steps_scene_stride=sst)
        p = m.cc_projection
        c1 = ctx.ws.get("vf.cc1", (NVq, 768))
        c2 = ctx.ws.get("vf.cc2", (NVq, 768))
        ctx.gemv_rows(p[0].weight, p[0].bias, self.clip_v_embed[q0:q0 + NVq], c1, act_out=hip.ACT_SILU)
        ctx.gemv_rows(p[2].weight, p[2].bias, c1, c2, act_out=hip.ACT_SILU)
        ctx.gemv_rows(p[4].weight, p[4].bias, c2, self.context[:NVq])
        if self.drop_masks is not None:
            clip_m, vol_m, cat_m = self.drop_masks
            self.context[:NVq] *= clip_m[:, None]
            self.vol.view(B, -1)[:NVq] *= vol_m[:, None]
            vp = self.vol_planes.view(B, S * S * D, -1)
            vp[:NVq, :, 2 * self.vol_col:] *= vol_m.to(torch.int16)[:, None, None]
        ctx.context = self.context
        xq, x0q, epsq = self.x[q0:q0 + NVq], self.x0[q0:q0 + NVq], self.eps[q0:q0 + NVq]
        hip.check(L.mvd_unet_input_scenes(hip.ptr(xq), hip.ptr(self.input_latents), hip.ptr(self.x_in), N, Vq, S, 32,
                                          int(self.cfg), st()))
        if self.drop_masks is not None:
            xin = self.x_in.view(B, S * S, 64)
            cm = self.drop_masks[2].to(torch.int16)[:, None, None]
            xin[:NVq, :, 5:10] *= cm
            xin[:NVq, :, 37:42] *= cm
        unet = m.unet_model.unet_model
        ctx.vol_levels = m.unet_model.volume_pyramid(ctx, self.vol.view(B, S, S, D, 768), B, S, D)
        tsu = ctx.ws.get("vf.tsin_unet", (R, unet.model_channels))
        hip.check(L.mvd_timestep_embedding_scenes(hip.ptr(self.steps), hip.ptr(self.iter), hip.ptr(self.funet), hip.ptr(tsu),
                                                  unet.model_channels, R, sst, st()))
        y = unet.run(ctx, self.x_in, tsu, S)
        hip.check(L.mvd_cfg_ddim_update(hip.ptr(y), 8, hip.ptr(xq), hip.ptr(x0q), hip.ptr(epsq),
                                        hip.ptr(self.ddim_noise[:, q0:q0 + NVq]), N * V * 5 * S * S, hip.ptr(self.steps),
                                        hip.ptr(self.iter), NVq, S, int(self.cfg), float(cfg_scale), int(do_update), st()))
        if do_update:
            hip.check(L.mvd_advance_iter(hip.ptr(self.iter), st()))

    @property
    def t_rows(self):
        return self.N if self.steps_scene_stride else 1

    def step(self, cfg_scale, do_update, use_graph=True):
        key = (float(cfg_scale), bool(do_update), int(self.depth_mode), self.steps_scene_stride, self.pin)
        if self.done >= self.n_rows:
            raise IndexError(f"StepEngine.step: iteration {self.done} is past the {self.n_rows}-row step table "
                             "(set_schedule() / rewind() before stepping again)")
        if do_update:
            self.done += 1
        if not use_graph:
            return self.enqueue(cfg_scale, do_update)
        g = self.graphs.get(key)
        if g is None:
            it0 = self.iter.clone()
            x_keep, x0_keep = self.x.clone(), self.x0.clone()
            hip.AUTOTUNE = True
            try:
                self.enqueue(cfg_scale, do_update)
            finally:
                hip.AUTOTUNE = False
                hip.release_tuning_buffers()
            torch.cuda.synchronize()
            pf = None
            if PREFETCH_WEIGHTS == "ws":
                pf = hip.WeightPrefetcher(self.x.device, **PREFETCH_OPTIONS)
                self.iter.copy_(it0)
                self.x.copy_(x_keep)
                self.x0.copy_(x0_keep)
                with pf.following(record=True):
                    self.enqueue(cfg_scale, do_update)
                torch.cuda.synchronize()
            self.iter.copy_(it0)
            self.x.copy_(x_keep)
            self.x0.copy_(x0_keep)
            g = hip.Graph()
            self.ctx.ws.frozen = True
            try:
                with g:
                    if pf is None:
                        self.enqueue(cfg_scale, do_update)
                    else:
                        with pf.following():
                            self.enqueue(cfg_scale, do_update, prefetcher=pf)
            finally:
                self.ctx.ws.frozen = False
            self.graphs[key] = g
            self.prefetchers[key] = pf
        g.launch()


class _HipTrainingLoss(torch.autograd.Function):

    @staticmethod
    def forward(ctx, model, batch, trainer_config, names, *params):
        loss, grads = model.gradients(batch, trainer_config, noise_source=getattr(model, "_noise_source", None), only_trainable=True)
        ctx.grads = [grads.get(n) for n in names]
        ctx.shapes = [p.shape for p in params]
        return loss.clone()

    @staticmethod
    def backward(ctx, grad_out):
        if getattr(ctx, "_scaled", False):
            raise RuntimeError("_HipTrainingLoss.backward ran twice on one node: the step's gradient buffers were already scaled in place "
                               "(call model(batch, cfg) again instead of retain_graph=True)")
        ctx._scaled = True
        live, seen, spans = [], set(), []
        for g in ctx.grads:
            if g is None:
                continue
            key = (g.untyped_storage().data_ptr(), g.storage_offset(), tuple(g.shape), tuple(g.stride()))
            if key in seen:
                continue
            seen.add(key)
            live.append(g)
            spans.append((g.data_ptr(), g.data_ptr() + g.numel() * g.element_size()) if g.is_contiguous() else None)
        disjoint = all(sp is not None for sp in spans)
        if disjoint:
            srt = sorted(spans)
            disjoint = all(srt[i][1] <= srt[i + 1][0] for i in range(len(srt) - 1))
        if live and disjoint:
            torch._foreach_mul_(live, grad_out.to(live[0].dtype))
            pick = lambda g: g
        else:
            pick = lambda g: g * grad_out.to(g.dtype)
        outs = [torch.zeros(s, dtype=grad_out.dtype, device=grad_out.device) if g is None else pick(g).reshape(s)
                for g, s in zip(ctx.grads, ctx.shapes)]
        return (None, None, None, None, *outs)


class ViewFusion(nn.Module):
    def __init__(self, view_attn_config, unet_config, ddpm_config, vae_config=None, unet_path="", vae_path="",
                 clip_path="", unet_cc_path="", z_scale_factor=0.18215, vae_max_batch=8, objective="noise",
                 loss_type="l2", embed_camera_pose=True, finetune_projection=False, finetune_unet=False,
                 finetune_cross_attn=True, finetune_view_attn=True, feed_prev_depth=False, drop_conditions=False,
                 vae=None, clip_image_encoder=None, precision=None, reference_eval_dropout=False, overwrite_x_noisy=False, **kwargs):
        super().__init__()
        assert embed_camera_pose, "this build implements the embed_camera_pose=True configuration of configs/*.yaml"
        self.finetune_projection, self.finetune_unet, self.z_scale_factor = finetune_projection, finetune_unet, z_scale_factor
        self.vae_max_batch, self.objective, self.loss_type = vae_max_batch, objective, loss_type
        self.embed_camera_pose, self.finetune_cross_attn, self.finetune_view_attn = \
            embed_camera_pose, finetune_cross_attn, finetune_view_attn
        self.feed_prev_depth, self.drop_conditions = feed_prev_depth, drop_conditions
        self.reference_eval_dropout = bool(reference_eval_dropout)
        from .configs import DEFAULT_PRECISION
        precision = precision or DEFAULT_PRECISION
        fmt, self.precision, self.precision_policy = hip.parse_precision(precision)
        hip.set_operand_format(fmt)
        self.precision_name = precision

        def params(cfg):
            return dict(cfg.get("params", cfg)) if hasattr(cfg, "get") else dict(cfg)

        self.view_attn = GridAttn(**params(view_attn_config))
        self.unet_model = UNetWrapper(unet_config, unet_path=unet_path or None, drop_conditions=drop_conditions,
                                      drop_scheme="default", finetune_unet=finetune_unet,
                                      finetune_cross_attn=finetune_cross_attn, finetune_view_attn=finetune_view_attn,
                                      use_zero_123=True,
                                      remove_keys=["input_blocks.0.0.weight", "out.2.weight", "out.2.bias"])
        self.scheduler = DDPMScheduler(**params(ddpm_config))
        if vae is not None:
            self.vae = vae
        elif vae_config is not None:
            from .load_model import instantiate_from_config
            self.vae = instantiate_from_config(vae_config)
            if vae_path:
                sd = torch.load(vae_path, map_location="cpu")
                sd = sd.get("state_dict", sd)
                self.vae.load_state_dict({k.replace("first_stage_model.", ""): v for k, v in sd.items()}, strict=False)
        if clip_image_encoder is not None:
            self.clip_image_encoder = clip_image_encoder
        elif clip_path:
            from .encoders import FrozenCLIPImageEmbedder
            self.clip_image_encoder = FrozenCLIPImageEmbedder(model=clip_path, precision=precision)
            for prm in self.clip_image_encoder.parameters():
                prm.requires_grad_(False)
        self.cc_projection = nn.Sequential(nn.Linear(768 + 14 * 2, 768), nn.SiLU(True), nn.Linear(768, 768),
                                           nn.SiLU(True), nn.Linear(768, 768))
        nn.init.eye_(list(self.cc_projection.parameters())[0][:768, :768])
        nn.init.zeros_(list(self.cc_projection.parameters())[1])
        self.time_embed_dim = 256
        self.time_embed = nn.Sequential(nn.Linear(256, 256), nn.SiLU(True), nn.Linear(256, 256))
        self.register_buffer("_device", torch.tensor([0.0]), persistent=False)
        self.latent_size = int(self.view_attn.input_size)
        self.ddim = DDIMSampler(self, ddim_num_steps=50, ddim_discretize="uniform", ddim_eta=1.0,
                                latent_size=self.latent_size, z_dim=4, feed_prev_depth=feed_prev_depth,
                                overwrite_x_noisy=overwrite_x_noisy)
        self._engines = {}
        self._packed_sig = None
        assert self.finetune_view_attn is True, "must finetune new view attention layers"
# ... 430 lines not shown
```

Measured before the change: 120.4 steps/s.

## Fuse small per-step launches: pyramid pooling, paired embeddings, zembed, iter advance

Several small kernels are merged to cut launch count per denoising step. Three area-pool launches become one pyramid kernel, the two timestep embeddings and the two z-embeds each run as one paired launch, and the iteration counter is advanced by the last block of the DDIM update through an atomic ticket. The gemv kernel also gains an M<=8 variant, batched row loads, and a butterfly cross-row reduction. Split-plane creation is routed through a raw-planes helper. Risks: the ticket/volatile-iter scheme relies on correct ordering, and with CFG the pyramid is computed only over the conditional rows (n_cond).

Result: no change. 121.5 steps/s, median of 6 (+0.9%).

```diff
diff --git a/include/mvd_hip.h b/include/mvd_hip.h
--- a/include/mvd_hip.h
+++ b/include/mvd_hip.h
@@ -156,6 +156,8 @@
 int mvd_concat_groupnorm(const float* a, int Ca, const float* b, int Cb, float* out, void* raw_sp, void* y_sp, const float* gamma,
                          const float* beta, long long* gn_stats, int B, int hw, int groups, float eps, int silu, mvd_stream_t stream);
 int mvd_area_pool(const float* vol, void* out_sp, int B, int S, int D, int C, int factor, int ldp, mvd_stream_t stream);
+int mvd_area_pool_pyramid(const float* vol, void* out2_sp, int ldp2, void* out4_sp, int ldp4, void* out8_sp, int ldp8, int B, int S, int D,
+                          int C, mvd_stream_t stream);
 int mvd_fill_zero(float* p, size_t n, mvd_stream_t stream);
 
 #define MVD_STEP_STRIDE 8
@@ -163,12 +165,16 @@
                            mvd_stream_t stream);
 int mvd_timestep_embedding_scenes(const float* steps, const int* iter, const float* freqs, float* out, int dim, int nscene,
                                   int steps_scene_stride, mvd_stream_t stream);
+int mvd_timestep_embedding_pair(const float* steps, const int* iter, const float* freqs_a, float* out_a, int dim_a, const float* freqs_b,
+                                float* out_b, int dim_b, int nscene, int steps_scene_stride, mvd_stream_t stream);
 int mvd_advance_iter(int* iter, mvd_stream_t stream);
 
 #define MVD_CAM_RECORD 20
 #define MVD_TOKEN_DIM 723
 #define MVD_TOKEN_LD 736
 int mvd_zembed(const float* lat, const float* w, const float* b, float* feat, int N, int S, mvd_stream_t stream);
+int mvd_zembed_pair(const float* lat_a, float* feat_a, int Na, const float* lat_b, float* feat_b, int Nb, const float* w, const float* b,
+                    int S, mvd_stream_t stream);
 int mvd_gridattn_tokens(const float* x, const float* depth_noise, const float* steps, const int* iter,
                         const float* grid_lin ,
                         const float* feat, const float* in_feat, const float* cams, const float* in_cam,
@@ -216,6 +222,9 @@
                         const float* ddim_noise, size_t noise_stride ,
                         const float* steps, const int* iter, int V, int S, int cfg, float cfg_scale, int do_update,
                         mvd_stream_t stream);
+int mvd_cfg_ddim_update_advance(const float* eps_nhwc, int ldc, float* x, float* x0, float* eps_out, const float* ddim_noise,
+                                size_t noise_stride, const float* steps, int* iter, int V, int S, int cfg, float cfg_scale, int do_update,
+                                unsigned int* ticket, mvd_stream_t stream);
 
 int mvd_pin_views(float* x, float* x0, const float* known, const float* noise, size_t noise_stride ,
                   const float* steps, const int* iter, int groups, int group_views, int K, int S, int mode, mvd_stream_t stream);
diff --git a/mvdfusion_amd/csrc/elementwise.hip b/mvdfusion_amd/csrc/elementwise.hip
--- a/mvdfusion_amd/csrc/elementwise.hip
+++ b/mvdfusion_amd/csrc/elementwise.hip
@@ -21,20 +21,25 @@
   for (int m = 0; m < MR; ++m) acc[m] = 0.f;
   const float* wr = W + (size_t)n * K;
   if ((K & 3) == 0) {
+    constexpr int RB = MR <= 8 ? MR : 4;
     for (int k = lane * 4; k < K; k += 256) {
       const float4 w4 = *(const float4*)(wr + k);
 #pragma unroll
-      for (int m = 0; m < MR; ++m) {
-        if (m < M) {
-          float4 x4 = *(const float4*)(x + (size_t)m * ldx + k);
-          if (act_in) {
-            x4.x = act_apply(x4.x, act_in);
-            x4.y = act_apply(x4.y, act_in);
-            x4.z = act_apply(x4.z, act_in);
-            x4.w = act_apply(x4.w, act_in);
+      for (int mb = 0; mb < MR; mb += RB) {
+        float4 x4[RB];
+#pragma unroll
+        for (int m = 0; m < RB; ++m) x4[m] = *(const float4*)(x + (size_t)(mb + m < M ? mb + m : 0) * ldx + k);
+        if (act_in) {
+#pragma unroll
+          for (int m = 0; m < RB; ++m) {
+            x4[m].x = act_apply(x4[m].x, act_in);
+            x4[m].y = act_apply(x4[m].y, act_in);
+            x4[m].z = act_apply(x4[m].z, act_in);
+            x4[m].w = act_apply(x4[m].w, act_in);
           }
-          acc[m] += w4.x * x4.x + w4.y * x4.y + w4.z * x4.z + w4.w * x4.w;
         }
+#pragma unroll
+        for (int m = 0; m < RB; ++m) acc[mb + m] += w4.x * x4[m].x + w4.y * x4[m].y + w4.z * x4[m].z + w4.w * x4[m].w;
       }
     }
   } else {
@@ -45,15 +50,23 @@
         if (m < M) acc[m] += w1 * act_apply(x[(size_t)m * ldx + k], act_in);
     }
   }
-#pragma unroll
-  for (int m = 0; m < MR; ++m) {
-    if (m < M) {
-      float v = wave_sum(acc[m]);
-      if (lane == 0) {
-        if (bias) v += bias[n];
-        y[(size_t)m * ldy + n] = act_apply(v, act_out);
-      }
-    }
+  int o = 32;
+#pragma unroll
+  for (int cnt = MR; cnt > 1; cnt >>= 1, o >>= 1) {
+    const bool hi = (lane & o) != 0;
+#pragma unroll
+    for (int j = 0; j < cnt / 2; ++j) {
+      const float send = hi ? acc[j] : acc[j + cnt / 2], keep = hi ? acc[j + cnt / 2] : acc[j];
+      acc[j] = keep + __shfl_xor(send, o, 64);
+    }
+  }
+  float v = acc[0];
+#pragma unroll
+  for (; o > 0; o >>= 1) v += __shfl_xor(v, o, 64);
+  const int m = (lane * MR >> 6) & (MR - 1);
+  if ((lane & (64 / MR - 1)) == 0 && m < M) {
+    if (bias) v += bias[n];
+    y[(size_t)m * ldy + n] = act_apply(v, act_out);
   }
 }
 
@@ -296,6 +309,61 @@
   }
 }
 
+__device__ __forceinline__ void store_sp2(u16* __restrict__ base, size_t row, int ld, int k, float a, float b) {
+  uint32_t hh, ll;
+  split_op16x2(a, b, hh, ll);
+  u16* p = base + sp_index(row, ld, k);
+  *(uint32_t*)p = hh;
+  *(uint32_t*)(p + 32) = ll;
+}
+
+__global__ __launch_bounds__(64) void area_pool_pyramid_kernel(const float2* __restrict__ vol, u16* __restrict__ o2, int ld2,
+                                                               u16* __restrict__ o4, int ld4, u16* __restrict__ o8, int ld8, int B, int S,
+                                                               int D, int C2) {
+  const int S8 = S >> 3, S4 = S >> 2, S2 = S >> 1;
+  const size_t total = (size_t)B * S8 * S8 * D * C2;
+  for (size_t e = (size_t)blockIdx.x * 64 + threadIdx.x; e < total; e += (size_t)gridDim.x * 64) {
+    const int c = (int)(e % C2);
+    size_t r = e / C2;
+    const int d = (int)(r % D);
+    r /= D;
+    const int wx = (int)(r % S8);
+    r /= S8;
+    const int wy = (int)(r % S8);
+    const int b = (int)(r / S8);
+    const float2 zero = make_float2(0.f, 0.f);
+    float2 a8 = zero, a4[2] = {zero, zero};
+#pragma unroll 1
+    for (int y = 0; y < 8; y += 2) {
+      float2 v[2][8];
+#pragma unroll
+      for (int yy = 0; yy < 2; ++yy)
+#pragma unroll
+        for (int xx = 0; xx < 8; ++xx) v[yy][xx] = vol[((((size_t)b * S + wy * 8 + y + yy) * S + wx * 8 + xx) * D + d) * C2 + c];
+      if ((y & 3) == 0) a4[0] = a4[1] = zero;
+      float2 a2[4] = {zero, zero, zero, zero};
+#pragma unroll
+      for (int yy = 0; yy < 2; ++yy)
+#pragma unroll
+        for (int xx = 0; xx < 8; ++xx) {
+          const float2 t = v[yy][xx];
+          a8.x += t.x; a8.y += t.y;
+          a4[xx >> 2].x += t.x; a4[xx >> 2].y += t.y;
+          a2[xx >> 1].x += t.x; a2[xx >> 1].y += t.y;
+        }
+#pragma unroll
+      for (int j = 0; j < 4; ++j)
+        store_sp2(o2, (((size_t)b * S2 + wy * 4 + (y >> 1)) * S2 + wx * 4 + j) * D + d, ld2, c * 2, a2[j].x * 0.25f, a2[j].y * 0.25f);
+      if ((y & 3) == 2) {
+#pragma unroll
+        for (int j = 0; j < 2; ++j)
+          store_sp2(o4, (((size_t)b * S4 + wy * 2 + (y >> 2)) * S4 + wx * 2 + j) * D + d, ld4, c * 2, a4[j].x * 0.0625f, a4[j].y * 0.0625f);
+      }
+    }
+    store_sp2(o8, (((size_t)b * S8 + wy) * S8 + wx) * D + d, ld8, c * 2, a8.x * 0.015625f, a8.y * 0.015625f);
+  }
+}
+
 __global__ __launch_bounds__(256) void fill_zero_kernel(float* p, size_t n) {
   for (size_t e = (size_t)blockIdx.x * 256 + threadIdx.x; e < n; e += (size_t)gridDim.x * 256) p[e] = 0.f;
 }
@@ -312,6 +380,21 @@
   }
 }
 
+__global__ void timestep_embedding_pair_kernel(const float* __restrict__ steps, const int* __restrict__ iter, const float* __restrict__ freqs_a,
+                                               float* __restrict__ out_a, int dim_a, const float* __restrict__ freqs_b,
+                                               float* __restrict__ out_b, int dim_b, int steps_scene_stride) {
+  const float t = steps[((size_t)iter[0] + (size_t)blockIdx.x * steps_scene_stride) * MVD_STEP_STRIDE + 0];
+  const float* freqs = blockIdx.y ? freqs_b : freqs_a;
+  const int dim = blockIdx.y ? dim_b : dim_a;
+  float* out = (blockIdx.y ? out_b : out_a) + (size_t)blockIdx.x * dim;
+  const int half = dim / 2;
+  for (int i = threadIdx.x; i < half; i += blockDim.x) {
+    const float a = t * freqs[i];
+    out[i] = cosf(a);
+    out[half + i] = sinf(a);
+  }
+}
+
 __global__ void advance_iter_kernel(int* iter) {
   if (threadIdx.x == 0) iter[0] += 1;
 }
@@ -319,9 +402,9 @@
 __global__ __launch_bounds__(256) void cfg_ddim_kernel(const float* __restrict__ eps_nhwc, int ldc, float* __restrict__ x,
                                                        float* __restrict__ x0, float* __restrict__ eps_out,
                                                        const float* __restrict__ noise, const float* __restrict__ steps,
-                                                       const int* __restrict__ iter, int V, int S, int cfg, float cfg_scale,
-                                                       int do_update, size_t noise_stride) {
-  const int it = iter[0];
+                                                       int* iter, int V, int S, int cfg, float cfg_scale,
+                                                       int do_update, size_t noise_stride, unsigned int* ticket) {
+  const int it = *(const volatile int*)iter;
   const float* st = steps + (size_t)it * MVD_STEP_STRIDE;
   const float a_t = st[3], a_prev = st[4], sigma = st[5], s1m = st[6], has_noise = st[7];
   const int SS = S * S;
@@ -344,6 +427,16 @@
       if (has_noise != 0.f) xp = xp + sigma * noise[(size_t)it * noise_stride + e];
       x0[e] = px0;
       x[e] = xp;
+    }
+  }
+  if (ticket != nullptr) {
+    __syncthreads();
+    if (threadIdx.x == 0) {
+      __threadfence();
+      if (atomicAdd(ticket, 1u) == gridDim.x - 1) {
+        *ticket = 0u;
+        *iter = it + 1;
+      }
     }
   }
 }
@@ -406,6 +499,8 @@
     hipLaunchKernelGGL(gemv_kernel<1>, grid, block, 0, s, W, bias, x, y, M, N, K, ldx, ldy, act_in, act_out);
   else if (M <= 4)
     hipLaunchKernelGGL(gemv_kernel<4>, grid, block, 0, s, W, bias, x, y, M, N, K, ldx, ldy, act_in, act_out);
+  else if (M <= 8)
+    hipLaunchKernelGGL(gemv_kernel<8>, grid, block, 0, s, W, bias, x, y, M, N, K, ldx, ldy, act_in, act_out);
   else
     hipLaunchKernelGGL(gemv_kernel<16>, grid, block, 0, s, W, bias, x, y, M, N, K, ldx, ldy, act_in, act_out);
   MVD_CHECK_LAUNCH("mvd_gemv");
@@ -492,6 +587,22 @@
   return 0;
 }
 
+extern "C" int mvd_area_pool_pyramid(const float* vol, void* out2_sp, int ldp2, void* out4_sp, int ldp4, void* out8_sp, int ldp8, int B, int S,
+                                     int D, int C, mvd_stream_t stream) {
+  MVD_CHECK_ARG(vol && out2_sp && out4_sp && out8_sp && C % 32 == 0 && C > 0 && B > 0 && S > 0 && D > 0 && S % 8 == 0,
+                "mvd_area_pool_pyramid: bad arguments (C %% 32 == 0, S %% 8 == 0; S=%d C=%d)", S, C);
+  MVD_CHECK_ARG(ldp2 >= C && ldp2 % 32 == 0 && ldp4 >= C && ldp4 % 32 == 0 && ldp8 >= C && ldp8 % 32 == 0 &&
+                    (((uintptr_t)out2_sp | (uintptr_t)out4_sp | (uintptr_t)out8_sp) & 127) == 0,
+                "mvd_area_pool_pyramid: every ldp must be >= C and %% 32 == 0, every output 128-byte aligned (ldp %d %d %d)", ldp2, ldp4, ldp8);
+  const size_t total = (size_t)B * (S / 8) * (S / 8) * D * (C / 2);
+  size_t blocks = (total + 63) / 64;
+  if (blocks > 8192) blocks = 8192;
+  hipLaunchKernelGGL(area_pool_pyramid_kernel, dim3((unsigned)blocks), dim3(64), 0, (hipStream_t)stream, (const float2*)vol, (u16*)out2_sp, ldp2,
+                     (u16*)out4_sp, ldp4, (u16*)out8_sp, ldp8, B, S, D, C / 2);
+  MVD_CHECK_LAUNCH("mvd_area_pool_pyramid");
+  return 0;
+}
+
 extern "C" int mvd_fill_zero(float* p, size_t n, mvd_stream_t stream) {
   MVD_CHECK_ARG(p != nullptr, "mvd_fill_zero: null pointer");
   if (n == 0) return 0;
@@ -520,6 +631,20 @@
   return 0;
 }
 
+extern "C" int mvd_timestep_embedding_pair(const float* steps, const int* iter, const float* freqs_a, float* out_a, int dim_a,
+                                           const float* freqs_b, float* out_b, int dim_b, int nscene, int steps_scene_stride,
+                                           mvd_stream_t stream) {
+  MVD_CHECK_ARG(steps && iter && freqs_a && out_a && freqs_b && out_b && dim_a > 0 && dim_a % 2 == 0 && dim_b > 0 && dim_b % 2 == 0,
+                "mvd_timestep_embedding_pair: bad arguments");
+  MVD_CHECK_ARG(nscene >= 1 && nscene <= 65535 && steps_scene_stride >= 0 && (nscene > 1 || steps_scene_stride == 0),
+                "mvd_timestep_embedding_pair: nscene=%d (1 ... 65535), steps_scene_stride=%d (>= 0; 0 when nscene = 1)", nscene,
+                steps_scene_stride);
+  hipLaunchKernelGGL(timestep_embedding_pair_kernel, dim3(nscene, 2), dim3(256), 0, (hipStream_t)stream, steps, iter, freqs_a, out_a, dim_a,
+                     freqs_b, out_b, dim_b, steps_scene_stride);
+  MVD_CHECK_LAUNCH("mvd_timestep_embedding_pair");
+  return 0;
+}
+
 extern "C" int mvd_advance_iter(int* iter, mvd_stream_t stream) {
   MVD_CHECK_ARG(iter != nullptr, "mvd_advance_iter: null pointer");
   hipLaunchKernelGGL(advance_iter_kernel, dim3(1), dim3(64), 0, (hipStream_t)stream, iter);
@@ -527,16 +652,24 @@
   return 0;
 }
 
+extern "C" int mvd_cfg_ddim_update_advance(const float* eps_nhwc, int ldc, float* x, float* x0, float* eps_out,
+                                           const float* ddim_noise, size_t noise_stride, const float* steps, int* iter, int V,
+                                           int S, int cfg, float cfg_scale, int do_update, unsigned int* ticket, mvd_stream_t stream) {
+  MVD_CHECK_ARG(eps_nhwc && steps && iter && V > 0 && S > 0 && ldc >= 5, "mvd_cfg_ddim_update: bad arguments");
+  if (do_update) MVD_CHECK_ARG(x && x0 && ddim_noise, "mvd_cfg_ddim_update: update needs x, x0, ddim_noise");
+  MVD_CHECK_ARG(ticket == nullptr || do_update, "mvd_cfg_ddim_update_advance: the counter advances with a DDIM update only (do_update=%d)", do_update);
+  const size_t total = (size_t)V * 5 * S * S;
+  hipLaunchKernelGGL(cfg_ddim_kernel, dim3(grid_for(total)), dim3(256), 0, (hipStream_t)stream, eps_nhwc, ldc, x, x0, eps_out,
+                     ddim_noise, steps, iter, V, S, cfg, cfg_scale, do_update, noise_stride, ticket);
+  MVD_CHECK_LAUNCH("mvd_cfg_ddim_update");
+  return 0;
+}
+
 extern "C" int mvd_cfg_ddim_update(const float* eps_nhwc, int ldc, float* x, float* x0, float* eps_out,
                                    const float* ddim_noise, size_t noise_stride, const float* steps, const int* iter, int V,
                                    int S, int cfg, float cfg_scale, int do_update, mvd_stream_t stream) {
-  MVD_CHECK_ARG(eps_nhwc && steps && iter && V > 0 && S > 0 && ldc >= 5, "mvd_cfg_ddim_update: bad arguments");
-  if (do_update) MVD_CHECK_ARG(x && x0 && ddim_noise, "mvd_cfg_ddim_update: update needs x, x0, ddim_noise");
-  const size_t total = (size_t)V * 5 * S * S;
-  hipLaunchKernelGGL(cfg_ddim_kernel, dim3(grid_for(total)), dim3(256), 0, (hipStream_t)stream, eps_nhwc, ldc, x, x0, eps_out,
-                     ddim_noise, steps, iter, V, S, cfg, cfg_scale, do_update, noise_stride);
-  MVD_CHECK_LAUNCH("mvd_cfg_ddim_update");
-  return 0;
+  return mvd_cfg_ddim_update_advance(eps_nhwc, ldc, x, x0, eps_out, ddim_noise, noise_stride, steps, (int*)iter, V, S, cfg, cfg_scale, do_update,
+                                     nullptr, stream);
 }
 
 extern "C" int mvd_pin_views(float* x, float* x0, const float* known, const float* noise, size_t noise_stride, const float* steps,
diff --git a/mvdfusion_amd/csrc/gridattn.hip b/mvdfusion_amd/csrc/gridattn.hip
--- a/mvdfusion_amd/csrc/gridattn.hip
+++ b/mvdfusion_amd/csrc/gridattn.hip
@@ -49,10 +49,16 @@
 }
 
 __global__ __launch_bounds__(256) void zembed_kernel(const float* __restrict__ lat, const float* __restrict__ w,
-                                                     const float* __restrict__ bias, float* __restrict__ feat, int N, int SS) {
+                                                     const float* __restrict__ bias, float* __restrict__ feat, int N, int SS,
+                                                     const float* __restrict__ lat_b, float* __restrict__ feat_b, int Nb) {
   const int lane = threadIdx.x & 63;
-  const size_t p = (size_t)blockIdx.x * 4 + (threadIdx.x >> 6);
-  if (p >= (size_t)N * SS) return;
+  size_t p = (size_t)blockIdx.x * 4 + (threadIdx.x >> 6);
+  if (p >= (size_t)(N + Nb) * SS) return;
+  if (p >= (size_t)N * SS) {
+    p -= (size_t)N * SS;
+    lat = lat_b;
+    feat = feat_b;
+  }
   const int n = (int)(p / SS), pix = (int)(p % SS);
   float in[5];
 #pragma unroll
@@ -107,8 +113,19 @@
 extern "C" int mvd_zembed(const float* lat, const float* w, const float* b, float* feat, int N, int S, mvd_stream_t stream) {
   MVD_CHECK_ARG(lat && w && b && feat && N > 0 && S > 0, "mvd_zembed: bad arguments");
   const size_t npix = (size_t)N * S * S;
-  hipLaunchKernelGGL(zembed_kernel, dim3(cdiv(npix, 4)), dim3(256), 0, (hipStream_t)stream, lat, w, b, feat, N, S * S);
+  hipLaunchKernelGGL(zembed_kernel, dim3(cdiv(npix, 4)), dim3(256), 0, (hipStream_t)stream, lat, w, b, feat, N, S * S, (const float*)nullptr,
+                     (float*)nullptr, 0);
   MVD_CHECK_LAUNCH("mvd_zembed");
+  return 0;
+}
+
+extern "C" int mvd_zembed_pair(const float* lat_a, float* feat_a, int Na, const float* lat_b, float* feat_b, int Nb, const float* w,
+                               const float* b, int S, mvd_stream_t stream) {
+  MVD_CHECK_ARG(lat_a && feat_a && lat_b && feat_b && w && b && Na > 0 && Nb > 0 && S > 0, "mvd_zembed_pair: bad arguments");
+  const size_t npix = ((size_t)Na + Nb) * S * S;
+  MVD_CHECK_ARG((npix + 3) / 4 <= 0x7fffffff, "mvd_zembed_pair: too many pixels");
+  hipLaunchKernelGGL(zembed_kernel, dim3(cdiv(npix, 4)), dim3(256), 0, (hipStream_t)stream, lat_a, w, b, feat_a, Na, S * S, lat_b, feat_b, Nb);
+  MVD_CHECK_LAUNCH("mvd_zembed_pair");
   return 0;
 }
 
diff --git a/mvdfusion_amd/engine.py b/mvdfusion_amd/engine.py
--- a/mvdfusion_amd/engine.py
+++ b/mvdfusion_amd/engine.py
@@ -74,6 +74,8 @@
         self._unwritten = set()
         self.next_cat = None
         self._cat_done = set()
+        self.next_raw = None
+        self._raw_done = {}
         self.keep_fp32 = False
 
     def begin_step(self):
@@ -82,8 +84,10 @@
         self._gn_done.clear()
         self._unwritten.clear()
         self._cat_done.clear()
+        self._raw_done.clear()
         self.next_gn = None
         self.next_cat = None
+        self.next_raw = None
         self._gn_next = 0
         if self.gn_from_producer:
             hip.check(hip.lib().mvd_fill_zero(hip.ptr(self.gn_arena), self.gn_arena.numel() * 2, hip.stream()))
@@ -100,6 +104,7 @@
     def _forget(self, out):
         ptr = out.data_ptr()
         self._gn.pop(ptr, None)
+        self._raw_done.pop(ptr, None)
         self._unwritten.discard(ptr)
         if self._gn_done:
             for k in [k for k in self._gn_done if k[0] == ptr]:
@@ -166,6 +171,12 @@
                             planes = self.ws.planes(pname, out.shape[0], out.shape[-1])
                             kw["gn_apply"] = (norm.weight, norm.bias, norm.eps, hip.GNA_SILU if silu else 0, planes)
                             self._gn_done[(out.data_ptr(), id(norm))] = (planes, bool(silu))
+            if not handled and gn is not None and gn_apply is None and self.next_raw is not None and not self.keep_fp32 and \
+                    out.is_contiguous() and out.shape[-1] % 32 == 0 and getattr(W, "n_real", None) == W.N == out.shape[-1] and \
+                    kw.get("epi", hip.EPI_STORE) == hip.EPI_STORE and "out_planes" not in kw and "ldo" not in kw and "gn_apply" not in kw:
+                raw = self.ws.planes(self.next_raw, out.shape[0], out.shape[-1])
+                kw["raw_planes"] = raw
+                self._raw_done[out.data_ptr()] = raw
         if gn is not None:
             if os.environ.get("MVD_GN_DEBUG") and not self.capturing:
                 print(f"[gn] kind={kind} M={out.shape[0]} N={out.shape[-1]} explicit={gn_apply is not None} hint={self.next_gn is not None} "
@@ -173,10 +184,20 @@
             if gn_apply is None:
                 self.next_gn = None
                 self.next_cat = None
+                self.next_raw = None
         r = hip.gemm(A, W, out, **kw)
         if gn_apply is not None and not applied:
             self.groupnorm(out, gn_apply[1], gn_apply[0], gn[0], gn[1], out.shape[-1], gn_apply[2])
         return r
+
+    def raw_planes_of(self, x, name):
+        planes = self.ws.planes(name, x.shape[0], x.shape[-1])
+        done = self._raw_done.pop(x.data_ptr(), None)
+        if done is not None and done.data_ptr() == planes.data_ptr() and done.shape == planes.shape:
+            return planes
+        if x.data_ptr() in self._unwritten:
+            raise RuntimeError("raw planes of a tensor whose fused producer left the fp32 data unwritten")
+        return hip.split_planes(x, planes)
 
     def groupnorm(self, x, y, norm, B, HW, C, silu):
         done = self._gn_done.pop((x.data_ptr(), id(norm)), None)
diff --git a/mvdfusion_amd/hip.py b/mvdfusion_amd/hip.py
--- a/mvdfusion_amd/hip.py
+++ b/mvdfusion_amd/hip.py
@@ -158,6 +158,10 @@
     "mvd_timestep_embedding": (_i, [_vp, _vp, _vp, _vp, _i, _vp]),
     "mvd_timestep_embedding_scenes": (_i, [_vp, _vp, _vp, _vp, _i, _i, _i, _vp]),
     "mvd_advance_iter": (_i, [_vp, _vp]),
+    "mvd_timestep_embedding_pair": (_i, [_vp, _vp, _vp, _vp, _i, _vp, _vp, _i, _i, _i, _vp]),
+    "mvd_zembed_pair": (_i, [_vp, _vp, _i, _vp, _vp, _i, _vp, _vp, _i, _vp]),
+    "mvd_area_pool_pyramid": (_i, [_vp, _vp, _i, _vp, _i, _vp, _i, _i, _i, _i, _i, _vp]),
+    "mvd_cfg_ddim_update_advance": (_i, [_vp, _i, _vp, _vp, _vp, _vp, _sz, _vp, _vp, _i, _i, _i, _f, _i, _vp, _vp]),
     "mvd_zembed": (_i, [_vp, _vp, _vp, _vp, _i, _i, _vp]),
     "mvd_gridattn_tokens": (_i, [_vp] * 10 + [_i, _i, _i, _i, _i, _f, _f, _vp]),
     "mvd_gridattn_tokens_scenes": (_i, [_vp] * 10 + [_i, _i, _i, _i, _i, _i, _f, _f, _vp]),
@@ -579,7 +583,7 @@
 def gemm(A, W, out=None, *, prec=PREC_X4, M=None, lda=None, bias=True, act=ACT_NONE, res=None, colscale=None,
          bias_b=None, rows_per_batch=0, epi=EPI_STORE, conv=None, qkv=None, workspace=None, splitk=0, ldo=None,
          out_planes=None, out_planes_col=0, cfg=None, gn_stats=None, gn_hw=0, gn_groups=32, row_stats=None, ln=None, gn_apply=None, cat=None,
-         acc_scale_dev=None, a2=None):
+         acc_scale_dev=None, a2=None, raw_planes=None):
     assert A.dtype == torch.int16, "A must be in split-planes format (see hip.split_planes)"
     d = GemmDesc()
     d.N, d.K = W.N, W.K
@@ -621,6 +625,11 @@
         assert out_planes_col % 32 == 0 and out_planes.dtype == torch.int16
         d.out_sp = out_planes.data_ptr() + 4 * int(out_planes_col)
         d.ldp = int(out_planes.shape[-1] // 2)
+    if raw_planes is not None:
+        assert out_planes is None and epi == EPI_STORE and raw_planes.dtype == torch.int16 and raw_planes.shape[-1] == 2 * d.N and \
+            raw_planes.numel() // raw_planes.shape[-1] == d.M and W.n_real == d.N and gn_apply is None, \
+            "raw_planes: (M, 2 * N) planes of a STORE launch without out_planes or gn_apply"
+        d.out_sp, d.ldp = raw_planes.data_ptr(), d.N
     d.n_store = W.n_real
     if bias and W.bias is not None:
         d.bias = W.bias.data_ptr()
diff --git a/mvdfusion_amd/unet.py b/mvdfusion_amd/unet.py
--- a/mvdfusion_amd/unet.py
+++ b/mvdfusion_amd/unet.py
@@ -38,7 +38,7 @@
             wp = self._p
         if out is None:
             out = ctx.act((ctx.B * 4 * H * W, self.out_channels))
-        xp = hip.split_planes(x, ctx.ws.planes("updown.x", ctx.B * H * W, self.channels))
+        xp = ctx.raw_planes_of(x, "updown.x")
         ctx.gemm(xp, wp, out, conv=dict(B=ctx.B, Hin=H, Win=W, Cin=self.channels, Hout=2 * H, Wout=2 * W,
                                             stride=1, upsample=1), gn=(ctx.B, 4 * H * W), kind="conv")
         return out, 2 * H, 2 * W
@@ -57,7 +57,7 @@
         Ho, Wo = H // 2, W // 2
         if out is None:
             out = ctx.act((ctx.B * Ho * Wo, self.out_channels))
-        xp = hip.split_planes(x, ctx.ws.planes("updown.x", ctx.B * H * W, self.channels))
+        xp = ctx.raw_planes_of(x, "updown.x")
         ctx.gemm(xp, self._p, out, conv=dict(B=ctx.B, Hin=H, Win=W, Cin=self.channels, Hout=Ho, Wout=Wo, stride=2,
                                             upsample=0), gn=(ctx.B, Ho * Wo), kind="conv")
         return out, Ho, Wo
@@ -104,7 +104,7 @@
                  gn=(B, H * W), kind="conv",
                  gn_apply=(self.out_layers[0], a2, True, True))
         if (wsk is not None or w2.tail_cin) and x_planes is None:
-            x_planes = hip.split_planes(x, ctx.ws.planes("res.xp", M, Ci))
+            x_planes = ctx.raw_planes_of(x, "res.xp")
         if out is None:
             out = ctx.act((M, Co))
         if w2.tail_cin:
@@ -131,6 +131,14 @@
     return None
 
 
+def raw_hint(layer):
+    if isinstance(layer, (Upsample, Downsample)):
+        return "updown.x"
+    if isinstance(layer, ResBlock) and not isinstance(layer.skip_connection, nn.Identity):
+        return "res.xp"
+    return None
+
+
 class TimestepEmbedSequential(nn.Sequential, TimestepBlock):
     def run(self, ctx, x, H, W, out=None, x_planes=None, next_layer=None, next_cat=None):
         n = len(self)
@@ -138,6 +146,7 @@
             dst = out if i == n - 1 else None
             ctx.next_gn = gn_hint(self[i + 1] if i + 1 < n else next_layer)
             ctx.next_cat = next_cat if i == n - 1 else None
+            ctx.next_raw = raw_hint(self[i + 1] if i + 1 < n else next_layer)
             if isinstance(layer, (Upsample, Downsample)):
                 x, H, W = layer.run(ctx, x, H, W, out=dst)
             elif isinstance(layer, ResBlock):
@@ -146,6 +155,7 @@
                 x = layer.run(ctx, x, H, W, out=dst)
             ctx.next_gn = None
             ctx.next_cat = None
+            ctx.next_raw = None
         return x, H, W
 
 
@@ -383,10 +393,13 @@
             return ctx.ws.get("ovol0", (rows, 2 * (c0 + 768)), torch.int16, zero=True), c0
         return ctx.ws.get("vol0", (rows, 2 * 768), torch.int16, zero=True), 0
 
-    def volume_pyramid(self, ctx, vol, B, S, D):
+    pyramid_one_launch = True
+
+    def volume_pyramid(self, ctx, vol, B, S, D, n_cond=None):
         levels = [self.level0_operand(ctx, B, S, D)]
         Cc = vol.shape[-1]
         chans = self.level_channels()
+        dst = []
         for i in range(1, len(self.unet_model.channel_mult)):
             f = 2 ** i
             rows = B * (S // f) * (S // f) * D
@@ -395,7 +408,14 @@
                 o = ctx.ws.get(f"ovol{i}", (rows, 2 * ld), torch.int16, zero=True)
             else:
                 ld, col = Cc, 0
-                o = ctx.ws.planes(f"vol{i}", rows, Cc)
-            hip.check(hip.lib().mvd_area_pool(hip.ptr(vol), hip.c_void_p(o.data_ptr() + 4 * col), B, S, D, Cc, f, ld, hip.stream()))
+                o = ctx.ws.get(f"vol{i}", (rows, 2 * Cc), torch.int16, zero=True)
+            dst.append((hip.c_void_p(o.data_ptr() + 4 * col), ld, f))
             levels.append((o, col))
+        if self.pyramid_one_launch and len(dst) == 3 and S % 8 == 0:
+            (o2, l2, _), (o4, l4, _), (o8, l8, _) = dst
+            hip.check(hip.lib().mvd_area_pool_pyramid(hip.ptr(vol), o2, l2, o4, l4, o8, l8, B if n_cond is None else n_cond, S, D, Cc,
+                                                      hip.stream()))
+        else:
+            for o, ld, f in dst:
+                hip.check(hip.lib().mvd_area_pool(hip.ptr(vol), o, B, S, D, Cc, f, ld, hip.stream()))
         return levels
diff --git a/mvdfusion_amd/view_attn_efficient2.py b/mvdfusion_amd/view_attn_efficient2.py
--- a/mvdfusion_amd/view_attn_efficient2.py
+++ b/mvdfusion_amd/view_attn_efficient2.py
@@ -236,9 +236,8 @@
         z = self.z_embedder[0]
         feat = ctx.ws.get("ga.feat", (N * V, S, S, 256))
         in_feat = ctx.ws.get("ga.infeat", (N, S, S, 256))
-        hip.check(L.mvd_zembed(hip.ptr(x), hip.ptr(z.weight), hip.ptr(z.bias), hip.ptr(feat), N * V, S, hip.stream()))
-        hip.check(L.mvd_zembed(hip.ptr(input_latents), hip.ptr(z.weight), hip.ptr(z.bias), hip.ptr(in_feat), N, S,
-                               hip.stream()))
+        hip.check(L.mvd_zembed_pair(hip.ptr(x), hip.ptr(feat), N * V, hip.ptr(input_latents), hip.ptr(in_feat), N, hip.ptr(z.weight),
+                                    hip.ptr(z.bias), S, hip.stream()))
         nseq = N * Vq * S * S * D
         W = self.window
         R = self.rows_per_point(V)
diff --git a/mvdfusion_amd/viewfusion_zero_depth_rgb.py b/mvdfusion_amd/viewfusion_zero_depth_rgb.py
--- a/mvdfusion_amd/viewfusion_zero_depth_rgb.py
+++ b/mvdfusion_amd/viewfusion_zero_depth_rgb.py
@@ -23,6 +23,8 @@
 
 
 class StepEngine:
+
+    fuse_iter_advance = True
 
     def __init__(self, model, V, S, D, cfg, device, prec, q0=0, Vq=None, policy=None, scenes=1):
         self.m, self.V, self.S, self.D, self.cfg = model, V, S, D, bool(cfg)
@@ -48,6 +50,7 @@
         self.vol_planes, self.vol_col = model.unet_model.level0_operand(self.ctx, B, S, D)
         self.x_in = torch.zeros(B * S * S, 2 * 32, dtype=torch.int16, device=dev)
         self.iter = torch.zeros(1, dtype=torch.int32, device=dev)
+        self.iter_ticket = torch.zeros(1, dtype=torch.int32, device=dev)
         self.steps = z(1, hip.STEP_STRIDE)
         self.steps_nodiv = z(1, hip.STEP_STRIDE)
         self.prev = z(NV, 5, S, S)
@@ -143,6 +146,7 @@
     def rewind(self, it=0):
         assert 0 <= it < self.n_rows
         self.iter.fill_(it)
+        self.iter_ticket.zero_()
         self.done = it
 
     def depth_geo(self):
@@ -168,8 +172,10 @@
         ts = ctx.ws.get("vf.tsin", (R, 256))
         te1 = ctx.ws.get("vf.te1", (R, 256))
         c = ctx.ws.get("vf.c", (R, 256))
-        hip.check(L.mvd_timestep_embedding_scenes(hip.ptr(self.steps), hip.ptr(self.iter), hip.ptr(self.f256), hip.ptr(ts), 256, R, sst,
-                                                  st()))
+        unet = m.unet_model.unet_model
+        tsu = ctx.ws.get("vf.tsin_unet", (R, unet.model_channels))
+        hip.check(L.mvd_timestep_embedding_pair(hip.ptr(self.steps), hip.ptr(self.iter), hip.ptr(self.f256), hip.ptr(ts), 256,
+                                                hip.ptr(self.funet), hip.ptr(tsu), unet.model_channels, R, sst, st()))
         ctx.gemv_rows(m.time_embed[0].weight, m.time_embed[0].bias, ts, te1, act_out=hip.ACT_SILU)
         ctx.gemv_rows(m.time_embed[2].weight, m.time_embed[2].bias, te1, c)
         dsrc, dsteps = self.depth_geo()
@@ -198,16 +204,14 @@
             cm = self.drop_masks[2].to(torch.int16)[:, None, None]
             xin[:NVq, :, 5:10] *= cm
             xin[:NVq, :, 37:42] *= cm
-        unet = m.unet_model.unet_model
-        ctx.vol_levels = m.unet_model.volume_pyramid(ctx, self.vol.view(B, S, S, D, 768), B, S, D)
-        tsu = ctx.ws.get("vf.tsin_unet", (R, unet.model_channels))
-        hip.check(L.mvd_timestep_embedding_scenes(hip.ptr(self.steps), hip.ptr(self.iter), hip.ptr(self.funet), hip.ptr(tsu),
-                                                  unet.model_channels, R, sst, st()))
+        ctx.vol_levels = m.unet_model.volume_pyramid(ctx, self.vol.view(B, S, S, D, 768), B, S, D, n_cond=NVq if self.cfg else None)
         y = unet.run(ctx, self.x_in, tsu, S)
-        hip.check(L.mvd_cfg_ddim_update(hip.ptr(y), 8, hip.ptr(xq), hip.ptr(x0q), hip.ptr(epsq),
-                                        hip.ptr(self.ddim_noise[:, q0:q0 + NVq]), N * V * 5 * S * S, hip.ptr(self.steps),
-                                        hip.ptr(self.iter), NVq, S, int(self.cfg), float(cfg_scale), int(do_update), st()))
-        if do_update:
+        fuse = bool(do_update) and self.fuse_iter_advance
+        hip.check(L.mvd_cfg_ddim_update_advance(hip.ptr(y), 8, hip.ptr(xq), hip.ptr(x0q), hip.ptr(epsq),
+                                                hip.ptr(self.ddim_noise[:, q0:q0 + NVq]), N * V * 5 * S * S, hip.ptr(self.steps),
+                                                hip.ptr(self.iter), NVq, S, int(self.cfg), float(cfg_scale), int(do_update),
+                                                hip.ptr(self.iter_ticket) if fuse else None, st()))
+        if do_update and not fuse:
             hip.check(L.mvd_advance_iter(hip.ptr(self.iter), st()))
 
     @property
```
